# jvasilakes/disentanglement-vae

Hardware: NVIDIA B200
Metric: train_tokens_per_sec (higher is better)
Workload: dtype f32

## Files before the change

disentanglement-vae_b200/_lib.py:

```python
import ctypes as C
import os

_HERE = os.path.dirname(os.path.abspath(__file__))
LIB_PATH = os.path.join(_HERE, "libdvae_b200.so")

MAX_SPACES = 8
HEADS_NSCALARS = 3 + 3 * MAX_SPACES


class DvaeError(RuntimeError):
    pass


_p = C.c_void_p
_i = C.c_int
_l = C.c_int64
_f = C.c_float
_u32 = C.c_uint32
_pp = C.POINTER(C.c_void_p)
_ip = C.POINTER(C.c_int)

SIGNATURES = {
    "dvae_last_error_string": (C.c_char_p, []),
    "dvae_version": (_i, []),
    "dvae_launch_count": (_l, []),
    "dvae_weight_planes_floats": (_l, [_i, _i, _i]),
    "dvae_weight_planes_register": (_i, [_p, _i, _i, _p, _p]),
    "dvae_weight_planes_refresh": (_i, [_p]),
    "dvae_weight_planes_refresh_ex": (_i, [_i, _i, _p]),
    "dvae_weight_planes_enable": (_i, [_i]),
    "dvae_weight_planes_clear": (_i, []),
    "dvae_defer_joins": (_i, [_i]),
    "dvae_join_side_streams": (_i, [_p]),
    "dvae_linear": (_i, [_p, _l, _i, _p, _l, _i, _p, _l, _i, _i, _i, _p, _p, _f, _i, _p]),
    "dvae_tc_linear": (_i, [_p, _l, _i, _p, _l, _i, _p, _l, _i, _i, _i, _p, _p, _f, _i, _i, _p]),
    "dvae_tc16_linear": (_i, [_p, _l, _i, _p, _l, _i, _p, _l, _i, _i, _i, _p, _p, _f, _i, _f, _f, _p, _p, _p]),
    "dvae_colsum": (_i, [_p, _l, _i, _i, _p, _f, _p]),
    "dvae_randn": (_i, [_p, _l, _p, _u32, _p]),
    "dvae_embedding_fwd": (_i, [_p, _i, _p, _l, _l, _i, _i, _f, _p, _u32, _l, _i, _p, _p]),
    "dvae_embedding_bwd": (_i, [_p, _i, _p, _l, _l, _i, _i, _f, _p, _u32, _l, _i, _p, _p]),
    "dvae_bow_encoder_fwd": (_i, [_p, _i, _p, _l, _l, _i, _i, _f, _p, _u32, _p, _l, _p, _p]),
    "dvae_bow_encoder_bwd": (_i, [_p, _l, _p, _i, _p, _l, _l, _i, _i, _f, _p, _u32, _p, _p]),
    "dvae_dropout": (_i, [_p, _l, _l, _i, _f, _p, _u32, _p, _l, _l, _p]),
    "dvae_lstm_step": (_i, [_p, _l, _i, _i, _i, _i, _i, _p, _p, _p, _p, _p, _p, _l, _p, _p, _p, _p, _p]),
    "dvae_vocab_sample_step": (_i, [_p, _l, _i, _i, _i, _p, _p, _p, _u32, _p, _l, _p, _p]),
    "dvae_vocab_sample_step_ex": (_i, [_p, _l, _i, _i, _i, _p, _p, _p, _u32, _p, _l, _p, _p, _p]),
    "dvae_vocab_w_planes_floats": (_l, [_i, _i]),
    "dvae_vocab_w_planes": (_i, [_p, _i, _i, _p, _p]),
    "dvae_vocab_sample_step_planes": (_i, [_p, _l, _i, _i, _i, _p, _p, _p, _p, _u32, _p, _l, _p, _p, _p]),
    "dvae_recount_lengths": (_i, [_p, _l, _l, _i, _i, _l, _l, _l, _p, _p]),
    "dvae_bleu_counts": (_i, [_p, _l, _i, _p, _l, _i, _i, _l, _p, _p]),
    "dvae_bleu_score": (_i, [_p, _p, _p]),
    "dvae_lstm_state_ws_floats": (_l, [_i, _i, _i]),
    "dvae_lstm_seq_fwd": (_i, [_p, _l, _i, _i, _i, _i, _i, _pp, _pp, _pp, _pp, _p, _p, _l, _l, _p, _p, _l, _p, _p,
                               _l, _l, _p, _p, _p, _p]),
    "dvae_lstm_input_proj": (_i, [_p, _l, _i, _i, _i, _i, _i, _pp, _pp, _pp, _p, _p]),
    "dvae_lstm_seq_fwd_ex": (_i, [_p, _l, _i, _i, _i, _i, _i, _pp, _pp, _pp, _pp, _p, _p, _l, _l, _p, _p, _l, _p, _p,
                                  _l, _l, _p, _p, _p, _i, _p]),
    "dvae_lstm_seq_bwd": (_i, [_p, _l, _i, _i, _i, _i, _i, _pp, _pp, _p, _p, _l, _l, _p, _p, _l, _p, _p, _p, _l,
                               _p, _p, _l, _l, _p, _l, _pp, _pp, _pp, _pp, _p, _p, _l, _l, _p, _p]),
    "dvae_lstm_bwd_planes_ws_floats": (_l, [_i, _i, _i, _i, _i]),
    "dvae_lstm_seq_bwd_ex": (_i, [_p, _l, _i, _i, _i, _i, _i, _pp, _pp, _p, _p, _l, _l, _p, _p, _l, _p, _p, _p, _l,
                                  _p, _p, _l, _l, _p, _l, _pp, _pp, _pp, _pp, _p, _p, _l, _l, _p, _p, _p]),
    "dvae_counter_increment": (_i, [_p, _p]),
    "dvae_fork_after": (_i, [_i, _p, _p, C.POINTER(C.c_void_p)]),
    "dvae_nvls_barrier_words": (_l, []),
    "dvae_nvls_all_reduce": (_i, [_p, _l, _pp, _i, _i, _p, C.c_uint32, C.c_uint32, _i, C.c_uint64, _p, _p]),
    "dvae_p2p_all_reduce": (_i, [_pp, _l, _pp, _i, _i, _p, C.c_uint32, C.c_uint32, _i, C.c_uint64, _p, _p]),
    "dvae_heads_ws_floats": (_l, [_i, _i]),
    "dvae_latent_heads_fwd": (_i, [_p, _i, _i, _i, _ip, _ip, _p, _p, _p, _p, _p, _p, _p, _p, _p, _i, _p, _p, _p,
                                   _p, _p, _p, _p, _p]),
    "dvae_heads_bwd_ws_floats": (_l, [_i, _i, _i]),
    "dvae_latent_heads_bwd": (_i, [_p, _i, _i, _i, _ip, _ip, _p, _p, _p, _p, _p, _p, _i, _p, _p, _p, _p, _p, _p,
                                   _p, _p, _p, _p, _p, _p, _p, _p, _p, _p, _p, _p, _p]),
    "dvae_dsc_loss": (_i, [_p, _p, _i, _i, _ip, _ip, _p, _p, _p, _p]),
    "dvae_vocab_ce_ws_floats": (_l, [_i, _i, _i]),
    "dvae_vocab_ce_fwd": (_i, [_p, _l, _i, _i, _i, _i, _p, _p, _p, _l, _p, _i, _p, _p, _p, _p, _p, _p]),
    "dvae_vocab_split_w": (_i, [_p, _i, _i, _i, _p, _p]),
    "dvae_vocab_ce_fwd_ex": (_i, [_p, _l, _i, _i, _i, _i, _p, _p, _p, _l, _p, _i, _p, _p, _p, _p, _p, _i, _p]),
    "dvae_vocab_ce_partials": (_i, [_p, _l, _i, _i, _i, _i, _p, _p, _p, _l, _p, _i, _p, _p]),
    "dvae_vocab_ce_bwd_ws_floats": (_l, [_i, _i, _i]),
    "dvae_vocab_ce_bwd": (_i, [_p, _l, _i, _i, _i, _i, _p, _p, _p, _l, _p, _p, _p, _p, _l, _p, _p, _p, _p, _p]),
    "dvae_entropy_loss": (_i, [_p, _i, _i, _p, _p, _p, _p]),
    "dvae_club_mi": (_i, [_p, _p, _p, _i, _i, _p, _p, _p, _p, _p, _p, _p]),
    "dvae_club_nll": (_i, [_p, _p, _p, _i, _i, _p, _p, _p, _p, _p]),
    "dvae_act_bwd": (_i, [_p, _p, _p, _l, _i, _p]),
    "dvae_relu": (_i, [_p, _l, _p]),
    "dvae_grad_sumsq": (_i, [_p, _l, _p, _p, _p]),
    "dvae_clip_adam": (_i, [_p, _p, _p, _p, _l, _p, _f, _f, _p, _i, _p]),
}

_lib = None
planes_owner = None


def load():
    global _lib
    if _lib is not None:
        return _lib
    if not os.path.exists(LIB_PATH):
        raise DvaeError(
            f"{LIB_PATH} not found: build it with `python -c 'import __graft_entry__ as g; g.build()'` "
            "(nvcc, sm_100a).  There is no CPU or PyTorch fallback for this path.")
    lib = C.CDLL(LIB_PATH)
    for name, (res, args) in SIGNATURES.items():
        try:
            fn = getattr(lib, name)
        except AttributeError as e:
            raise DvaeError(f"{LIB_PATH} does not export {name}") from e
        fn.restype = res
        fn.argtypes = args
    _lib = lib
    return lib


def check(rc, what):
    if rc != 0:
        msg = load().dvae_last_error_string()
        raise DvaeError(f"{what} failed ({rc}): {msg.decode() if msg else ''}")


def ptr(t):
    return None if t is None else t.data_ptr()


def ptr_array(tensors):
    arr = (C.c_void_p * max(len(tensors), 1))()
    for i, t in enumerate(tensors):
        arr[i] = None if t is None else t.data_ptr()
    return arr


def int_array(vals):
    arr = (C.c_int * max(len(vals), 1))()
    for i, v in enumerate(vals):
        arr[i] = int(v)
    return arr


def stream_ptr():
    import torch
    return torch.cuda.current_stream().cuda_stream


def launch_count():
    return int(load().dvae_launch_count())
```

disentanglement-vae_b200/csrc/tc_gemm16.cu:

```cuda
#include <cuda_fp16.h>
#include <stdlib.h>
#include <string.h>

#include "tc_gemm.cuh"
#include "tc_gemm16.cuh"
#include "tc_planes.cuh"

namespace dvae {
namespace tc16 {

using namespace tc;

constexpr int BM = 128, BN = 128, BK = 32;
constexpr int STAGES = 6, MAX_STAGES = 14;
constexpr int RAW_TILE = BM * BK * 4;
constexpr int STAGE_BYTES = 2 * RAW_TILE;
constexpr int PS_PLANE = BM * BK * 2, PS_TILE = 2 * PS_PLANE;
constexpr int PS_LBO = 128, PS_SBO = 512;
static_assert(PS_TILE == RAW_TILE, "in-place conversion: fp16 hi + lo planes occupy exactly the landed fp32 tile");
constexpr int EPI_WARPS = 8, MMA_WARP = 4, TMA_WARP = 5, PROD_WARP0 = 6, PROD_WARPS = 16, EPI2_WARP0 = PROD_WARP0 + PROD_WARPS;
constexpr int NUM_THREADS = (EPI2_WARP0 + 4) * 32;
constexpr int CONV_BARRIER = 1;
constexpr int EPI_SCRATCH_BYTES = 8 * 32 * 32 * 4;
#ifndef DVAE_AS_KB
#define DVAE_AS_KB 2
#endif
constexpr int AS_MAX_KB = 8, AS_KB_PER_STAGE = DVAE_AS_KB, AS_STAGE_BYTES = AS_KB_PER_STAGE * PS_TILE;
constexpr int AS_STAGES = 12 / AS_KB_PER_STAGE, AS_STAGES_NOSCRATCH = 14 / AS_KB_PER_STAGE;
constexpr uint32_t AS_T_AHI = 256, AS_T_ALO = 384;
constexpr float kSingleScale = 256.f;
constexpr int OFF_SCRATCH = STAGES * STAGE_BYTES;
constexpr int OFF_BIAS = OFF_SCRATCH + EPI_SCRATCH_BYTES;
constexpr int OFF_BAR = OFF_BIAS + 8 * 64 * 4;
constexpr int SMEM_BYTES = OFF_BAR + 512;
static_assert(AS_STAGES * AS_STAGE_BYTES <= OFF_SCRATCH, "A-stationary ring must end before the transpose scratch");
static_assert(AS_STAGES_NOSCRATCH * AS_STAGE_BYTES <= OFF_BIAS, "A-stationary mode-1 ring must end before the bias tiles");
static_assert(AS_STAGES_NOSCRATCH <= MAX_STAGES && (3 * MAX_STAGES + 5) * 8 + 4 <= 512, "barrier area");
static_assert(SMEM_BYTES <= 232448, "shared memory per CTA");
constexpr int TMEM_COLS = 512;
constexpr float kLoScale = 2048.f, kLoInv = 1.f / 2048.f;

__device__ __forceinline__ float ex2_ftz(float x) {
  float y;
  asm("ex2.approx.ftz.f32 %0, %1;" : "=f"(y) : "f"(x));
  return y;
}
constexpr float kLog2e = 1.4426950408889634f;

__device__ __forceinline__ unsigned long long gtime16() {
  unsigned long long t;
  asm volatile("mov.u64 %0, %%globaltimer;" : "=l"(t));
  return t;
}
#ifdef DVAE_TC16_PROBES
#define DVAE_TC16_FLAG(bit) (p.dbg_skip_epilogue & (bit))
#define DVAE_TC16_MARK(cond, i) do { if (cond) DBG16(i); } while (0)
#else
#define DVAE_TC16_FLAG(bit) false
#define DVAE_TC16_MARK(cond, i) do { } while (0)
#endif
#define DBG16(i) do { if (p.dbg && blockIdx.x == 0 && blockIdx.y == 0 && blockIdx.z == 0) p.dbg[i] = gtime16(); } while (0)

__device__ __forceinline__ float scale_from_amax(const uint32_t* amax_bits, int n, float static_scale) {
  if (!amax_bits) return static_scale;
  uint32_t mx = 0;
  for (int i = 0; i < n; ++i) mx = max(mx, __ldg(amax_bits + i));
  int se = 267 - (int)(mx >> 23);
  se = se < 1 ? 1 : (se > 253 ? 253 : se);
  return __uint_as_float((unsigned)se << 23);
}

__device__ __forceinline__ void load_tile(uint32_t raw, int mn_major, int ptid, float (&v)[8]) {
  const int row = ptid & 127, kc = ptid >> 7;
  if (!mn_major) {
    const uint32_t ra = raw + (uint32_t)row * 128, sw = row & 7;
#pragma unroll
    for (int i = 0; i < 2; ++i) {
      const uint4 t = lds128(ra + (((uint32_t)(2 * kc + i) ^ sw) << 4));
      v[4 * i] = __uint_as_float(t.x); v[4 * i + 1] = __uint_as_float(t.y);
      v[4 * i + 2] = __uint_as_float(t.z); v[4 * i + 3] = __uint_as_float(t.w);
    }
  } else {
    const uint32_t src = raw + (uint32_t)(8 * kc) * (BM * 4) + (uint32_t)row * 4;
#pragma unroll
    for (int j = 0; j < 8; ++j) v[j] = lds32(src + j * (BM * 4));
  }
}

__device__ __forceinline__ void store_tile(uint32_t tile, int ptid, float s, const float (&v)[8]) {
  const int row = ptid & 127, kc = ptid >> 7;
  const uint32_t base = tile + (uint32_t)(row >> 3) * PS_SBO + (uint32_t)kc * PS_LBO + (row & 7) * 16;
  uint4 hi, lo;
  hi.x = pack_hi_lo(v[0], v[1], s, lo.x);
  hi.y = pack_hi_lo(v[2], v[3], s, lo.y);
  hi.z = pack_hi_lo(v[4], v[5], s, lo.z);
  hi.w = pack_hi_lo(v[6], v[7], s, lo.w);
  sts128(base, hi);
  sts128(base + PS_PLANE, lo);
}

__device__ __forceinline__ uint32_t cluster_size() {
  uint32_t n;
  asm volatile("mov.u32 %0, %%cluster_nctaid.x;" : "=r"(n));
  return n;
}
__device__ __forceinline__ uint32_t cluster_rank() {
  uint32_t r;
  asm volatile("mov.u32 %0, %%cluster_ctarank;" : "=r"(r));
  return r;
}
__device__ __forceinline__ void cluster_sync_all() {
  asm volatile("barrier.cluster.arrive.release.aligned;\n\tbarrier.cluster.wait.acquire.aligned;" ::: "memory");
}
__device__ __forceinline__ void bulk_load_multicast(uint32_t smem_dst, const void* src, uint32_t bytes, uint64_t* bar, uint16_t mask) {
  asm volatile("cp.async.bulk.shared::cluster.global.mbarrier::complete_tx::bytes.multicast::cluster [%0], [%1], %2, [%3], %4;" ::"r"(smem_dst),
               "l"(src), "r"(bytes), "r"(smem_u32(bar)), "h"(mask)
               : "memory");
}
__device__ __forceinline__ void tc_commit_multicast(uint64_t* bar, uint16_t mask) {
  asm volatile("tcgen05.commit.cta_group::1.mbarrier::arrive::one.shared::cluster.multicast::cluster.b64 [%0], %1;" ::"r"(smem_u32(bar)),
               "h"(mask)
               : "memory");
}

__device__ __forceinline__ void bulk_load(uint32_t smem_dst, const void* src, uint32_t bytes, uint64_t* bar) {
  asm volatile("cp.async.bulk.shared::cluster.global.mbarrier::complete_tx::bytes [%0], [%1], %2, [%3];" ::"r"(smem_dst), "l"(src),
               "r"(bytes), "r"(smem_u32(bar))
               : "memory");
}

__global__ void split_planes_kernel(const float* __restrict__ X, int64_t ld, int R, int K, float scale, float lo_scale,
                                    uint8_t* __restrict__ planes) {
  const int KB = (K + BK - 1) / BK, KC = KB * (BK / 8), RP = (R + BM - 1) / BM * BM;
  const int64_t total = (int64_t)RP * KC;
  for (int64_t i = (int64_t)blockIdx.x * blockDim.x + threadIdx.x; i < total; i += (int64_t)gridDim.x * blockDim.x) {
    const int kc = (int)(i % KC), r = (int)(i / KC);
    float v[8];
#pragma unroll
    for (int e = 0; e < 8; ++e) v[e] = (r < R && kc * 8 + e < K) ? __ldg(X + (int64_t)r * ld + kc * 8 + e) : 0.f;
    uint4 h, l;
    h.x = pack_hi_lo(v[0], v[1], scale, l.x, lo_scale); h.y = pack_hi_lo(v[2], v[3], scale, l.y, lo_scale);
    h.z = pack_hi_lo(v[4], v[5], scale, l.z, lo_scale); h.w = pack_hi_lo(v[6], v[7], scale, l.w, lo_scale);
    const int64_t off = ((int64_t)(r >> 7) * KB + (kc >> 2)) * (2 * PS_PLANE) + ((r & 127) >> 3) * PS_SBO + (kc & 3) * PS_LBO + (r & 7) * 16;
    *reinterpret_cast<uint4*>(planes + off) = h;
    *reinterpret_cast<uint4*>(planes + off + PS_PLANE) = l;
  }
}

__global__ void weight_planes_kernel(PlaneTable tab) {
  const PlaneTable::Entry e = tab.e[blockIdx.y >> 1];
  const int tr = blockIdx.y & 1;
  uint8_t* out = reinterpret_cast<uint8_t*>(tr ? e.planes_t : e.planes);
  if (!out) return;
  const int R = tr ? e.C : e.R, K = tr ? e.R : e.C;
  const int64_t ld = e.ld ? e.ld : e.C;
  const float sc = scale_from_amax(e.amax, e.amax_n, 1.f);
  const int KB = (K + BK - 1) / BK, KC = KB * (BK / 8), RP = (R + BM - 1) / BM * BM;
  const int64_t total = (int64_t)RP * KC;
  for (int64_t i = (int64_t)blockIdx.x * blockDim.x + threadIdx.x; i < total; i += (int64_t)gridDim.x * blockDim.x) {
    int kc, r;
    if (!tr) { kc = (int)(i % KC); r = (int)(i / KC); }
    else { r = (int)(i % RP); kc = (int)(i / RP); }
    float v[8];
#pragma unroll
    for (int j = 0; j < 8; ++j) {
      const int k = kc * 8 + j;
      v[j] = (r < R && k < K) ? __ldg(tr ? e.w + (int64_t)k * ld + r : e.w + (int64_t)r * ld + k) : 0.f;
    }
    uint4 h, l;
    h.x = pack_hi_lo(v[0], v[1], sc, l.x); h.y = pack_hi_lo(v[2], v[3], sc, l.y);
    h.z = pack_hi_lo(v[4], v[5], sc, l.z); h.w = pack_hi_lo(v[6], v[7], sc, l.w);
    const int64_t off = ((int64_t)(r >> 7) * KB + (kc >> 2)) * (2 * PS_PLANE) + ((r & 127) >> 3) * PS_SBO + (kc & 3) * PS_LBO + (r & 7) * 16;
    *reinterpret_cast<uint4*>(out + off) = h;
    *reinterpret_cast<uint4*>(out + off + PS_PLANE) = l;
  }
}

int weight_planes_launch(const PlaneTable& tab, cudaStream_t st) {
  if (tab.n <= 0) return DVAE_OK;
  int64_t most = 1;
  for (int i = 0; i < tab.n; ++i) most = max(most, (int64_t)tab.e[i].R * tab.e[i].C / 8);
  int bx = ceil_div(most, 256 * 4);
  bx = bx < 8 ? 8 : (bx > 4 * 148 ? 4 * 148 : bx);
  weight_planes_kernel<<<dim3(bx, 2 * tab.n), 256, 0, st>>>(tab);
  DVAE_LAUNCH_CHECK();
  return DVAE_OK;
}

__global__ void __launch_bounds__(NUM_THREADS, 1)
tc16_gemm_kernel(const __grid_constant__ CUtensorMap tmA, const __grid_constant__ CUtensorMap tmB, Params p) {
  extern __shared__ __align__(1024) uint8_t smem[];
  if (p.skip_flag && *p.skip_flag) return;
  uint64_t* bars = reinterpret_cast<uint64_t*>(smem + OFF_BAR);
  uint64_t* full = bars;
  uint64_t* empty = bars + MAX_STAGES;
  uint64_t* raw_full = bars + 2 * MAX_STAGES;
  uint64_t* tmem_full = raw_full + MAX_STAGES;
  uint64_t* tmem_empty = tmem_full + 2;
  uint64_t* a_full = tmem_empty + 2;
  uint32_t* tmem_slot = reinterpret_cast<uint32_t*>(a_full + 1);

  const int tid = threadIdx.x, warp = tid >> 5, lane = tid & 31;
  const bool wide_epi = p.presplit && p.mode != 0;
  const uint32_t csize = p.mcast ? cluster_size() : 1, crank = p.mcast ? cluster_rank() : 0;
  const uint16_t cmask = (uint16_t)((1u << csize) - 1);
  const bool conv_as_epi = wide_epi && warp >= PROD_WARP0 && warp < PROD_WARP0 + EPI_WARPS;
  asm volatile("griddepcontrol.launch_dependents;" ::: "memory");
  if (tid == 0) DBG16(0);
  if (p.zero_buf) {
    float4* z4 = reinterpret_cast<float4*>(p.zero_buf);
    const int64_t nblk = (int64_t)gridDim.x * gridDim.y * gridDim.z;
    const int64_t blk = ((int64_t)blockIdx.z * gridDim.y + blockIdx.y) * gridDim.x + blockIdx.x;
    for (int64_t i = blk * NUM_THREADS + tid; i < p.zero_n4; i += nblk * NUM_THREADS) z4[i] = make_float4(0.f, 0.f, 0.f, 0.f);
    if (p.zero_buf2) {
      float4* y4 = reinterpret_cast<float4*>(p.zero_buf2);
      for (int64_t i = blk * NUM_THREADS + tid; i < p.zero2_n4; i += nblk * NUM_THREADS) y4[i] = make_float4(0.f, 0.f, 0.f, 0.f);
    }
  }
  const int m0 = blockIdx.x * BM;
  const int nt0 = blockIdx.y * p.tiles_per_cta;
  const int n_tiles = (p.N + BN - 1) / BN;
  const int nt1 = min(n_tiles, nt0 + p.tiles_per_cta);
  const int nkb_total = (p.K + BK - 1) / BK;
  const int kb0 = blockIdx.z * p.kb_per_split;
  const int nkb = max(0, min(nkb_total, kb0 + p.kb_per_split) - kb0);
  const int b_tile0 = p.b_row0 / BN;

  if (tid == 0) {
    if (smem_u32(smem) & 1023) {
      printf("dvae tc16_gemm: dynamic shared memory base is not 1024-byte aligned\n");
      __trap();
    }
    for (int s = 0; s < MAX_STAGES; ++s) {
      mbar_init(&full[s], p.presplit ? 1 : PROD_WARPS / 2 + (p.b_presplit ? 1 : 0));
      mbar_init(&empty[s], p.mcast ? csize : 1);
      mbar_init(&raw_full[s], 1);
    }
    for (int a = 0; a < 2; ++a) {
      mbar_init(&tmem_full[a], 1);
      mbar_init(&tmem_empty[a], wide_epi ? 2 * EPI_WARPS : EPI_WARPS);
    }
    mbar_init(a_full, 2 * EPI_WARPS);
    fence_barrier_init();
  }
  if (warp == TMA_WARP && lane == 0 && !p.presplit) {
    tma_prefetch_desc(&tmA);
    tma_prefetch_desc(&tmB);
  }
  const bool a_stat = p.presplit && !p.no_astat && nkb_total <= AS_MAX_KB && gridDim.z == 1;
  const int nstages = a_stat ? (p.mode == 1 ? AS_STAGES_NOSCRATCH : AS_STAGES) : STAGES;
  const uint32_t stage_bytes = a_stat ? AS_STAGE_BYTES : STAGE_BYTES;
  const int a_blk = min((int)blockIdx.x, (p.M + BM - 1) / BM - 1);
  if (warp == MMA_WARP) tmem_alloc(tmem_slot, TMEM_COLS);
  tc_fence_before();
  __syncthreads();
  if (p.mcast) cluster_sync_all();
  tc_fence_after();
  const uint32_t tmem_base = *tmem_slot;
  const uint32_t smem_u = smem_u32(smem);

  if (warp == TMA_WARP) {
    if (DVAE_TC16_FLAG(16)) {
    } else if (lane == 0 && a_stat) {
      const uint8_t* b_planes = reinterpret_cast<const uint8_t*>(p.b_planes);
      int stage = 0, phase = 0;
      for (int nt = nt0; nt < nt1; ++nt) {
        for (int kb = 0; kb < nkb; kb += AS_KB_PER_STAGE) {
          DVAE_TC16_MARK(nt == nt0 + 1 && kb < 8, 32 + 2 * kb);
          if (!DVAE_TC16_FLAG(8)) mbar_wait(&empty[stage], phase ^ 1);
          else mbar_wait(&full[stage], phase ^ 1);
          DVAE_TC16_MARK(nt == nt0 + 1 && kb < 8, 33 + 2 * kb);
          const uint32_t dst = smem_u + stage * AS_STAGE_BYTES;
          const uint32_t bytes = (uint32_t)min(AS_KB_PER_STAGE, nkb - kb) * PS_TILE;
          mbar_expect_tx(&full[stage], bytes);
          const uint8_t* src = b_planes + ((int64_t)(nt + b_tile0) * nkb_total + kb) * PS_TILE;
          if (csize == 1) {
            bulk_load(dst, src, bytes, &full[stage]);
          } else {
            const uint32_t part = bytes / csize, off = crank * part;
            bulk_load_multicast(dst + off, src + off, part, &full[stage], cmask);
          }
          if (++stage == nstages) { stage = 0; phase ^= 1; }
        }
      }
      if (DVAE_TC16_FLAG(8))
        for (int s2 = 0; s2 < nstages; ++s2) mbar_wait(&full[s2], s2 < stage ? phase : phase ^ 1);
    } else if (lane == 0 && p.presplit) {
      const uint8_t* a_tiles = reinterpret_cast<const uint8_t*>(p.a_planes) +
                               ((int64_t)blockIdx.x * (p.a_kbtot ? p.a_kbtot : nkb_total) + p.a_kb0) * PS_TILE;
      const uint8_t* b_planes = reinterpret_cast<const uint8_t*>(p.b_planes);
      int stage = 0, phase = 0;
      for (int nt = nt0; nt < nt1; ++nt) {
        for (int kb = 0; kb < nkb; ++kb) {
          mbar_wait(&empty[stage], phase ^ 1);
          const uint32_t dst = smem_u + stage * STAGE_BYTES;
          mbar_expect_tx(&full[stage], STAGE_BYTES);
          bulk_load(dst, a_tiles + (int64_t)(kb0 + kb) * PS_TILE, PS_TILE, &full[stage]);
          bulk_load(dst + PS_TILE, b_planes + ((int64_t)(nt + b_tile0) * (p.b_kbtot ? p.b_kbtot : nkb_total) + p.b_kb0 + kb0 + kb) * PS_TILE,
                    PS_TILE, &full[stage]);
          if (++stage == STAGES) { stage = 0; phase ^= 1; }
        }
      }
    } else if (lane == 0) {
      int stage = 0, phase = 0;
      for (int nt = nt0; nt < nt1; ++nt) {
        for (int kb = 0; kb < nkb; ++kb) {
          mbar_wait(&empty[stage], phase ^ 1);
          uint8_t* dst = smem + stage * STAGE_BYTES;
          mbar_expect_tx(&raw_full[stage], p.b_presplit ? RAW_TILE : STAGE_BYTES);
          const int k0 = (kb0 + kb) * BK;
          if (!p.a_mn) tma_load_2d(dst, &tmA, k0, m0, &raw_full[stage]);
          else tma_load_2d(dst, &tmA, m0, k0, &raw_full[stage]);
          if (p.b_presplit) {
            mbar_expect_tx(&full[stage], PS_TILE);
            bulk_load(smem_u + stage * STAGE_BYTES + RAW_TILE,
                      reinterpret_cast<const uint8_t*>(p.b_planes) + ((int64_t)(nt + b_tile0) * p.b_kbtot + p.b_kb0 + kb0 + kb) * PS_TILE,
                      PS_TILE, &full[stage]);
          } else if (!p.b_mn) tma_load_2d(dst + RAW_TILE, &tmB, k0, nt * BN, &raw_full[stage]);
          else tma_load_2d(dst + RAW_TILE, &tmB, nt * BN, k0, &raw_full[stage]);
          if (++stage == STAGES) { stage = 0; phase ^= 1; }
        }
      }
    }
  } else if (warp >= PROD_WARP0 && warp < EPI2_WARP0 && !conv_as_epi) {
    const int ptid = tid - PROD_WARP0 * 32;
    const float sa = scale_from_amax(p.a_amax, p.a_amax_n, p.a_scale), sb = scale_from_amax(p.b_amax, p.b_amax_n, p.b_scale);
    const int n_items = p.presplit ? 0 : (nt1 - nt0) * nkb;
    const int grp = ptid >> 8, gtid = ptid & 255;
    for (int it = grp; it < n_items; it += 2) {
      const int stage = it % STAGES, phase = (it / STAGES) & 1;
      DVAE_TC16_MARK(ptid == 0 && it == 12, 2);
      mbar_wait(&raw_full[stage], phase);
      DVAE_TC16_MARK(ptid == 0 && it == 12, 3);
      float va0[8], va1[8], vb0[8], vb1[8];
      const uint32_t st = smem_u + stage * STAGE_BYTES;
      load_tile(st, p.a_mn, gtid, va0);
      load_tile(st, p.a_mn, gtid + 256, va1);
      if (!p.b_presplit) {
        load_tile(st + RAW_TILE, p.b_mn, gtid, vb0);
        load_tile(st + RAW_TILE, p.b_mn, gtid + 256, vb1);
      }
      asm volatile("bar.sync %0, %1;" ::"r"(CONV_BARRIER + grp), "n"(PROD_WARPS * 16) : "memory");
      store_tile(st, gtid, sa, va0);
      store_tile(st, gtid + 256, sa, va1);
      if (!p.b_presplit) {
        store_tile(st + PS_TILE, gtid, sb, vb0);
        store_tile(st + PS_TILE, gtid + 256, sb, vb1);
      }
      DVAE_TC16_MARK(ptid == 0 && it == 12, 4);
      fence_proxy_async();
      __syncwarp();
      if (lane == 0) mbar_arrive(&full[stage]);
      DVAE_TC16_MARK(ptid == 0 && it == 12, 5);
    }
  } else if (warp == MMA_WARP) {
    constexpr uint32_t idesc = (1u << 4) | ((uint32_t)(BN >> 3) << 17) | ((uint32_t)(BM >> 4) << 24);
    if (elect_one() && nkb > 0) {
      if (a_stat) {
        mbar_wait(a_full, 0);
        tc_fence_after();
      }
      constexpr uint32_t d_hi = ((PS_SBO >> 4) & 0x3FFF) | (1u << 14);
      constexpr uint32_t d_lo = ((PS_LBO >> 4) & 0x3FFF) << 16;
      constexpr uint32_t kstep16 = (2 * PS_LBO) >> 4, plane16 = PS_PLANE >> 4;
      const uint32_t stage16 = stage_bytes >> 4;
      const uint32_t base16 = smem_u >> 4;
      const uint32_t ring16 = base16;
      const uint32_t b_off16 = a_stat ? 0 : 2 * plane16;
      auto desc = [&](uint32_t addr16) { return ((uint64_t)d_hi << 32) | (uint64_t)(d_lo | (addr16 & 0x3FFF)); };
      int stage = 0, phase = 0;
      uint32_t st16 = ring16;
      for (int tile = 0; tile < nt1 - nt0; ++tile) {
        const int acc = tile & 1;
        if (tile >= 2) {
          mbar_wait(&tmem_empty[acc], ((tile >> 1) - 1) & 1);
          tc_fence_after();
        }
        const uint32_t d1 = tmem_base + (a_stat ? acc * 128 : acc * 256), d2 = d1 + 128;
        if (a_stat) {
          for (int kb = 0; kb < nkb; kb += AS_KB_PER_STAGE) {
            if (!DVAE_TC16_FLAG(4)) mbar_wait(&full[stage], phase);
            if (!DVAE_TC16_FLAG(2)) {
#pragma unroll
              for (int kk = 0; kk < AS_KB_PER_STAGE; ++kk) {
                if (kb + kk < nkb) {
                  const uint32_t ta = tmem_base + (uint32_t)(kb + kk) * 16, sb16 = st16 + kk * (PS_TILE >> 4);
#pragma unroll
                  for (int k = 0; k < BK / 16; ++k) {
                    const uint32_t adv = k * kstep16;
                    mma_f16_ts(d1, ta + AS_T_AHI + 8 * k, desc(sb16 + adv), idesc, (kb | kk | k) ? 1u : 0u);
                    mma_f16_ts(d1, ta + AS_T_AHI + 8 * k, desc(sb16 + plane16 + adv), idesc, 1u);
                    mma_f16_ts(d1, ta + AS_T_ALO + 8 * k, desc(sb16 + adv), idesc, 1u);
                  }
                }
              }
            }
            if (!DVAE_TC16_FLAG(8)) {
              if (csize == 1) tc_commit(&empty[stage]);
              else tc_commit_multicast(&empty[stage], cmask);
            }
            st16 += stage16;
            if (++stage == nstages) { stage = 0; phase ^= 1; st16 = ring16; }
          }
          tc_commit(&tmem_full[acc]);
          continue;
        }
        for (int kb = 0; kb < nkb; ++kb) {
          DVAE_TC16_MARK(tile == 1 && kb < 8, 48 + 2 * kb);
          if (!DVAE_TC16_FLAG(4)) mbar_wait(&full[stage], phase);
          DVAE_TC16_MARK(tile == 1 && kb < 8, 49 + 2 * kb);
          const uint32_t sa16 = st16, sb16 = st16 + b_off16;
          if (!DVAE_TC16_FLAG(2)) {
#pragma unroll
            for (int k = 0; k < BK / 16; ++k) {
              const uint32_t adv = k * kstep16;
              const uint32_t accum = (kb | k) ? 1u : 0u;
              mma_f16(d1, desc(sa16 + adv), desc(sb16 + adv), idesc, accum);
              mma_f16(d2, desc(sa16 + adv), desc(sb16 + plane16 + adv), idesc, accum);
              mma_f16(d2, desc(sa16 + plane16 + adv), desc(sb16 + adv), idesc, 1u);
            }
          }
          if (!DVAE_TC16_FLAG(8)) {
            if (csize == 1) tc_commit(&empty[stage]);
            else tc_commit_multicast(&empty[stage], cmask);
          }
          st16 += stage16;
          if (++stage == nstages) { stage = 0; phase ^= 1; st16 = ring16; }
        }
        tc_commit(&tmem_full[acc]);
      }
    }
    __syncwarp();
  } else {
    const int quarter = warp & 3, ehalf = warp >= EPI2_WARP0 ? 1 : 0;
    const int c_lo = !wide_epi ? 2 * ehalf : (conv_as_epi ? 1 + 2 * ((warp - PROD_WARP0) >> 2) : 2 * ehalf);
    const int c_hi = wide_epi ? c_lo + 1 : c_lo + 2;
    const int ew = wide_epi ? c_lo * 4 + quarter : ehalf * 4 + quarter;
    const int row = m0 + quarter * 32 + lane;
    const bool row_ok = row < p.M;
    const float oscale = p.alpha * (p.alpha_dev ? *p.alpha_dev : 1.f) * ((p.c_row_scale && row_ok) ? __ldg(p.c_row_scale + row) : 1.f) /
                         (scale_from_amax(p.a_amax, p.a_amax_n, p.a_scale) * scale_from_amax(p.b_amax, p.b_amax_n, p.b_scale));
    float rm = -INFINITY, rs = 0.f, rt = 0.f, rav = -INFINITY, row_lse = 0.f, row_nlse2 = 0.f, row_scale = 0.f;
    int rai = 0x7fffffff, tgt = -1;
    if (p.mode != 0 && row_ok) {
      const int b = row % p.B, tpos = row / p.B + 1;
      if (p.targets) tgt = (int)p.targets[(int64_t)b * p.tgt_stride_b + tpos];
      if (p.mode == 2) {
        row_lse = p.lse[row];
        row_nlse2 = -row_lse * kLog2e;
        row_scale = (tpos < p.lengths[b]) ? (p.grad_scale ? p.grad_scale[0] : 1.f) / (float)p.B : 0.f;
        tgt -= p.v0;
      }
    }
    if (a_stat) {
      const uint8_t* a_tiles = reinterpret_cast<const uint8_t*>(p.a_planes) + (int64_t)a_blk * nkb_total * PS_TILE;
      const int r = quarter * 32 + lane;
      const uint32_t roff = (uint32_t)(r >> 3) * PS_SBO + (r & 7) * 16;
      const uint32_t tlane = tmem_base + ((uint32_t)(quarter * 32) << 16);
#pragma unroll
      for (int i = 0; i < 2; ++i) {
        const int kb = 2 * c_lo + i;
        if (kb < nkb) {
          const uint8_t* t = a_tiles + (int64_t)kb * PS_TILE + roff;
#pragma unroll
          for (int pl = 0; pl < 2; ++pl) {
            uint32_t v[16];
#pragma unroll
            for (int kc = 0; kc < 4; ++kc) {
              const uint4 q = __ldg(reinterpret_cast<const uint4*>(t + pl * PS_PLANE + kc * PS_LBO));
              v[4 * kc] = q.x; v[4 * kc + 1] = q.y; v[4 * kc + 2] = q.z; v[4 * kc + 3] = q.w;
            }
            tmem_st16(tlane + (pl ? AS_T_ALO : AS_T_AHI) + kb * 16, v);
          }
        }
      }
      tmem_st_wait();
      tc_fence_before();
      __syncwarp();
      if (lane == 0) mbar_arrive(a_full);
    }
    float bias_next[2] = {0.f, 0.f};
    if (p.mode != 0 && nkb > 0) {
#pragma unroll
      for (int h2 = 0; h2 < 2; ++h2) {
        const int col = nt0 * BN + (c_lo + h2) * 32 + lane;
        bias_next[h2] = (nt0 < nt1 && h2 < c_hi - c_lo && col < p.N) ? __ldg(p.bias + col) : 0.f;
      }
    }
    int tile = 0;
    for (int nt = nt0; nt < nt1 && nkb > 0; ++nt, ++tile) {
      const int n0 = nt * BN, acc = tile & 1;
      mbar_wait(&tmem_full[acc], (tile >> 1) & 1);
      tc_fence_after();
      if (tid == 0 && tile < 4) DBG16(14 + 2 * tile);
      DVAE_TC16_MARK(tid == 0 && tile == 2, 96);
      float* sbias = reinterpret_cast<float*>(smem + OFF_BIAS) + (wide_epi ? ew * 32 : ew * 64);
      const uint32_t sbias_u = smem_u + OFF_BIAS + (wide_epi ? ew * 32 : ew * 64) * 4;
      if (p.mode != 0) {
        __syncwarp();
#pragma unroll
        for (int h2 = 0; h2 < 2; ++h2)
          if (h2 < c_hi - c_lo) sbias[h2 * 32 + lane] = bias_next[h2];
        __syncwarp();
#pragma unroll
        for (int h2 = 0; h2 < 2; ++h2) {
          const int col = n0 + BN + (c_lo + h2) * 32 + lane;
          bias_next[h2] = (nt + 1 < nt1 && h2 < c_hi - c_lo && col < p.N) ? __ldg(p.bias + col) : 0.f;
        }
      }
      DVAE_TC16_MARK(tid == 0 && tile == 2, 97);
#pragma unroll 1
      for (int c = c_lo; c < c_hi; ++c) {
        const int col0 = n0 + c * 32;
        if (col0 >= p.N || DVAE_TC16_FLAG(~0)) continue;
        const uint32_t ta = tmem_base + ((uint32_t)(quarter * 32) << 16) + (a_stat ? acc * 128 : acc * 256) + c * 32;
        if (p.mode == 2 && wide_epi) {
          const uint32_t sc = smem_u + OFF_SCRATCH + ew * (32 * 16 * 4);
          const int r0 = m0 + quarter * 32;
          const int nr = min(32, p.M - r0);
          const bool dead = row_scale == 0.f;
          DVAE_TC16_MARK(tid == 0 && tile == 2, 104);
#pragma unroll
          for (int hh = 0; hh < 2; ++hh) {
#pragma unroll
            for (int h8 = 0; h8 < 2; ++h8) {
              float v[8], w[8];
              if (a_stat) {
                tmem_ld8_pair(ta + hh * 16 + h8 * 8, ta + hh * 16 + h8 * 8, v, w);
#pragma unroll
                for (int j = 0; j < 8; ++j) w[j] = 0.f;
              } else {
                tmem_ld8_pair(ta + hh * 16 + h8 * 8, ta + 128 + hh * 16 + h8 * 8, v, w);
              }
#pragma unroll
              for (int q = 0; q < 2; ++q) {
                const uint4 t = lds128(sbias_u + (hh * 16 + h8 * 8 + 4 * q) * 4);
                const float bq[4] = {__uint_as_float(t.x), __uint_as_float(t.y), __uint_as_float(t.z), __uint_as_float(t.w)};
#pragma unroll
                for (int jj = 0; jj < 4; ++jj) {
                  const int j = 4 * q + jj, col = col0 + hh * 16 + h8 * 8 + j;
                  const float e = ex2_ftz(fmaf(fmaf(fmaf(w[j], kLoInv, v[j]), oscale, bq[jj]), kLog2e, row_nlse2));
                  v[j] = (dead || col >= p.N) ? 0.f : (e - (col == tgt ? 1.f : 0.f)) * row_scale;
                }
              }
              if (p.p_planes_a && col0 + hh * 16 + h8 * 8 < p.p_kb_a * BK && m0 < (p.M + BM - 1) / BM * BM)
                store_plane_chunk(p.p_planes_a, row, col0 + hh * 16 + h8 * 8, p.p_kb_a, v, p.p_scale);
#pragma unroll
              for (int j = 0; j < 8; ++j) sts32(sc + (lane * 16 + ((h8 * 8 + j) ^ ((lane >> 1) & 15))) * 4, v[j]);
            }
            __syncwarp();
            if (p.p_planes_t) {
              const int cc = lane & 15, rg = lane >> 4, colw = col0 + hh * 16 + cc;
              float tv[16], ssum = 0.f;
#pragma unroll
              for (int k = 0; k < 16; ++k) {
                const int r = rg * 16 + k;
                tv[k] = lds32(sc + (r * 16 + (cc ^ ((r >> 1) & 15))) * 4);
                ssum += tv[k];
              }
              ssum += __shfl_xor_sync(0xffffffffu, ssum, 16);
              if (colw < p.N) {
                if (rg == 0 && p.p_colsum) atomicAdd(p.p_colsum + colw, ssum);
                const float lo8[8] = {tv[0], tv[1], tv[2], tv[3], tv[4], tv[5], tv[6], tv[7]};
                const float hi8[8] = {tv[8], tv[9], tv[10], tv[11], tv[12], tv[13], tv[14], tv[15]};
                if (r0 + rg * 16 < p.p_kb_t * BK) store_plane_chunk(p.p_planes_t, colw, r0 + rg * 16, p.p_kb_t, lo8, p.p_scale);
                if (r0 + rg * 16 + 8 < p.p_kb_t * BK) store_plane_chunk(p.p_planes_t, colw, r0 + rg * 16 + 8, p.p_kb_t, hi8, p.p_scale);
              }
              __syncwarp();
              continue;
            }
            const int colw = col0 + hh * 16 + (lane & 15);
            float* cp = p.C + (int64_t)(r0 + (lane >> 4)) * p.ldc + colw;
            if (colw < p.N) {
#pragma unroll
              for (int k = 0; k < 16; ++k) {
                const float val = lds32(sc + ((2 * k + (lane >> 4)) * 16 + ((lane & 15) ^ k)) * 4);
                if (2 * k + (lane >> 4) < nr) cp[(int64_t)(2 * k) * p.ldc] = val;
              }
            }
            __syncwarp();
          }
          DVAE_TC16_MARK(tid == 0 && tile == 2, 105);
          continue;
        }
        if (p.mode != 1) {
          const uint32_t sc = smem_u + OFF_SCRATCH + ew * (32 * 32 * 4);
          DVAE_TC16_MARK(tid == 0 && tile == 2, 104 + 3 * (c - c_lo));
#pragma unroll
          for (int hh = 0; hh < 2; ++hh) {
            float v[16], w[16];
            tmem_ld16_pair(ta + hh * 16, ta + 128 + hh * 16, v, w);
            float x[16];
#pragma unroll
            for (int j = 0; j < 16; ++j) x[j] = fmaf(w[j], kLoInv, v[j]) * oscale;
            if (p.mode == 2) {
              float bv[16];
#pragma unroll
              for (int q = 0; q < 4; ++q) {
                const uint4 t = lds128(sbias_u + ((c - c_lo) * 32 + hh * 16 + 4 * q) * 4);
                bv[4 * q] = __uint_as_float(t.x); bv[4 * q + 1] = __uint_as_float(t.y);
                bv[4 * q + 2] = __uint_as_float(t.z); bv[4 * q + 3] = __uint_as_float(t.w);
              }
              const bool dead = row_scale == 0.f;
#pragma unroll
              for (int j = 0; j < 16; ++j) {
                const int col = col0 + hh * 16 + j;
                const float e = ex2_ftz(fmaf(x[j] + bv[j], kLog2e, row_nlse2));
                x[j] = (dead || col >= p.N) ? 0.f : (e - (col == tgt ? 1.f : 0.f)) * row_scale;
              }
            }
#pragma unroll
            for (int j = 0; j < 16; ++j) sts32(sc + (lane * 32 + ((hh * 16 + j) ^ lane)) * 4, x[j]);
          }
          DVAE_TC16_MARK(tid == 0 && tile == 2, 105 + 3 * (c - c_lo));
          __syncwarp();
          const int col = col0 + lane;
          const int r0 = m0 + quarter * 32;
          const int nr = min(32, p.M - r0);
          if (col < p.N && nr > 0) {
            const bool split = gridDim.z > 1 || p.atomic_out;
            float badd = 0.f;
            if (p.mode == 0 && (!split || blockIdx.z == 0)) {
              if (p.bias) badd += __ldg(p.bias + col);
              if (p.bias2) badd += __ldg(p.bias2 + col);
            }
            float* cp = p.C + (int64_t)r0 * p.ldc + col;
            const int64_t ldc = p.ldc;
            auto chunk_at = [&](int rr) { return lds32(sc + (uint32_t)(rr * 32 + (lane ^ rr)) * 4); };
            if (p.mode == 2 || (!split && p.act == 0 && p.beta == 0.f)) {
              if (nr == 32) {
#pragma unroll
                for (int rr = 0; rr < 32; ++rr) cp[rr * ldc] = chunk_at(rr) + badd;
              } else {
                for (int rr = 0; rr < nr; ++rr) cp[rr * ldc] = chunk_at(rr) + badd;
              }
            } else if (split) {
              for (int rr = 0; rr < nr; ++rr) atomicAdd(cp + rr * ldc, chunk_at(rr) + badd);
            } else {
              const float beta = p.beta;
              const bool do_tanh = p.act == 1;
              if (nr == 32 && beta != 0.f) {
#pragma unroll 1
                for (int r8 = 0; r8 < 32; r8 += 8) {
                  float old[8];
#pragma unroll
                  for (int rr = 0; rr < 8; ++rr) old[rr] = cp[(r8 + rr) * ldc];
#pragma unroll
                  for (int rr = 0; rr < 8; ++rr) {
                    float x = chunk_at(r8 + rr) + badd;
                    if (do_tanh) x = tanhf(x);
                    cp[(r8 + rr) * ldc] = fmaf(beta, old[rr], x);
                  }
                }
              } else {
                for (int rr = 0; rr < nr; ++rr) {
                  float x = chunk_at(rr) + badd;
                  if (do_tanh) x = tanhf(x);
                  if (beta != 0.f) x = fmaf(beta, cp[rr * ldc], x);
                  cp[rr * ldc] = x;
                }
              }
            }
          }
          DVAE_TC16_MARK(tid == 0 && tile == 2, 106 + 3 * (c - c_lo));
          __syncwarp();
          continue;
        }
        const bool sample = p.gumbel_seed != nullptr;
        const uint64_t gseed = sample ? *p.gumbel_seed : 0;
#pragma unroll
        for (int hh = 0; hh < 2; ++hh) {
          float v[16], w[16];
          DVAE_TC16_MARK(tid == 0 && tile == 2, 98 + 3 * hh);
          if (a_stat) {
            tmem_ld16(ta + hh * 16, v);
#pragma unroll
            for (int j = 0; j < 16; ++j) w[j] = 0.f;
          } else {
            tmem_ld16_pair(ta + hh * 16, ta + 128 + hh * 16, v, w);
          }
          DVAE_TC16_MARK(tid == 0 && tile == 2, 99 + 3 * hh);
          if (!row_ok) continue;
          const int base = col0 + hh * 16;
          float x[16], xs[16];
          {
            const uint32_t ba = sbias_u + ((c - c_lo) * 32 + hh * 16) * 4;
            float bv[16];
#pragma unroll
            for (int q = 0; q < 4; ++q) {
              const uint4 t = lds128(ba + q * 16);
              bv[4 * q] = __uint_as_float(t.x); bv[4 * q + 1] = __uint_as_float(t.y);
              bv[4 * q + 2] = __uint_as_float(t.z); bv[4 * q + 3] = __uint_as_float(t.w);
            }
#pragma unroll
            for (int j = 0; j < 16; ++j) x[j] = fmaf(fmaf(w[j], kLoInv, v[j]), oscale, bv[j]);
            if (base + 16 > p.N) {
#pragma unroll
              for (int j = 0; j < 16; ++j)
                if (base + j >= p.N) x[j] = -INFINITY;
            }
          }
          if (sample) {
#pragma unroll
            for (int j4 = 0; j4 < 16; j4 += 4) {
              float g[4];
              gumbel4(gseed, p.gumbel_salt, row, base + j4, (p.N + 3) >> 2, g);
#pragma unroll
              for (int jj = 0; jj < 4; ++jj) xs[j4 + jj] = x[j4 + jj] + g[jj];
            }
          } else {
#pragma unroll
            for (int j = 0; j < 16; ++j) xs[j] = x[j];
          }
          float m8[8], m4[4];
#pragma unroll
          for (int j = 0; j < 8; ++j) m8[j] = fmaxf(xs[2 * j], xs[2 * j + 1]);
#pragma unroll
          for (int j = 0; j < 4; ++j) m4[j] = fmaxf(m8[2 * j], m8[2 * j + 1]);
          const float smax = fmaxf(fmaxf(m4[0], m4[1]), fmaxf(m4[2], m4[3]));
          if (smax > rav) {
            unsigned eq = 0;
#pragma unroll
            for (int j = 0; j < 16; ++j) eq |= (xs[j] == smax ? 1u : 0u) << j;
            rav = smax;
            rai = base + __ffs(eq) - 1;
          }
          if (tgt >= base && tgt < base + 16) {
#pragma unroll
            for (int j = 0; j < 16; ++j)
              if (base + j == tgt) rt = x[j];
          }
          float tmax = smax;
          if (sample) {
#pragma unroll
            for (int j = 0; j < 8; ++j) m8[j] = fmaxf(x[2 * j], x[2 * j + 1]);
#pragma unroll
            for (int j = 0; j < 4; ++j) m4[j] = fmaxf(m8[2 * j], m8[2 * j + 1]);
            tmax = fmaxf(fmaxf(m4[0], m4[1]), fmaxf(m4[2], m4[3]));
          }
          if (tmax > rm) { rs *= ex2_ftz((rm - tmax) * kLog2e); rm = tmax; }
          const float nrm2 = -rm * kLog2e;
          float e8[8];
#pragma unroll
          for (int j = 0; j < 8; ++j) e8[j] = ex2_ftz(fmaf(x[2 * j], kLog2e, nrm2)) + ex2_ftz(fmaf(x[2 * j + 1], kLog2e, nrm2));
          rs += ((e8[0] + e8[1]) + (e8[2] + e8[3])) + ((e8[4] + e8[5]) + (e8[6] + e8[7]));
          DVAE_TC16_MARK(tid == 0 && tile == 2, 100 + 3 * hh);
        }
      }
      tc_fence_before();
      __syncwarp();
      if (lane == 0) mbar_arrive(&tmem_empty[acc]);
      if (tid == 0 && tile < 4) DBG16(15 + 2 * tile);
    }
    if (p.mode == 1 && row_ok) {
      const int64_t sp = wide_epi ? (int64_t)blockIdx.y * 4 + c_lo : (int64_t)blockIdx.y * 2 + ehalf;
      *reinterpret_cast<float4*>(p.part + (sp * p.M + row) * 4) = make_float4(rm, rs, rt, rav);
      p.part_idx[sp * p.M + row] = rai;
    }
  }
  tc_fence_before();
  __syncthreads();
  if (p.mcast) cluster_sync_all();
  if (warp == MMA_WARP) tmem_dealloc(tmem_base, TMEM_COLS);
  if (tid == 0) DBG16(1);
}

bool supported(const float* A, int64_t lda, int trans_a, const float* B, int64_t ldb, int trans_b, int M, int N, int K) {
  return enabled() && shape_ok(A, lda, trans_a, B, ldb, trans_b, M, N, K);
}

bool enabled() {
  const char* e = getenv("DVAE_GEMM_IMPL");
  return !(e && (e[0] == 't' || e[0] == 's'));
}

bool shape_ok(const float* A, int64_t lda, int trans_a, const float* B, int64_t ldb, int trans_b, int M, int N, int K) {
  if (((reinterpret_cast<uintptr_t>(A) | reinterpret_cast<uintptr_t>(B)) & 15) || lda % 4 || ldb % 4) return false;
  return M >= 1 && N >= 1 && K >= 1;
}

typedef CUresult (*EncodeTiledFn)(CUtensorMap*, CUtensorMapDataType, cuuint32_t, void*, const cuuint64_t*, const cuuint64_t*,
                                  const cuuint32_t*, const cuuint32_t*, CUtensorMapInterleave, CUtensorMapSwizzle,
                                  CUtensorMapL2promotion, CUtensorMapFloatOOBfill);
static EncodeTiledFn encode_fn() {
  static EncodeTiledFn fn = nullptr;
  if (!fn) {
    void* q = nullptr;
    cudaDriverEntryPointQueryResult r;
    if (cudaGetDriverEntryPoint("cuTensorMapEncodeTiled", &q, cudaEnableDefault, &r) == cudaSuccess && r == cudaDriverEntryPointSuccess)
      fn = reinterpret_cast<EncodeTiledFn>(q);
  }
  return fn;
}
static int make_map(CUtensorMap* m, const float* base, int64_t ld, int mn_major, int rows, int K) {
  EncodeTiledFn fn = encode_fn();
  DVAE_REQUIRE(fn != nullptr, "tc16_gemm: cuTensorMapEncodeTiled is not available from the driver");
  cuuint64_t dims[2] = {(cuuint64_t)(mn_major ? rows : K), (cuuint64_t)(mn_major ? K : rows)};
  cuuint64_t strides[1] = {(cuuint64_t)ld * sizeof(float)};
  cuuint32_t box[2] = {(cuuint32_t)(mn_major ? BM : BK), (cuuint32_t)(mn_major ? BK : BM)};
  cuuint32_t estr[2] = {1, 1};
  CUresult r = fn(m, CU_TENSOR_MAP_DATA_TYPE_FLOAT32, 2, const_cast<float*>(base), dims, strides, box, estr,
                  CU_TENSOR_MAP_INTERLEAVE_NONE, mn_major ? CU_TENSOR_MAP_SWIZZLE_NONE : CU_TENSOR_MAP_SWIZZLE_128B,
                  CU_TENSOR_MAP_L2_PROMOTION_L2_128B, CU_TENSOR_MAP_FLOAT_OOB_FILL_NONE);
  DVAE_REQUIRE(r == CUDA_SUCCESS, "tc16_gemm: cuTensorMapEncodeTiled failed (%d) rows=%d K=%d ld=%lld", (int)r, rows, K, (long long)ld);
  return DVAE_OK;
}

int64_t plane_floats(int R, int K) { return (int64_t)ceil_div(R, BM) * BM * ceil_div(K, BK) * BK; }

bool presplit_enabled() {
  const char* e = getenv("DVAE_VOCAB_PRESPLIT");
  return !(e && e[0] == '0');
}

bool single_acc_planes(int K) { return ceil_div(K, BK) <= AS_MAX_KB; }

int split_planes(const float* X, int64_t ld, int R, int K, float scale, void* planes, cudaStream_t st, bool force_dual) {
  const bool single = !force_dual && single_acc_planes(K);
  const float lo_scale = single ? 1.f : kLoScale;
  if (single) scale *= kSingleScale;
  DVAE_REQUIRE(X && planes && R > 0 && K > 0, "tc16 split_planes: bad argument");
  const int64_t work = (int64_t)ceil_div(R, BM) * BM * ceil_div(K, BK) * (BK / 8);
  int blocks = ceil_div(work, 256);
  if (blocks > 148 * 8) blocks = 148 * 8;
  split_planes_kernel<<<blocks, 256, 0, st>>>(X, ld, R, K, scale, lo_scale, reinterpret_cast<uint8_t*>(planes));
  DVAE_LAUNCH_CHECK();
  return DVAE_OK;
}

static int launch(const Params& p_in, dim3 grid, cudaStream_t st) {
  Params p = p_in;
  if (p.dbg)
    if (const char* e = getenv("DVAE_TC_DBG_MODE"))
      if (atoi(e) != p.mode) p.dbg = nullptr;
  static bool ready = false;
  if (!ready) {
    DVAE_CUDA(cudaFuncSetAttribute(tc16_gemm_kernel, cudaFuncAttributeMaxDynamicSharedMemorySize, SMEM_BYTES));
    ready = true;
  }
  CUtensorMap ma, mb;
  int rc;
  if (p.presplit) {
    memset(&ma, 0, sizeof(ma));
    memset(&mb, 0, sizeof(mb));
  } else {
    if ((rc = make_map(&ma, p.A, p.lda, p.a_mn, p.M, p.K))) return rc;
    if (p.b_presplit) memset(&mb, 0, sizeof(mb));
    else if ((rc = make_map(&mb, p.Bm, p.ldb, p.b_mn, p.N, p.K))) return rc;
  }
  const char* mc_env = getenv("DVAE_TC16_MCAST");
  const bool mcast_on = mc_env && mc_env[0] == '1';
  if (mcast_on && p.presplit && ceil_div(p.K, BK) <= AS_MAX_KB && grid.z == 1 && grid.x >= 2) {
    p.mcast = 1;
    grid.x = (grid.x + 1) / 2 * 2;
    cudaLaunchConfig_t cfg = {};
    cfg.gridDim = grid; cfg.blockDim = dim3(NUM_THREADS); cfg.dynamicSmemBytes = SMEM_BYTES; cfg.stream = st;
    cudaLaunchAttribute attr[1];
    attr[0].id = cudaLaunchAttributeClusterDimension;
    attr[0].val.clusterDim.x = 2; attr[0].val.clusterDim.y = 1; attr[0].val.clusterDim.z = 1;
    cfg.attrs = attr; cfg.numAttrs = 1;
    DVAE_CUDA(cudaLaunchKernelEx(&cfg, tc16_gemm_kernel, ma, mb, p));
    DVAE_LAUNCH_CHECK();
    return DVAE_OK;
  }
  tc16_gemm_kernel<<<grid, NUM_THREADS, SMEM_BYTES, st>>>(ma, mb, p);
  DVAE_LAUNCH_CHECK();
  return DVAE_OK;
}

__global__ void tc16_scale_rows_kernel(float* C, int64_t ldc, int M, int N, float beta) {
  int64_t i = (int64_t)blockIdx.x * blockDim.x + threadIdx.x;
  if (i >= (int64_t)M * N) return;
  float* c = C + (i / N) * ldc + (i % N);
  *c = beta == 0.f ? 0.f : *c * beta;
}

static void apply_hints(Params& p, const GemmHints& h) {
  if (const char* e = getenv("DVAE_TC_DBG")) p.dbg = reinterpret_cast<unsigned long long*>(strtoull(e, nullptr, 0));
  if (const char* e = getenv("DVAE_TC_SKIP_EPILOGUE")) p.dbg_skip_epilogue = atoi(e);
  p.a_amax = h.a_amax_bits; p.b_amax = h.b_amax_bits; p.a_amax_n = h.a_amax_n; p.b_amax_n = h.b_amax_n;
  p.a_scale = h.a_scale; p.b_scale = h.b_scale;
  p.alpha = 1.f; p.alpha_dev = nullptr;
  p.atomic_out = h.atomic_out ? 1 : 0;
}

int linear(const float* A, int64_t lda, int trans_a, const float* B, int64_t ldb, int trans_b, float* C, int64_t ldc, int M,
           int N, int K, const float* bias, const float* bias2, float beta, int act, const GemmHints& hints, cudaStream_t st) {
  Params p = {};
  p.A = A; p.lda = lda; p.Bm = B; p.ldb = ldb;
  p.M = M; p.N = N; p.K = K; p.a_mn = trans_a ? 1 : 0; p.b_mn = trans_b ? 1 : 0; p.tiles_per_cta = 1;
  p.C = C; p.ldc = ldc; p.bias = bias; p.bias2 = bias2; p.beta = beta; p.act = act; p.mode = 0;
  apply_hints(p, hints);
  PlaneHit hit;
  if (hints.b_planes) {
    p.b_presplit = 1; p.b_planes = hints.b_planes; p.b_row0 = hints.b_tile0 * BN; p.b_kb0 = hints.b_kb0; p.b_kbtot = hints.b_kbtot;
  } else if (!hints.b_amax_bits && hints.b_scale == 1.f && find_weight_planes(B, ldb, trans_b, N, K, &hit)) {
    p.b_presplit = 1; p.b_planes = hit.planes; p.b_row0 = hit.tile0 * BN; p.b_kb0 = hit.kb0; p.b_kbtot = hit.kbtot;
  }
  const int tiles = ceil_div(M, BM) * ceil_div(N, BN), nkb = ceil_div(K, BK);
  int splits = 1;
  if (act == 0 && nkb >= 16) {
    const float t_kb = p.b_presplit ? 0.33f + 0.15f * p.a_mn : 0.5f + 0.2f * (p.a_mn + p.b_mn);
    float best = 1e30f;
    for (int s2 = 1; s2 <= 16 && s2 <= nkb / 4; ++s2) {
      const int kbs = ceil_div(nkb, s2), se = ceil_div(nkb, kbs);
      if (se != s2) continue;
      if (hints.max_ctas > 0 && s2 > 1 && tiles * se > hints.max_ctas) break;
      const int waves = ceil_div(tiles * se, 148);
      const float t = waves * (kbs * t_kb + (se > 1 ? 6.f : 4.f)) + (se > 1 ? 2.f : 0.f);
      if (t < best * 0.95f) { best = t; splits = se; }
    }
  }
  if (const char* e = getenv("DVAE_TC16_SPLITS_BIG_MN"))
    if (p.a_mn && p.b_mn && tiles >= 64 && act == 0) splits = atoi(e);
  p.kb_per_split = ceil_div(nkb, splits);
  splits = ceil_div(nkb, p.kb_per_split);
  if (splits > 1 && beta != 1.f && !(beta == 0.f && hints.c_zeroed)) {
    if (beta == 0.f && ldc == N) {
      DVAE_CUDA(cudaMemsetAsync(C, 0, sizeof(float) * (size_t)M * N, st));
    } else {
      tc16_scale_rows_kernel<<<ceil_div((int64_t)M * N, 256), 256, 0, st>>>(C, ldc, M, N, beta);
      DVAE_LAUNCH_CHECK();
    }
  }
  const int conc = hints.concurrency > 1 ? hints.concurrency : 1;
  const int sm_budget = hints.max_ctas > 0 ? hints.max_ctas : 148;
  if (splits == 1 && tiles * conc > sm_budget && ceil_div(N, BN) >= 2) {
    int tpc = ceil_div(tiles * conc, sm_budget);
    if (tpc < 2) tpc = 2;
    if (tpc > ceil_div(N, BN)) tpc = ceil_div(N, BN);
    p.tiles_per_cta = tpc;
  }
  return launch(p, dim3(ceil_div(M, BM), ceil_div(ceil_div(N, BN), p.tiles_per_cta), splits), st);
}

int linear_planes(const void* a_planes, const void* b_planes, float* C, int64_t ldc, int M, int N, int K, const float* bias,
                  float beta, int act, float a_scale, float b_scale, const float* c_row_scale, bool c_zeroed, int max_splits,
                  cudaStream_t st, int b_kb0, int b_kbtot, int max_ctas, int a_kb0, int a_kbtot, const uint32_t* a_amax, int a_amax_n) {
  DVAE_REQUIRE(a_planes && b_planes && C && M > 0 && N > 0 && K > 0, "tc16 linear_planes: bad argument");
  Params p = {};
  p.presplit = 1; p.no_astat = 1; p.a_planes = a_planes; p.b_planes = b_planes; p.a_rows = M; p.b_rows = N;
  p.M = M; p.N = N; p.K = K; p.tiles_per_cta = 1; p.C = C; p.ldc = ldc; p.bias = bias; p.beta = beta; p.act = act; p.mode = 0;
  apply_hints(p, GemmHints());
  p.a_scale = a_scale; p.b_scale = b_scale; p.c_row_scale = c_row_scale;
  p.b_kb0 = b_kb0; p.b_kbtot = b_kbtot;
  p.a_kb0 = a_kb0; p.a_kbtot = a_kbtot;
  if (a_amax) { p.a_amax = a_amax; p.a_amax_n = a_amax_n; }
  const int tiles = ceil_div(M, BM) * ceil_div(N, BN), nkb = ceil_div(K, BK);
  int splits = 1;
  if (act == 0 && nkb >= 8) {
    const float t_kb = 0.27f;
    float best = 1e30f;
    for (int s2 = 1; s2 <= max_splits && s2 <= nkb / 4; ++s2) {
      const int kbs = ceil_div(nkb, s2), se = ceil_div(nkb, kbs);
      if (se != s2) continue;
      if (max_ctas > 0 && s2 > 1 && tiles * se > max_ctas) break;
      const int waves = ceil_div(tiles * se, 148);
      const float t = waves * (kbs * t_kb + (se > 1 ? 5.f : 4.f)) + (se > 1 ? 1.5f : 0.f);
      if (t < best * 0.95f) { best = t; splits = se; }
    }
  }
  p.kb_per_split = ceil_div(nkb, splits);
  splits = ceil_div(nkb, p.kb_per_split);
  if (splits > 1 && beta != 1.f && !(beta == 0.f && c_zeroed)) {
    if (beta == 0.f && ldc == N) {
      DVAE_CUDA(cudaMemsetAsync(C, 0, sizeof(float) * (size_t)M * N, st));
    } else {
      tc16_scale_rows_kernel<<<ceil_div((int64_t)M * N, 256), 256, 0, st>>>(C, ldc, M, N, beta);
      DVAE_LAUNCH_CHECK();
    }
  }
  const int sm_budget = max_ctas > 0 ? max_ctas : 148;
  if (splits == 1 && tiles > sm_budget && ceil_div(N, BN) >= 2) {
    int tpc = ceil_div(tiles, sm_budget);
    if (tpc < 2) tpc = 2;
    if (tpc > ceil_div(N, BN)) tpc = ceil_div(N, BN);
    p.tiles_per_cta = tpc;
  }
  return launch(p, dim3(ceil_div(M, BM), ceil_div(ceil_div(N, BN), p.tiles_per_cta), splits), st);
}

int ce_partials(const float* h, int64_t ldh, int N, int B, int H, int V, const float* w, const float* bias,
                const int64_t* targets, int64_t tgt_stride_b, const int64_t* lengths, int tiles_per_split, int nsplit,
                float* part, int* part_idx, const uint64_t* gumbel_seed, uint32_t gumbel_salt, const void* h_planes,
                const void* w_planes, const int* skip_flag, cudaStream_t st) {
  Params p = {};
  p.skip_flag = skip_flag;
  if (h_planes && w_planes) { p.presplit = 1; p.a_planes = h_planes; p.b_planes = w_planes; p.a_rows = N; p.b_rows = V; }
  p.A = h; p.lda = ldh; p.Bm = w; p.ldb = H;
  p.M = N; p.N = V; p.K = H; p.tiles_per_cta = tiles_per_split; p.bias = bias; p.mode = 1;
  p.kb_per_split = ceil_div(H, BK);
  p.targets = targets; p.tgt_stride_b = tgt_stride_b; p.lengths = lengths; p.B = B; p.part = part; p.part_idx = part_idx;
  p.gumbel_seed = gumbel_seed; p.gumbel_salt = gumbel_salt;
  apply_hints(p, GemmHints());
  if (p.presplit && single_acc_planes(H)) p.a_scale = p.b_scale = kSingleScale;
  return launch(p, dim3(ceil_div(N, BM), nsplit, 1), st);
}

int softmax_grad(const float* h, int64_t ldh, int N, int B, int H, int V, int v0, int vc, const float* w, const float* bias,
                 const int64_t* targets, int64_t tgt_stride_b, const int64_t* lengths, const float* lse,
                 const float* grad_scale, float* P, int64_t ldp, const void* h_planes, const void* w_planes, float* zero_buf,
                 int64_t zero_n4, float* zero_buf2, int64_t zero2_n4, cudaStream_t st, void* p_planes_a, void* p_planes_t,
                 float* p_colsum, float p_scale) {
  Params p = {};
  if (p_planes_a && p_planes_t && h_planes && w_planes) {
    p.p_planes_a = reinterpret_cast<uint8_t*>(p_planes_a); p.p_planes_t = reinterpret_cast<uint8_t*>(p_planes_t);
    p.p_colsum = p_colsum; p.p_scale = p_scale; p.p_kb_a = ceil_div(vc, BK); p.p_kb_t = ceil_div(N, BK);
  }
  p.zero_buf = zero_buf; p.zero_n4 = zero_n4; p.zero_buf2 = zero_buf2; p.zero2_n4 = zero2_n4;
  if (!p.zero_buf) { p.zero_buf = p.zero_buf2; p.zero_n4 = p.zero2_n4; p.zero_buf2 = nullptr; p.zero2_n4 = 0; }
  DVAE_REQUIRE(!(h_planes && w_planes) || v0 % BN == 0, "tc16 softmax_grad: pre-split chunks must start on a %d-row block (v0=%d)", BN, v0);
  if (h_planes && w_planes) { p.presplit = 1; p.a_planes = h_planes; p.b_planes = w_planes; p.a_rows = N; p.b_rows = V; p.b_row0 = v0; }
  p.A = h; p.lda = ldh; p.Bm = w + (int64_t)v0 * H; p.ldb = H;
  const int row_tiles = ceil_div(N, BM), col_tiles = ceil_div(vc, BN);
  int per_cta = ceil_div(col_tiles, max(1, 148 / row_tiles));
  if (per_cta < 1) per_cta = 1;
  p.M = N; p.N = vc; p.K = H; p.tiles_per_cta = per_cta; p.bias = bias + v0; p.mode = 2;
  p.kb_per_split = ceil_div(H, BK);
  p.targets = targets; p.tgt_stride_b = tgt_stride_b; p.lengths = lengths; p.B = B; p.lse = lse; p.grad_scale = grad_scale;
  p.v0 = v0; p.C = P; p.ldc = ldp;
  apply_hints(p, GemmHints());
  if (p.presplit && single_acc_planes(H)) p.a_scale = p.b_scale = kSingleScale;
  return launch(p, dim3(row_tiles, ceil_div(col_tiles, per_cta), 1), st);
}

}
}

extern "C" int dvae_tc16_linear(const float* A, int64_t lda, int trans_a, const float* B, int64_t ldb, int trans_b, float* C,
                                int64_t ldc, int M, int N, int K, const float* bias, const float* bias2, float beta, int act,
                                float a_scale, float b_scale, const uint32_t* a_amax_bits, const uint32_t* b_amax_bits,
                                void* stream) {
  DVAE_REQUIRE(A && B && C && M > 0 && N > 0 && K > 0, "dvae_tc16_linear: bad argument");
  DVAE_REQUIRE(act == 0 || act == 1, "dvae_tc16_linear: unknown activation %d", act);
  DVAE_REQUIRE(dvae::tc16::shape_ok(A, lda, trans_a, B, ldb, trans_b, M, N, K),
               "dvae_tc16_linear: operands must be 16-byte aligned with ld %% 4 == 0 (TMA)");
  dvae::GemmHints h;
  h.a_scale = a_scale; h.b_scale = b_scale; h.a_amax_bits = a_amax_bits; h.b_amax_bits = b_amax_bits;
  return dvae::tc16::linear(A, lda, trans_a, B, ldb, trans_b, C, ldc, M, N, K, bias, bias2, beta, act, h, (cudaStream_t)stream);
}
```

disentanglement-vae_b200/csrc/tc_gemm16.cuh:

```cuda
#pragma once
#include "common.cuh"

namespace dvae {
namespace tc16 {

struct Params {
  const float* A; int64_t lda;
  const float* Bm; int64_t ldb;
  int M, N, K;
  int a_mn, b_mn;
  int tiles_per_cta;
  float* C; int64_t ldc;
  const float* bias; const float* bias2;
  float beta; int act;
  int mode;
  int kb_per_split;
  const uint32_t* a_amax; const uint32_t* b_amax; float a_scale, b_scale; int a_amax_n, b_amax_n;
  float alpha; const float* alpha_dev;
  const int64_t* targets; int64_t tgt_stride_b; const int64_t* lengths; int B;
  float* part; int* part_idx;
  const float* lse; const float* grad_scale; int v0;
  const uint64_t* gumbel_seed; uint32_t gumbel_salt;
  float* zero_buf; int64_t zero_n4;
  float* zero_buf2; int64_t zero2_n4;
  int mcast;
  int a_kbtot; int a_kb0;
  int b_presplit; int b_kbtot; int b_kb0;
  int atomic_out;
  int no_astat;
  const float* c_row_scale;
  int presplit; int b_row0;
  const void* a_planes; const void* b_planes; int a_rows, b_rows;
  uint8_t* p_planes_a; uint8_t* p_planes_t; float* p_colsum; float p_scale; int p_kb_a, p_kb_t;
  const int* skip_flag;
  int dbg_skip_epilogue;
  unsigned long long* dbg;
};

bool enabled();
bool shape_ok(const float* A, int64_t lda, int trans_a, const float* B, int64_t ldb, int trans_b, int M, int N, int K);
bool supported(const float* A, int64_t lda, int trans_a, const float* B, int64_t ldb, int trans_b, int M, int N, int K);
int linear(const float* A, int64_t lda, int trans_a, const float* B, int64_t ldb, int trans_b, float* C, int64_t ldc, int M,
           int N, int K, const float* bias, const float* bias2, float beta, int act, const GemmHints& hints, cudaStream_t st);
int64_t plane_floats(int R, int K);
int split_planes(const float* X, int64_t ld, int R, int K, float scale, void* planes, cudaStream_t st, bool force_dual = false);
int linear_planes(const void* a_planes, const void* b_planes, float* C, int64_t ldc, int M, int N, int K, const float* bias,
                  float beta, int act, float a_scale, float b_scale, const float* c_row_scale, bool c_zeroed, int max_splits,
                  cudaStream_t st, int b_kb0 = 0, int b_kbtot = 0, int max_ctas = 0, int a_kb0 = 0, int a_kbtot = 0,
                  const uint32_t* a_amax = nullptr, int a_amax_n = 1);
constexpr int kMaxPlaneEntries = 24;
struct PlaneTable {
  struct Entry { const float* w; int R, C; void* planes; void* planes_t; int64_t ld; const uint32_t* amax; int amax_n; };
  Entry e[kMaxPlaneEntries];
  int n;
};
int weight_planes_launch(const PlaneTable& tab, cudaStream_t st);
struct PlaneHit { const void* planes; int tile0, kb0, kbtot; };
bool find_weight_planes(const float* B, int64_t ldb, int trans_b, int N, int K, PlaneHit* hit);
bool presplit_enabled();
int ce_partials(const float* h, int64_t ldh, int N, int B, int H, int V, const float* w, const float* bias,
                const int64_t* targets, int64_t tgt_stride_b, const int64_t* lengths, int tiles_per_split, int nsplit,
                float* part, int* part_idx, const uint64_t* gumbel_seed, uint32_t gumbel_salt, const void* h_planes,
                const void* w_planes, const int* skip_flag, cudaStream_t st);
int softmax_grad(const float* h, int64_t ldh, int N, int B, int H, int V, int v0, int vc, const float* w, const float* bias,
                 const int64_t* targets, int64_t tgt_stride_b, const int64_t* lengths, const float* lse,
                 const float* grad_scale, float* P, int64_t ldp, const void* h_planes, const void* w_planes, float* zero_buf,
                 int64_t zero_n4, float* zero_buf2, int64_t zero2_n4, cudaStream_t st, void* p_planes_a = nullptr,
                 void* p_planes_t = nullptr, float* p_colsum = nullptr, float p_scale = 1.f);

}
}
```

disentanglement-vae_b200/csrc/tc_planes.cuh:

```cuda
#pragma once
#include <cuda_fp16.h>

#include "common.cuh"

namespace dvae {
namespace tc16 {

constexpr int kPlaneRows = 128, kPlaneK = 32;
constexpr int kPlaneBytes = kPlaneRows * kPlaneK * 2, kPlaneTileBytes = 2 * kPlaneBytes;
constexpr float kPlaneLoScale = 2048.f;

__device__ __forceinline__ uint32_t pack_hi_lo(float x0, float x1, float s, uint32_t& lo, float ls = kPlaneLoScale) {
  const float2 x = __fmul2_rn(make_float2(x0, x1), make_float2(s, s));
  const __half2 h = __float22half2_rn(x);
  const float2 hf = __half22float2(h);
  const float2 r = __ffma2_rn(x, make_float2(ls, ls), __fmul2_rn(hf, make_float2(-ls, -ls)));
  const __half2 l = __float22half2_rn(r);
  lo = *reinterpret_cast<const uint32_t*>(&l);
  return *reinterpret_cast<const uint32_t*>(&h);
}

__host__ __device__ __forceinline__ int64_t plane_chunk_offset(int r, int k, int KB) {
  return ((int64_t)(r >> 7) * KB + (k >> 5)) * kPlaneTileBytes + ((r & 127) >> 3) * 512 + ((k & 31) >> 3) * 128 + (r & 7) * 16;
}

__device__ __forceinline__ void store_plane_chunk(uint8_t* planes, int r, int k, int KB, const float (&v)[8], float s) {
  uint4 h, l;
  h.x = pack_hi_lo(v[0], v[1], s, l.x); h.y = pack_hi_lo(v[2], v[3], s, l.y);
  h.z = pack_hi_lo(v[4], v[5], s, l.z); h.w = pack_hi_lo(v[6], v[7], s, l.w);
  const int64_t off = plane_chunk_offset(r, k, KB);
  *reinterpret_cast<uint4*>(planes + off) = h;
  *reinterpret_cast<uint4*>(planes + off + kPlaneBytes) = l;
}

}
}
```

disentanglement-vae_b200/csrc/vocab_ce.cu:

```cuda
#include <math.h>

#include "gemm_simt.cuh"
#include "tc_gemm16.cuh"

namespace dvae {

int linear_impl(const float* A, int64_t lda, int trans_a, const float* B, int64_t ldb, int trans_b, float* C,
                int64_t ldc, int M, int N, int K, const float* bias, const float* bias2, float beta, int act,
                cudaStream_t st);
int colsum_impl(const float* X, int64_t ldx, int M, int N, float* out, float beta, cudaStream_t st);

using GCE = GemmTile<128, 128, 16, 8, 8, true, true>;

struct CeArgs;
static bool use_tc16(int N, int V, int H, const float* h, int64_t ldh, const float* w) {
  return !force_simt_gemm() && N >= 64 && V >= 128 && H >= 32 && tc16::supported(h, ldh, 0, w, H, 0, N, V, H);
}
static bool use_presplit(int N, int V, int H) { return tc16::presplit_enabled() && H % 32 == 0 && N >= 256 && V >= 1024; }

struct CeArgs {
  const float* h; int64_t ldh;
  const float* w; const float* bias;
  const int64_t* targets; int64_t tgt_stride_b;
  const int64_t* lengths;
  int N, B, H, V, sos;
  int tiles_per_split, nsplit;
  float* part;
  int* part_idx;
  const uint64_t* gumbel_seed; uint32_t gumbel_salt;
  const void* h_planes; const void* w_planes;
  const int* skip_flag;
};

__device__ __forceinline__ void merge_ms(float& m, float& s, float m2, float s2) {
  float M = fmaxf(m, m2);
  if (M == -INFINITY) { s = 0.f; m = M; return; }
  s = s * expf(m - M) + s2 * expf(m2 - M);
  m = M;
}

__global__ void __launch_bounds__(GCE::NT) vocab_ce_fwd_kernel(CeArgs p) {
  __shared__ __align__(16) float smem[GCE::SMEM_FLOATS];
  if (p.skip_flag && *p.skip_flag) return;
  const int m0 = blockIdx.x * GCE::BM, split = blockIdx.y;
  const int ty = threadIdx.x / GCE::TX, tx = threadIdx.x % GCE::TX;
  const int vtiles = (p.V + GCE::BN - 1) / GCE::BN;
  const int vt0 = split * p.tiles_per_split, vt1 = min(vtiles, vt0 + p.tiles_per_split);
  float rm[GCE::TM], rs[GCE::TM], rt[GCE::TM], rav[GCE::TM];
  int rai[GCE::TM], tgt[GCE::TM];
#pragma unroll
  for (int i = 0; i < GCE::TM; ++i) {
    rm[i] = -INFINITY; rs[i] = 0.f; rt[i] = 0.f; rav[i] = -INFINITY; rai[i] = 0x7fffffff;
    int n = m0 + GCE::row_of(ty, i);
    tgt[i] = -1;
    if (n < p.N && p.targets) tgt[i] = (int)p.targets[(int64_t)(n % p.B) * p.tgt_stride_b + (n / p.B) + 1];
  }
  for (int vt = vt0; vt < vt1; ++vt) {
    const int n0 = vt * GCE::BN;
    float acc[GCE::TM][GCE::TN];
#pragma unroll
    for (int i = 0; i < GCE::TM; ++i)
#pragma unroll
      for (int j = 0; j < GCE::TN; ++j) acc[i][j] = 0.f;
    GCE::run(p.h, p.ldh, m0, p.N, p.w, p.H, n0, p.V, 0, p.H, p.H, smem, acc);
    float bj[GCE::TN];
    int cj[GCE::TN];
#pragma unroll
    for (int j = 0; j < GCE::TN; ++j) {
      cj[j] = n0 + GCE::col_of(tx, j);
      bj[j] = cj[j] < p.V ? p.bias[cj[j]] : 0.f;
    }
#pragma unroll
    for (int i = 0; i < GCE::TM; ++i) {
      float tmax = -INFINITY;
      float gn[GCE::TN];
#pragma unroll
      for (int j = 0; j < GCE::TN; ++j) gn[j] = 0.f;
      if (p.gumbel_seed) {
        const uint64_t gseed = *p.gumbel_seed;
        const int n = m0 + GCE::row_of(ty, i);
#pragma unroll
        for (int j4 = 0; j4 < GCE::TN; j4 += 4) {
          float g[4];
          gumbel4(gseed, p.gumbel_salt, n, cj[j4], (p.V + 3) >> 2, g);
          gn[j4] = g[0]; gn[j4 + 1] = g[1]; gn[j4 + 2] = g[2]; gn[j4 + 3] = g[3];
        }
      }
#pragma unroll
      for (int j = 0; j < GCE::TN; ++j) {
        float v = cj[j] < p.V ? acc[i][j] + bj[j] : -INFINITY;
        acc[i][j] = v;
        tmax = fmaxf(tmax, v);
        const float vs = v + gn[j];
        if (vs > rav[i] || (vs == rav[i] && cj[j] < rai[i])) { rav[i] = vs; rai[i] = cj[j]; }
        if (cj[j] == tgt[i]) rt[i] = v;
      }
      if (tmax > rm[i]) { rs[i] *= expf(rm[i] - tmax); rm[i] = tmax; }
      if (rm[i] != -INFINITY) {
#pragma unroll
        for (int j = 0; j < GCE::TN; ++j) rs[i] += expf(acc[i][j] - rm[i]);
      }
    }
  }
#pragma unroll
  for (int i = 0; i < GCE::TM; ++i) {
#pragma unroll
    for (int o = 8; o > 0; o >>= 1) {
      float m2 = __shfl_xor_sync(0xffffffffu, rm[i], o), s2 = __shfl_xor_sync(0xffffffffu, rs[i], o);
      float t2 = __shfl_xor_sync(0xffffffffu, rt[i], o), av2 = __shfl_xor_sync(0xffffffffu, rav[i], o);
      int ai2 = __shfl_xor_sync(0xffffffffu, rai[i], o);
      merge_ms(rm[i], rs[i], m2, s2);
      rt[i] += t2;
      if (av2 > rav[i] || (av2 == rav[i] && ai2 < rai[i])) { rav[i] = av2; rai[i] = ai2; }
    }
    int n = m0 + GCE::row_of(ty, i);
    if (tx == 0 && n < p.N) {
      float4 o4 = make_float4(rm[i], rs[i], rt[i], rav[i]);
      *reinterpret_cast<float4*>(p.part + ((int64_t)split * p.N + n) * 4) = o4;
      p.part_idx[(int64_t)split * p.N + n] = rai[i];
    }
  }
}

constexpr int kFinThreads = 128, kFinMaxBlocks = 96, kFinLanes = 8;
__global__ void __launch_bounds__(kFinThreads) vocab_ce_finalize_kernel(CeArgs p, float* lse, float* nll, int32_t* argmax,
                                                                       float* block_sums) {
  __shared__ float red[kFinThreads / 32];
  const int sub = threadIdx.x % kFinLanes, slot = threadIdx.x / kFinLanes;
  constexpr int kRows = kFinThreads / kFinLanes;
  float local = 0.f;
  for (int n0 = blockIdx.x * kRows; n0 < p.N; n0 += gridDim.x * kRows) {
    const int n = n0 + slot;
    float m = -INFINITY, s = 0.f, t = 0.f, av = -INFINITY;
    int ai = 0x7fffffff;
    if (n < p.N) {
      for (int sp = sub; sp < p.nsplit; sp += kFinLanes) {
        float4 q = *reinterpret_cast<const float4*>(p.part + ((int64_t)sp * p.N + n) * 4);
        int qi = p.part_idx[(int64_t)sp * p.N + n];
        merge_ms(m, s, q.x, q.y);
        t += q.z;
        if (q.w > av || (q.w == av && qi < ai)) { av = q.w; ai = qi; }
      }
    }
#pragma unroll
    for (int o = 1; o < kFinLanes; o <<= 1) {
      const float m2 = __shfl_xor_sync(0xffffffffu, m, o), s2 = __shfl_xor_sync(0xffffffffu, s, o);
      const float t2 = __shfl_xor_sync(0xffffffffu, t, o), av2 = __shfl_xor_sync(0xffffffffu, av, o);
      const int ai2 = __shfl_xor_sync(0xffffffffu, ai, o);
      merge_ms(m, s, m2, s2);
      t += t2;
      if (av2 > av || (av2 == av && ai2 < ai)) { av = av2; ai = ai2; }
    }
    if (sub == 0 && n < p.N) {
      float l = m + logf(s), e = l - t;
      if (lse) lse[n] = l;
      if (nll) nll[n] = e;
      if (argmax) argmax[n] = ai;
      int b = n % p.B, tpos = n / p.B + 1;
      if (tpos < p.lengths[b]) local += e;
    }
  }
  local = warp_sum(local);
  if ((threadIdx.x & 31) == 0) red[threadIdx.x >> 5] = local;
  __syncthreads();
  if (threadIdx.x == 0) {
    float tot = 0.f;
    for (int i = 0; i < kFinThreads / 32; ++i) tot += red[i];
    block_sums[blockIdx.x] = tot;
  }
}

__global__ void __launch_bounds__(128) vocab_ce_loss_kernel(CeArgs p, const float* block_sums, int nblocks, float* loss) {
  __shared__ float red[4];
  float local = 0.f;
  for (int b = threadIdx.x; b < p.B; b += blockDim.x) {
    if (p.lengths[b] > 0) {
      float l0 = (float)(1.0 + log(1.0 + (double)(p.V - 1) * exp(-1.0)));
      local += l0 - (p.targets[(int64_t)b * p.tgt_stride_b] == p.sos ? 1.f : 0.f);
    }
  }
  local = warp_sum(local);
  if ((threadIdx.x & 31) == 0) red[threadIdx.x >> 5] = local;
  __syncthreads();
  if (threadIdx.x == 0) {
    float tot = red[0] + red[1] + red[2] + red[3];
    for (int i = 0; i < nblocks; ++i) tot += block_sums[i];
    loss[0] = tot / (float)p.B;
  }
}

__global__ void vocab_sample_finalize_kernel(CeArgs p, int64_t* tokens, int64_t tok_stride) {
  const int n = blockIdx.x * blockDim.x + threadIdx.x;
  if (n >= p.N || (p.skip_flag && *p.skip_flag)) return;
  float av = -INFINITY;
  int ai = 0x7fffffff;
  for (int sp = 0; sp < p.nsplit; ++sp) {
    const float q = p.part[((int64_t)sp * p.N + n) * 4 + 3];
    const int qi = p.part_idx[(int64_t)sp * p.N + n];
    if (q > av || (q == av && qi < ai)) { av = q; ai = qi; }
  }
  tokens[(int64_t)n * tok_stride] = ai;
}

struct PArgs {
  const float* h; int64_t ldh;
  const float* w; const float* bias;
  const int64_t* targets; int64_t tgt_stride_b;
  const int64_t* lengths;
  const float* lse;
  const float* grad_scale;
  int N, B, H, V, v0, vc;
  float* P; int64_t ldp;
};

__global__ void __launch_bounds__(GCE::NT) vocab_p_kernel(PArgs p) {
  __shared__ __align__(16) float smem[GCE::SMEM_FLOATS];
  const int m0 = blockIdx.y * GCE::BM, n0 = p.v0 + blockIdx.x * GCE::BN;
  const int ty = threadIdx.x / GCE::TX, tx = threadIdx.x % GCE::TX;
  float acc[GCE::TM][GCE::TN];
#pragma unroll
  for (int i = 0; i < GCE::TM; ++i)
#pragma unroll
    for (int j = 0; j < GCE::TN; ++j) acc[i][j] = 0.f;
  GCE::run(p.h, p.ldh, m0, p.N, p.w, p.H, n0, min(p.V, p.v0 + p.vc), 0, p.H, p.H, smem, acc);
  const float gs = (p.grad_scale ? p.grad_scale[0] : 1.f) / (float)p.B;
#pragma unroll
  for (int i = 0; i < GCE::TM; ++i) {
    int n = m0 + GCE::row_of(ty, i);
    if (n >= p.N) continue;
    int b = n % p.B, tpos = n / p.B + 1;
    float scale = (tpos < p.lengths[b]) ? gs : 0.f;
    int tgt = (int)p.targets[(int64_t)b * p.tgt_stride_b + tpos];
    float l = p.lse[n];
#pragma unroll
    for (int j = 0; j < GCE::TN; ++j) {
      int v = n0 + GCE::col_of(tx, j);
      if (v >= p.V || v >= p.v0 + p.vc) continue;
      float pr = scale == 0.f ? 0.f : (expf(acc[i][j] + p.bias[v] - l) - (v == tgt ? 1.f : 0.f)) * scale;
      p.P[(int64_t)n * p.ldp + (v - p.v0)] = pr;
    }
  }
}

static int ce_partials(CeArgs& p, cudaStream_t st) {
  if (!force_simt_gemm() && p.N >= 64 && p.V >= 128 && p.H >= 32 && tc16::supported(p.h, p.ldh, 0, p.w, p.H, 0, p.N, p.V, p.H)) {
    const int launched = p.nsplit;
    p.nsplit = (p.h_planes && p.w_planes ? 4 : 2) * launched;
    p.part_idx = reinterpret_cast<int*>(p.part + (int64_t)p.nsplit * p.N * 4);
    return tc16::ce_partials(p.h, p.ldh, p.N, p.B, p.H, p.V, p.w, p.bias, p.targets, p.tgt_stride_b, p.lengths,
                             p.tiles_per_split, launched, p.part, p.part_idx, p.gumbel_seed, p.gumbel_salt, p.h_planes,
                             p.w_planes, p.skip_flag, st);
  }
  if (!force_simt_gemm() && p.N >= 64 && p.V >= 128 && p.H >= 32 && tc::tc_linear_supported(p.h, p.ldh, p.w, p.H, p.N, p.V, p.H))
    return tc::tc_ce_partials(p.h, p.ldh, p.N, p.B, p.H, p.V, p.w, p.bias, p.targets, p.tgt_stride_b, p.lengths,
                              p.tiles_per_split, p.nsplit, p.part, p.part_idx, p.gumbel_seed, p.gumbel_salt, st);
  dim3 grid(ceil_div(p.N, GCE::BM), p.nsplit);
  vocab_ce_fwd_kernel<<<grid, GCE::NT, 0, st>>>(p);
  DVAE_LAUNCH_CHECK();
  return DVAE_OK;
}

static int ce_nsplit(int N, int V, int* tiles_per_split) {
  int row_tiles = ceil_div(N, GCE::BM), vtiles = ceil_div(V, GCE::BN);
  int want = 148 / row_tiles;
  if (want < 1) want = 1;
  if (want > vtiles) want = vtiles;
  int tps = ceil_div(vtiles, want);
  *tiles_per_split = tps;
  return ceil_div(vtiles, tps);
}

static int p_chunk(int N, int V) {
  int64_t vmax = (14LL << 20) / (N > 0 ? N : 1);
  vmax = vmax / 128 * 128;
  if (vmax < 128) vmax = 128;
  const int64_t vr = (int64_t)ceil_div(V, 128) * 128;
  if (vmax >= vr) return (int)vr;
  const int64_t nc = (vr + vmax - 1) / vmax;
  const int64_t vc = ((V + nc - 1) / nc + 127) / 128 * 128;
  return (int)vc;
}

static int p_chunk_planes(int N, int V) {
  static const int64_t budget = [] {
    const char* e = getenv("DVAE_VOCAB_PCHUNK_M");
    return (int64_t)(e ? atoi(e) : 512) << 20;
  }();
  int64_t vmax = budget / (N > 0 ? N : 1);
  vmax = vmax / 128 * 128;
  if (vmax < 128) vmax = 128;
  const int64_t vr = (int64_t)ceil_div(V, 128) * 128;
  if (vmax >= vr) return (int)vr;
  const int64_t nc = (vr + vmax - 1) / vmax;
  return (int)(((V + nc - 1) / nc + 127) / 128 * 128);
}
static bool p_planes_enabled() {
  const char* e = getenv("DVAE_VOCAB_PPLANES");
  return !(e && e[0] == '0');
}

}

using namespace dvae;

static int64_t ce_part_floats(int N, int V) {
  int tps;
  int ns = ce_nsplit(N, V, &tps);
  return (4LL * ns * N * 5 + 8 + kFinMaxBlocks + 3) / 4 * 4;
}
extern "C" int64_t dvae_vocab_ce_ws_floats(int N, int V, int H) {
  return ce_part_floats(N, V) + tc16::plane_floats(N, H) + tc16::plane_floats(V, H);
}

static thread_local const void* g_wsplit_ws = nullptr;
static thread_local const void* g_wsplit_w = nullptr;

extern "C" int dvae_vocab_split_w(const float* w, int N, int V, int H, float* ws, void* stream) {
  DVAE_REQUIRE(w && ws && N > 0 && V > 0 && H > 0, "dvae_vocab_split_w: bad argument");
  g_wsplit_ws = g_wsplit_w = nullptr;
  if (force_simt_gemm() || !tc16::enabled() || !use_presplit(N, V, H) || (reinterpret_cast<uintptr_t>(w) & 15)) return DVAE_OK;
  float* wp = ws + ce_part_floats(N, V) + tc16::plane_floats(N, H);
  int rc = tc16::split_planes(w, H, V, H, 1.f, wp, (cudaStream_t)stream);
  if (rc) return rc;
  g_wsplit_ws = ws; g_wsplit_w = w;
  return DVAE_OK;
}

static int vocab_ce_fwd_impl(const float* h, int64_t ldh, int T1, int B, int H, int V, const float* w,
                             const float* bias, const int64_t* targets, int64_t tgt_stride_b,
                             const int64_t* lengths, int sos, float* lse, float* nll, int32_t* argmax,
                             float* loss, float* ws, bool w_planes_ready, void* stream) {
  cudaStream_t st = (cudaStream_t)stream;
  DVAE_REQUIRE(h && w && bias && targets && lengths && loss && ws, "dvae_vocab_ce_fwd: null pointer");
  DVAE_REQUIRE(T1 > 0 && B > 0 && H > 0 && V > 0, "dvae_vocab_ce_fwd: bad shape T1=%d B=%d H=%d V=%d", T1, B, H, V);
  CeArgs p;
  p.h = h; p.ldh = ldh; p.w = w; p.bias = bias; p.targets = targets; p.tgt_stride_b = tgt_stride_b;
  p.lengths = lengths; p.N = T1 * B; p.B = B; p.H = H; p.V = V; p.sos = sos;
  p.nsplit = ce_nsplit(p.N, V, &p.tiles_per_split);
  p.part = ws;
  p.part_idx = reinterpret_cast<int*>(ws + (int64_t)p.nsplit * p.N * 4);
  p.gumbel_seed = nullptr; p.gumbel_salt = 0;
  p.h_planes = p.w_planes = nullptr; p.skip_flag = nullptr;
  if (use_tc16(p.N, V, H, h, ldh, w) && use_presplit(p.N, V, H)) {
    float* hp = ws + ce_part_floats(p.N, V);
    float* wp = hp + tc16::plane_floats(p.N, H);
    int rc;
    if ((rc = tc16::split_planes(h, ldh, p.N, H, 1.f, hp, st))) return rc;
    if (!(w_planes_ready && g_wsplit_ws == ws && g_wsplit_w == w) && (rc = tc16::split_planes(w, H, V, H, 1.f, wp, st))) return rc;
    p.h_planes = hp; p.w_planes = wp;
  }
  g_wsplit_ws = g_wsplit_w = nullptr;
  { int rc = ce_partials(p, st); if (rc) return rc; }
  float* block_sums = ws + (int64_t)p.nsplit * p.N * 5 + 8;
  const int nblk = min(kFinMaxBlocks, ceil_div(p.N, kFinThreads / kFinLanes));
  vocab_ce_finalize_kernel<<<nblk, kFinThreads, 0, st>>>(p, lse, nll, argmax, block_sums);
  DVAE_LAUNCH_CHECK();
  vocab_ce_loss_kernel<<<1, 128, 0, st>>>(p, block_sums, nblk, loss);
  DVAE_LAUNCH_CHECK();
  return DVAE_OK;
}

extern "C" int dvae_vocab_ce_fwd(const float* h, int64_t ldh, int T1, int B, int H, int V, const float* w,
                                 const float* bias, const int64_t* targets, int64_t tgt_stride_b,
                                 const int64_t* lengths, int sos, float* lse, float* nll, int32_t* argmax,
                                 float* loss, float* ws, void* stream) {
  return vocab_ce_fwd_impl(h, ldh, T1, B, H, V, w, bias, targets, tgt_stride_b, lengths, sos, lse, nll, argmax, loss, ws,
                           false, stream);
}

extern "C" int dvae_vocab_ce_fwd_ex(const float* h, int64_t ldh, int T1, int B, int H, int V, const float* w,
                                    const float* bias, const int64_t* targets, int64_t tgt_stride_b,
                                    const int64_t* lengths, int sos, float* lse, float* nll, int32_t* argmax,
                                    float* loss, float* ws, int flags, void* stream) {
  return vocab_ce_fwd_impl(h, ldh, T1, B, H, V, w, bias, targets, tgt_stride_b, lengths, sos, lse, nll, argmax, loss, ws,
                           (flags & 1) != 0, stream);
}

static int p_buffers(int N, int V) { return p_chunk(N, V) < V ? 2 : 1; }

static int p_buffers_planes(int N, int V) { return p_chunk_planes(N, V) < V ? 2 : 1; }
static int64_t p_region_floats(int N, int V) {
  const int64_t a = (int64_t)p_buffers(N, V) * N * p_chunk(N, V);
  const int vcp = p_chunk_planes(N, V);
  const int64_t b = (int64_t)p_buffers_planes(N, V) * (tc16::plane_floats(N, vcp) + tc16::plane_floats(vcp, N));
  return (a > b ? a : b) + 4;
}
extern "C" int64_t dvae_vocab_ce_bwd_ws_floats(int N, int V, int H) {
  return p_region_floats(N, V) / 4 * 4 + tc16::plane_floats(N, H) + tc16::plane_floats(V, H) + tc16::plane_floats(H, V) +
         tc16::plane_floats(H, N);
}

extern "C" int dvae_vocab_ce_bwd(const float* h, int64_t ldh, int T1, int B, int H, int V, const float* w,
                                 const float* bias, const int64_t* targets, int64_t tgt_stride_b,
                                 const int64_t* lengths, const float* lse, const float* grad_scale_dev,
                                 float* d_h, int64_t lddh, float* d_w, float* d_bias, const float* fwd_ws, float* ws,
                                 void* stream) {
  cudaStream_t st = (cudaStream_t)stream;
  DVAE_REQUIRE(h && w && bias && targets && lengths && lse && d_h && d_w && d_bias && ws, "dvae_vocab_ce_bwd: null pointer");
  DVAE_REQUIRE(T1 > 0 && B > 0 && H > 0 && V > 0, "dvae_vocab_ce_bwd: bad shape");
  const int N = T1 * B;
  int vc_max = p_chunk(N, V), nbuf = p_buffers(N, V);
  const int64_t front = p_region_floats(N, V) / 4 * 4;
  PArgs p;
  p.h = h; p.ldh = ldh; p.w = w; p.bias = bias; p.targets = targets; p.tgt_stride_b = tgt_stride_b;
  p.lengths = lengths; p.lse = lse; p.grad_scale = grad_scale_dev; p.N = N; p.B = B; p.H = H; p.V = V;
  p.P = ws; p.ldp = vc_max;
  GemmHints ph;
  ph.a_scale = 1.f;
  while (ph.a_scale * 2.f <= (float)B) ph.a_scale *= 2.f;
  const void *h_planes = nullptr, *w_planes = nullptr;
  if (use_tc16(N, min(vc_max, V), H, h, ldh, w) && use_presplit(N, V, H)) {
    if (fwd_ws) {
      const float* hp = fwd_ws + ce_part_floats(N, V);
      h_planes = hp; w_planes = hp + tc16::plane_floats(N, H);
    } else {
      float* hp = ws + front;
      float* wp = hp + tc16::plane_floats(N, H);
      int rc;
      if ((rc = tc16::split_planes(h, ldh, N, H, 1.f, hp, st))) return rc;
      if ((rc = tc16::split_planes(w, H, V, H, 1.f, wp, st))) return rc;
      h_planes = hp; w_planes = wp;
    }
  }
  const void *wT_planes = nullptr, *hT_planes = nullptr;
  int wT_kbtot = 0;
  if (h_planes && H % 32 == 0 && N >= 128 && (reinterpret_cast<uintptr_t>(w) & 15) == 0 && ldh == H &&
      !(getenv("DVAE_VOCAB_TPLANES") && getenv("DVAE_VOCAB_TPLANES")[0] == '0')) {
    float* tp = ws + front + tc16::plane_floats(N, H) + tc16::plane_floats(V, H);
    tc16::PlaneHit hit;
    tc16::PlaneTable tab;
    tab.n = 0;
    if (tc16::find_weight_planes(w, H, 1, H, V, &hit) && hit.tile0 == 0 && hit.kb0 == 0) {
      wT_planes = hit.planes; wT_kbtot = hit.kbtot;
    } else {
      tab.e[tab.n++] = tc16::PlaneTable::Entry{w, V, H, nullptr, tp};
      wT_planes = tp; wT_kbtot = ceil_div(V, 32);
    }
    float* hp_t = tp + tc16::plane_floats(H, V);
    tab.e[tab.n++] = tc16::PlaneTable::Entry{h, N, H, nullptr, hp_t};
    hT_planes = hp_t;
    int rc = tc16::weight_planes_launch(tab, st);
    if (rc) return rc;
  }
  const bool pp = wT_planes && hT_planes && h_planes && w_planes && p_planes_enabled() && lddh % 4 == 0 &&
                  tc16::supported(h, ldh, 0, w, H, 0, N, min(vc_max, V), H);
  int64_t pa_fl = 0, pt_fl = 0;
  if (pp) {
    vc_max = p_chunk_planes(N, V); nbuf = p_buffers_planes(N, V);
    pa_fl = tc16::plane_floats(N, vc_max); pt_fl = tc16::plane_floats(vc_max, N);
    DVAE_CUDA(cudaMemsetAsync(d_bias, 0, sizeof(float) * V, st));
  }
  int chunk = 0;
  const int nchunks = ceil_div(V, vc_max);
  for (int v0 = 0; v0 < V; v0 += vc_max, ++chunk) {
    const int vc = min(vc_max, V - v0);
    float* Pc = ws + (int64_t)(chunk % nbuf) * N * vc_max;
    p.v0 = v0; p.vc = vc; p.P = Pc;
    int rc;
    bool dh_zeroed = false, dw_zeroed = false;
    if (pp) {
      float* pa = ws + (int64_t)(chunk % nbuf) * (pa_fl + pt_fl);
      float* pt = pa + pa_fl;
      const bool zh = chunk == 0 && lddh == H && (((uintptr_t)d_h) & 15) == 0 && ((int64_t)N * H) % 4 == 0;
      const bool zw = (((uintptr_t)(d_w + (int64_t)v0 * H)) & 15) == 0 && ((int64_t)vc * H) % 4 == 0;
      if ((rc = tc16::softmax_grad(h, ldh, N, B, H, V, v0, vc, w, bias, targets, tgt_stride_b, lengths, lse, grad_scale_dev, nullptr,
                                   vc_max, h_planes, w_planes, zh ? d_h : nullptr, (int64_t)N * H / 4,
                                   zw ? d_w + (int64_t)v0 * H : nullptr, (int64_t)vc * H / 4, st, pa, pt, d_bias + v0, ph.a_scale))) return rc;
      Fork fork(st);
      if ((rc = tc16::linear_planes(pa, wT_planes, d_h, lddh, N, H, vc, nullptr, chunk ? 1.f : 0.f, 0, ph.a_scale, 1.f, nullptr, zh, 16, st,
                                    v0 / 32, wT_kbtot))) return rc;
      static const int dw_cap = [] { const char* e = getenv("DVAE_VOCAB_DW_MAX_CTAS"); return e ? atoi(e) : 0; }();
      if ((rc = tc16::linear_planes(pt, hT_planes, d_w + (int64_t)v0 * H, H, vc, H, N, nullptr, 0.f, 0, ph.a_scale, 1.f, nullptr, zw, 16,
                                    fork.side(0), 0, 0, dw_cap))) return rc;
      if (chunk + 1 == nchunks || chunk + 1 >= nbuf)
        if ((rc = fork.join())) return rc;
      continue;
    }
    if (!force_simt_gemm() && N >= 64 && vc >= 128 && H >= 32 && tc16::supported(h, ldh, 0, w, H, 0, N, vc, H)) {
      const bool zh = chunk == 0 && lddh == H && (((uintptr_t)d_h) & 15) == 0 && ((int64_t)N * H) % 4 == 0;
      const bool zw = (((uintptr_t)(d_w + (int64_t)v0 * H)) & 15) == 0 && ((int64_t)vc * H) % 4 == 0;
      if ((rc = tc16::softmax_grad(h, ldh, N, B, H, V, v0, vc, w, bias, targets, tgt_stride_b, lengths, lse, grad_scale_dev, Pc,
                                   vc_max, h_planes, w_planes, zh ? d_h : nullptr, (int64_t)N * H / 4,
                                   zw ? d_w + (int64_t)v0 * H : nullptr, (int64_t)vc * H / 4, st))) return rc;
      dh_zeroed = zh; dw_zeroed = zw;
    } else if (!force_simt_gemm() && N >= 64 && vc >= 128 && H >= 32 && tc::tc_linear_supported(h, ldh, w, H, N, vc, H)) {
      if ((rc = tc::tc_softmax_grad(h, ldh, N, B, H, v0, vc, w, bias, targets, tgt_stride_b, lengths, lse, grad_scale_dev, Pc,
                                    vc_max, st))) return rc;
    } else {
      dim3 grid(ceil_div(vc, GCE::BN), ceil_div(N, GCE::BM));
      vocab_p_kernel<<<grid, GCE::NT, 0, st>>>(p);
      DVAE_LAUNCH_CHECK();
    }
    Fork fork(st);
    GemmHints ph_h = ph, ph_w = ph;
    ph_h.c_zeroed = dh_zeroed; ph_w.c_zeroed = dw_zeroed;
    if (wT_planes) { ph_h.b_planes = wT_planes; ph_h.b_tile0 = 0; ph_h.b_kb0 = v0 / 32; ph_h.b_kbtot = wT_kbtot; }
    if (hT_planes) { ph_w.b_planes = hT_planes; ph_w.b_tile0 = 0; ph_w.b_kb0 = 0; ph_w.b_kbtot = ceil_div(N, 32); }
    if ((rc = linear_impl_ex(Pc, vc_max, 0, w + (int64_t)v0 * H, H, 1, d_h, lddh, N, H, vc, nullptr, nullptr, chunk ? 1.f : 0.f, 0, ph_h, st))) return rc;
    if ((rc = linear_impl_ex(Pc, vc_max, 1, h, ldh, 1, d_w + (int64_t)v0 * H, H, vc, H, N, nullptr, nullptr, 0.f, 0, ph_w, fork.side(0)))) return rc;
    if ((rc = colsum_impl(Pc, vc_max, N, vc, d_bias + v0, 0.f, fork.side(1)))) return rc;
    if (chunk + 1 == nchunks || chunk + 1 >= nbuf)
      if ((rc = fork.join())) return rc;
  }
  return DVAE_OK;
}

extern "C" int dvae_vocab_ce_partials(const float* h, int64_t ldh, int T1, int B, int H, int V, const float* w,
                                      const float* bias, const int64_t* targets, int64_t tgt_stride_b,
                                      const int64_t* lengths, int sos, float* ws, void* stream) {
  DVAE_REQUIRE(h && w && bias && targets && lengths && ws, "dvae_vocab_ce_partials: null pointer");
  DVAE_REQUIRE(T1 > 0 && B > 0 && H > 0 && V > 0, "dvae_vocab_ce_partials: bad shape");
  CeArgs p;
  p.h = h; p.ldh = ldh; p.w = w; p.bias = bias; p.targets = targets; p.tgt_stride_b = tgt_stride_b;
  p.lengths = lengths; p.N = T1 * B; p.B = B; p.H = H; p.V = V; p.sos = sos;
  p.nsplit = ce_nsplit(p.N, V, &p.tiles_per_split);
  p.part = ws;
  p.part_idx = reinterpret_cast<int*>(ws + (int64_t)p.nsplit * p.N * 4);
  p.gumbel_seed = nullptr; p.gumbel_salt = 0;
  p.h_planes = p.w_planes = nullptr; p.skip_flag = nullptr;
  if (use_tc16(p.N, V, H, h, ldh, w) && use_presplit(p.N, V, H)) {
    float* hp = ws + ce_part_floats(p.N, V);
    p.h_planes = hp; p.w_planes = hp + tc16::plane_floats(p.N, H);
  }
  return ce_partials(p, (cudaStream_t)stream);
}

static int vocab_sample_step_impl(const float* h, int64_t ldh, int B, int H, int V, const float* w, const float* bias,
                                  const uint64_t* seed_dev, uint32_t salt, int64_t* tokens_out, int64_t tok_stride,
                                  const int32_t* forced_flag_dev, const float* w_planes, float* ws, void* stream) {
  cudaStream_t st = (cudaStream_t)stream;
  DVAE_REQUIRE(h && w && bias && seed_dev && tokens_out && ws, "dvae_vocab_sample_step: null pointer");
  DVAE_REQUIRE(B > 0 && H > 0 && V > 0, "dvae_vocab_sample_step: bad shape");
  CeArgs p;
  p.h = h; p.ldh = ldh; p.w = w; p.bias = bias; p.targets = nullptr; p.tgt_stride_b = 0; p.lengths = nullptr;
  p.N = B; p.B = B; p.H = H; p.V = V; p.sos = 0;
  p.nsplit = ce_nsplit(p.N, V, &p.tiles_per_split);
  p.part = ws;
  p.part_idx = reinterpret_cast<int*>(ws + (int64_t)p.nsplit * p.N * 4);
  p.gumbel_seed = seed_dev; p.gumbel_salt = salt;
  p.h_planes = p.w_planes = nullptr;
  p.skip_flag = forced_flag_dev;
  if (w_planes && use_tc16(B, V, H, h, ldh, w) && use_presplit(B, V, H)) {
    float* hp = ws + ce_part_floats(B, V);
    int rc2 = tc16::split_planes(h, ldh, B, H, 1.f, hp, st);
    if (rc2) return rc2;
    p.h_planes = hp; p.w_planes = w_planes;
  }
  int rc = ce_partials(p, st);
  if (rc) return rc;
  vocab_sample_finalize_kernel<<<ceil_div(B, 128), 128, 0, st>>>(p, tokens_out, tok_stride);
  DVAE_LAUNCH_CHECK();
  return DVAE_OK;
}

extern "C" int dvae_vocab_sample_step(const float* h, int64_t ldh, int B, int H, int V, const float* w, const float* bias,
                                      const uint64_t* seed_dev, uint32_t salt, int64_t* tokens_out, int64_t tok_stride,
                                      float* ws, void* stream) {
  return vocab_sample_step_impl(h, ldh, B, H, V, w, bias, seed_dev, salt, tokens_out, tok_stride, nullptr, nullptr, ws, stream);
}

extern "C" int dvae_vocab_sample_step_ex(const float* h, int64_t ldh, int B, int H, int V, const float* w, const float* bias,
                                         const uint64_t* seed_dev, uint32_t salt, int64_t* tokens_out, int64_t tok_stride,
                                         const int32_t* forced_flag_dev, float* ws, void* stream) {
  return vocab_sample_step_impl(h, ldh, B, H, V, w, bias, seed_dev, salt, tokens_out, tok_stride, forced_flag_dev, nullptr, ws, stream);
}

extern "C" int64_t dvae_vocab_w_planes_floats(int V, int H) { return tc16::plane_floats(V, H); }

extern "C" int dvae_vocab_w_planes(const float* w, int V, int H, float* planes, void* stream) {
  DVAE_REQUIRE(w && planes && V > 0 && H > 0, "dvae_vocab_w_planes: bad argument");
  return tc16::split_planes(w, H, V, H, 1.f, planes, (cudaStream_t)stream);
}

extern "C" int dvae_vocab_sample_step_planes(const float* h, int64_t ldh, int B, int H, int V, const float* w, const float* bias,
                                             const float* w_planes, const uint64_t* seed_dev, uint32_t salt, int64_t* tokens_out,
                                             int64_t tok_stride, const int32_t* forced_flag_dev, float* ws, void* stream) {
  return vocab_sample_step_impl(h, ldh, B, H, V, w, bias, seed_dev, salt, tokens_out, tok_stride, forced_flag_dev, w_planes, ws, stream);
}
```

disentanglement-vae_b200/engine.py:

```python
import os
import random

import torch
import torch.distributed as dist

from . import _lib
from ._lib import ptr, check
from .plan import StepPlan
from .losses import get_cyclic_kl_weight


def d_bow(plan):
    return bool(plan.d.bow)


class TrainEngine:
    NSLOT = max(3, int(os.environ.get("DVAE_ENGINE_SLOTS", "4")))

    def __init__(self, model, params, B, T, lr=None, total_steps=None, use_graph=True, max_norm=5.0,
                 process_group=None, seed=None, teacher_forcing_prob=None):
        model._require_cuda()
        self.model, self.params, self.B, self.T = model, params, B, T
        self.lib = _lib.load()
        self.device = model._flat.device
        self.plan = StepPlan(model, B, T, self.device)
        self.d = d = self.plan.d
        self.world = dist.get_world_size(process_group) if (dist.is_available() and dist.is_initialized()) else 1
        self.rank = dist.get_rank(process_group) if self.world > 1 else 0
        self.pg = process_group
        self.max_norm = max_norm
        self.lr = float(params["learn_rate"] if lr is None else lr)
        self.total_steps = total_steps
        self.lambdas = params["lambdas"]
        if total_steps is None and any(v == "cyclic" for v in self.lambdas.values()):
            raise ValueError("a \"cyclic\" lambda needs total_steps (= epochs * len(dataloader), run.py:215-216)")
        self.tf_prob = float(params.get("teacher_forcing_prob", 1.0) if teacher_forcing_prob is None else teacher_forcing_prob)
        self.sampled = self.tf_prob < 1.0
        self.aux = bool(len(model.adversaries) or len(model.mi_estimators))
        if self.aux and self.world > 1:
            raise NotImplementedError("adversarial_loss / mi_loss models train on one GPU through the engine (their private "
                                      "optimizers are not all-reduced)")
        self.n = model._flat_numel
        f32 = dict(device=self.device, dtype=torch.float32)
        self.flat = model._flat[:self.n]
        self.use_graph = use_graph
        self._nvls = None
        if self.world > 1 and use_graph and not self.aux and os.environ.get("DVAE_DP_NVLS", "1") != "0":
            self._setup_nvls()
        if self._nvls is None:
            self.grad = torch.zeros(self.n, **f32)
        self.m = torch.zeros(self.n, **f32)
        self.v = torch.zeros(self.n, **f32)
        self.G = model.grad_views(self.grad)
        named = dict(model.named_parameters())
        for n in model._layout:
            named[n].grad = self.G[n]
        self.n_dsc = max(sum(1 for o in d.dsc_out if o > 0), 1)
        self.hyper = torch.zeros(8, **f32)
        self.kl_w = torch.zeros(max(d.S, 1), **f32)
        self.sumsq = torch.zeros(1, **f32)
        self.red_ws = torch.zeros(1032, **f32)
        T1 = max(T - 1, 1)
        lay, off = {}, 0
        for name, nbytes in (("inputs", B * T * 8), ("lengths", B * 8), ("seed", 8), ("labels", self.n_dsc * B * 4),
                             ("scal", (8 + max(d.S, 1)) * 4), ("coins", T1 * 4)):
            lay[name] = (off, nbytes)
            off = (off + nbytes + 15) // 16 * 16
        self._stage_bytes, self._stage_lay = off, lay
        self.d_stage = torch.zeros(off, device=self.device, dtype=torch.uint8)

        def view(buf, name, dtype, *shape):
            o, n = lay[name]
            return buf[o:o + n].view(dtype).view(*shape)
        self.inputs = view(self.d_stage, "inputs", torch.int64, B, T)
        self.lengths = view(self.d_stage, "lengths", torch.int64, B)
        self.labels = view(self.d_stage, "labels", torch.float32, self.n_dsc, B)
        self.d_scal = view(self.d_stage, "scal", torch.float32, 8 + max(d.S, 1))
        self.coins = view(self.d_stage, "coins", torch.int32, T1)
        self.coins.fill_(1)
        self.plan.seed_dev = view(self.d_stage, "seed", torch.int64, 1)
        self.preds = torch.zeros(B, T, device=self.device, dtype=torch.int64) if self.sampled else None
        ns = self.NSLOT
        self.h_stage = torch.zeros(ns, off, dtype=torch.uint8).pin_memory()
        self.h_outs = torch.zeros(ns, self.plan.out.numel(), dtype=torch.float32).pin_memory()
        self._hv = [{k: view(self.h_stage[i], k, dt, *shp).numpy() for k, dt, shp in
                     (("inputs", torch.int64, (B, T)), ("lengths", torch.int64, (B,)), ("seed", torch.int64, (1,)),
                      ("labels", torch.float32, (self.n_dsc, B)), ("scal", torch.float32, (8 + max(d.S, 1),)),
                      ("coins", torch.int32, (T1,)))} for i in range(ns)]
        for hv in self._hv:
            hv["coins"][:] = 1
            hv["lengths"][:] = 1
        self.h_out = self.h_outs[0]
        self._slot_ev = [None] * ns
        self._slot = -1
        self.step_idx = 0
        self.adam_step = 0
        base = int(params.get("random_seed", 10)) if seed is None else int(seed)
        if seed is None:
            base += 7919 * self.rank
        self._gen = torch.Generator().manual_seed(base)
        self._pyrand = random.Random(base)
        self._eval_gen = torch.Generator().manual_seed(base + 0x5EED)
        self._eval_pyrand = random.Random(base + 0x5EED)
        self._eval = None
        self.use_graph = use_graph and not self.aux
        self._graphs = None
        self._buckets = None
        self._comm = None
        self._xchg_in_capture = False
        self._dp_ctr = torch.zeros(1, dtype=torch.int32, device=self.device)
        self._side = None
        self.label_names = [n for n, o in zip(d.space_names, d.dsc_out) if o > 0]
        self.last_aux = {}
        self.fixed_eps = None
        self._wplanes, self._plane_token = [], object()
        if os.environ.get("DVAE_WEIGHT_PLANES", "1") != "0" and not d.bow:
            self._alloc_weight_planes()

    def _alloc_weight_planes(self):
        lib, P = self.lib, self.model._P
        names = [n for n in P if (".recurrent.weight_ih_" in n)]
        todo = [(n, True, True) for n in names] + [("decoder.linear.weight", False, True)]
        for n, normal, transposed in todo:
            w = P[n]
            R, C = w.shape
            if R * C < (1 << 14) or (w.data_ptr() & 15):
                continue
            mk = lambda tr: torch.empty(lib.dvae_weight_planes_floats(R, C, tr), device=self.device, dtype=torch.float32)
            self._wplanes.append((w, mk(0) if normal else None, mk(1) if transposed else None))

    def _register_weight_planes(self):
        if not self._wplanes or _lib.planes_owner is self._plane_token:
            return
        check(self.lib.dvae_weight_planes_clear(), "dvae_weight_planes_clear")
        for w, pl, plt in self._wplanes:
            check(self.lib.dvae_weight_planes_register(ptr(w), w.size(0), w.size(1), ptr(pl), ptr(plt)), "dvae_weight_planes_register")
        _lib.planes_owner = self._plane_token

    def _forward(self, fork_ok=True, train=True, sampled=None, preds=None):
        pl, P, m = self.plan, self.model._P, self.model
        sampled = self.sampled if sampled is None else sampled
        preds = self.preds if preds is None else preds
        n_pl = len(self._wplanes)
        n_ih = sum(1 for w, a, b in self._wplanes if a is not None)
        if n_pl:
            check(self.lib.dvae_weight_planes_refresh_ex(0, n_ih, _lib.stream_ptr()), "dvae_weight_planes_refresh")
        self.hyper[:5].copy_(self.d_scal[:5])
        self.kl_w.copy_(self.d_scal[8:8 + self.kl_w.numel()])
        if self.fixed_eps is not None:
            pl.eps.copy_(self.fixed_eps)
        else:
            pl.randn_eps()
        cur = torch.cuda.current_stream()
        hoist = fork_ok and os.environ.get("DVAE_HOIST", "1") != "0" and not d_bow(pl) and not sampled
        refresh_wt = n_pl > n_ih and train
        fork_prep = None
        if hoist:
            if self._side is None:
                self._side = torch.cuda.Stream(device=self.device)

            def fork_prep():
                self._side.wait_stream(cur)
                with torch.cuda.stream(self._side):
                    pl.decode_prepare(P, self.inputs, m.sos_token_idx, train)
                    if refresh_wt:
                        check(self.lib.dvae_weight_planes_refresh_ex(n_ih, n_pl - n_ih, _lib.stream_ptr()), "dvae_weight_planes_refresh")
        if refresh_wt and not hoist:
            check(self.lib.dvae_weight_planes_refresh_ex(n_ih, n_pl - n_ih, _lib.stream_ptr()), "dvae_weight_planes_refresh")
        pl.encode(P, self.inputs, self.lengths, train, after_l0_proj=fork_prep)
        pl.heads(P, pl.ctx, pl.eps, self.labels, self.kl_w)
        if hoist:
            cur.wait_stream(self._side)
        if sampled:
            preds.copy_(self.inputs)
            preds[:, 0].fill_(m.sos_token_idx)
            h_top = pl.decode_sampled(P, preds, self.coins, train)
        else:
            h_top = pl.decode_forced(P, self.inputs, m.sos_token_idx, train)
        pl.vocab_ce(P, h_top, self.inputs, self.lengths)
        return h_top, hoist

    def _fwd_bwd(self, part=None, g_z=None):
        pl, P, G, m = self.plan, self.model._P, self.G, self.model
        st = _lib.stream_ptr()
        cur = torch.cuda.current_stream()
        xchg = self._xchg_in_capture and part is None
        if xchg:
            check(self.lib.dvae_counter_increment(ptr(self._dp_ctr), st), "dvae_counter_increment")
        if part == 0 or part is None or (part == 1 and not self._three_buckets()):
            h_top, hoist = self._forward()
            if callable(g_z):
                g_z = g_z()
            self._g_z = g_z
            self._g_top = pl.vocab_ce_bwd(P, G, h_top, self.inputs, self.lengths, None)
            self._hoist = hoist
            if part == 0:
                check(self.lib.dvae_join_side_streams(st), "dvae_join_side_streams")
                return
            if xchg:
                self._signal(0, True)
        if part in (None, 1):
            g_top, hoist = self._g_top, self._hoist
            check(self.lib.dvae_defer_joins(1), "dvae_defer_joins")
            try:
                pl.decode_bwd(P, G, g_top, emb_grad="decoder.embedding.weight" in m._layout,
                              aux_stream=self._side if hoist else None)
            finally:
                if part == 1:
                    check(self.lib.dvae_join_side_streams(st), "dvae_join_side_streams")
                    if hoist:
                        cur.wait_stream(self._side)
            self._aux_pending = hoist and part is None
            if xchg:
                self._signal(1, True, self._side if hoist else None)
        emb_enc = "encoder.embedding.weight" in m._layout
        if part in (None, 2):
            check(self.lib.dvae_defer_joins(1), "dvae_defer_joins")
            try:
                g_ctx = pl.heads_bwd(P, G, pl.ctx, pl.eps, self.labels, self.kl_w, pl.g_hid, g_z=getattr(self, "_g_z", None))
                if getattr(self, "_aux_pending", False):
                    torch.cuda.current_stream().wait_stream(self._side)
                    self._aux_pending = False
                self._g_ctx = g_ctx
                split = part == 2 and self._three_buckets()
                if xchg:
                    pl.encode_bwd(P, G, self.inputs, self.lengths, g_ctx, emb_grad=emb_enc, layers=(pl.d.Le - 1, 1))
                    self._signal(2, True)
                    pl.encode_bwd(P, G, self.inputs, self.lengths, g_ctx, emb_grad=emb_enc, layers=(0, 0))
                    self._signal(3, True)
                else:
                    pl.encode_bwd(P, G, self.inputs, self.lengths, g_ctx, emb_grad=emb_enc, layers=(pl.d.Le - 1, 1) if split else None)
            finally:
                check(self.lib.dvae_join_side_streams(st), "dvae_join_side_streams")
        if part == 3:
            check(self.lib.dvae_defer_joins(1), "dvae_defer_joins")
            try:
                pl.encode_bwd(P, G, self.inputs, self.lengths, self._g_ctx, emb_grad=emb_enc, layers=(0, 0))
            finally:
                check(self.lib.dvae_join_side_streams(st), "dvae_join_side_streams")

    def _setup_nvls(self):
        import sys
        import ctypes as C

        def agreed(ok, why, phase):
            flag = torch.tensor([1 if ok else 0], dtype=torch.int32, device=self.device)
            torch.cuda.synchronize()
            dist.all_reduce(flag, op=dist.ReduceOp.MIN, group=self.pg)
            if int(flag.item()) == 1:
                return True
            print(f"[dvae_b200] rank {self.rank}: in-graph gradient exchange unavailable ({phase}: {why or 'another rank failed'}); "
                  "using NCCL all-reduce between stage graphs", file=sys.stderr, flush=True)
            return False

        mode = "p2p" if self.world == 2 else "nvls"
        n_pad = (self.n + 3) // 4 * 4
        ok, why, st = True, "", {}
        try:
            import torch.distributed._symmetric_memory as symm
            grp = self.pg if self.pg is not None else dist.group.WORLD
            buf = symm.empty(n_pad, dtype=torch.float32, device=self.device)
            hb = symm.rendezvous(buf, group=grp)
            bar = symm.empty(int(self.lib.dvae_nvls_barrier_words()), dtype=torch.int32, device=self.device)
            bar.zero_()
            hbar = symm.rendezvous(bar, group=grp)
            if mode != "p2p" and not hb.multicast_ptr:
                raise RuntimeError("no multicast address (NVSwitch multicast unavailable)")
            buf.fill_(float(self.rank + 1))
            st = dict(buf=buf, bar=bar, hb=hb, hbar=hbar, mc=int(hb.multicast_ptr), mode=mode,
                      bar_ptrs=(C.c_void_p * self.world)(*[int(p) for p in hbar.buffer_ptrs]),
                      buf_ptrs=[int(p) for p in hb.buffer_ptrs])
        except Exception as e:
            ok, why = False, repr(e)[:200]
        if not agreed(ok, why, "symmetric memory"):
            return
        try:
            one = torch.ones(1, dtype=torch.int32, device=self.device)
            err = torch.zeros(1, dtype=torch.int32, device=self.device)
            if mode == "p2p":
                peers = (C.c_void_p * self.world)(*st["buf_ptrs"])
                check(self.lib.dvae_p2p_all_reduce(peers, n_pad, st["bar_ptrs"], self.rank, self.world, ptr(one), 1, 0, 0,
                                                   5_000_000_000, ptr(err), _lib.stream_ptr()), "dvae_p2p_all_reduce")
            else:
                check(self.lib.dvae_nvls_all_reduce(st["mc"], n_pad, st["bar_ptrs"], self.rank, self.world, ptr(one), 1, 0, 0,
                                                    5_000_000_000, ptr(err), _lib.stream_ptr()), "dvae_nvls_all_reduce")
            torch.cuda.synchronize()
            want = float(self.world * (self.world + 1) // 2)
            if int(err.item()) != 0 or not bool((st["buf"] == want).all()):
                raise RuntimeError("timeout or wrong sums")
        except Exception as e:
            ok, why = False, repr(e)[:200]
        if not agreed(ok, why, "self-test"):
            return
        st["buf"].zero_()
        if not agreed(True, "", "zero"):
            return
        self.grad = st["buf"][:self.n]
        self._nvls = st

    XCHG_CTAS = (16, 16, 32, 64)

    def _signal(self, k, include_sides, extra=None):
        import ctypes as C
        out = C.c_void_p()
        check(self.lib.dvae_fork_after(1 if include_sides else 0, extra.cuda_stream if extra is not None else None,
                                       _lib.stream_ptr(), C.byref(out)), "dvae_fork_after")
        nv = self._nvls
        ctas = self.XCHG_CTAS[k]
        for j, v in enumerate(self._buckets[k]):
            off = v.data_ptr() - nv["buf"].data_ptr()
            n = (v.numel() + 3) // 4 * 4
            if nv["mode"] == "p2p":
                peers = (C.c_void_p * self.world)(*[bp + off for bp in nv["buf_ptrs"]])
                check(self.lib.dvae_p2p_all_reduce(peers, n, nv["bar_ptrs"], self.rank, self.world, ptr(self._dp_ctr),
                                                   16, 2 * k + j + 1, ctas, 0, None, out.value), "dvae_p2p_all_reduce")
            else:
                check(self.lib.dvae_nvls_all_reduce(nv["mc"] + off, n, nv["bar_ptrs"], self.rank, self.world, ptr(self._dp_ctr),
                                                    16, 2 * k + j + 1, ctas, 0, None, out.value), "dvae_nvls_all_reduce")

    def _one_graph_dp(self):
        return self._nvls is not None and self.use_graph and self._three_buckets()

    @property
    def exchange_mode(self):
        if self.world == 1:
            return "none"
        return self._nvls["mode"] if self._one_graph_dp() else "nccl+stages"

# ... 446 lines not shown
```

disentanglement-vae_b200/plan.py:

```python
import torch

from . import _lib
from ._lib import ptr, ptr_array, int_array, check

SALT_ENC_EMB, SALT_DEC_EMB, SALT_ENC_LAYER, SALT_DEC_LAYER, SALT_EPS, SALT_SAMPLE = 1, 3, 16, 32, 64, 4096


class Dims:

    def __init__(self, model):
        enc, dec = model.encoder, model.decoder
        self.V, self.E = enc.embedding.weight.shape
        self.H = enc.hidden_size
        self.Hd = dec.hidden_size
        self.bow = not hasattr(enc, "recurrent")
        self.D = enc.num_directions
        self.Le = 0 if not hasattr(enc, "recurrent") else enc.num_layers
        self.Ld = dec.num_layers
        self.C = self.H * enc.num_layers * self.D
        self.space_names = list(model.context2params.keys())
        self.space_dims = [model.context2params[n].out_features // 2 for n in self.space_names]
        self.S = len(self.space_names)
        self.Z = sum(self.space_dims)
        self.dsc_out = [model.discriminators[n].output_dim if n in model.discriminators else 0
                        for n in self.space_names]
        self.OD = sum(self.dsc_out)
        self.H2L = 2 * self.Hd * self.Ld
        self.sos, self.eos = model.sos_token_idx, model.eos_token_idx
        self.p_enc, self.p_dec = float(enc.dropout_rate), float(dec.dropout_rate)
        assert self.S <= _lib.MAX_SPACES, f"at most {_lib.MAX_SPACES} latent spaces"


class StepPlan:
    def __init__(self, model, B, T, device):
        self.lib = _lib.load()
        self.d = d = Dims(model)
        self.B, self.T, self.T1 = B, T, T - 1
        self.N = self.T1 * B
        self.device = device
        self.busy = False
        f32 = dict(device=device, dtype=torch.float32)
        H, D, E = d.H, d.D, d.E

        def buf(*shape):
            return torch.empty(*shape, **f32)

        self.x_enc = buf(T, B, E)
        self.e_gates = [buf(D, T, B, 4 * H) for _ in range(d.Le)]
        self.e_cs = [buf(D, T, B, H) for _ in range(d.Le)]
        self.e_hs = [buf(T, B, D * H) for _ in range(d.Le)]
        self.e_xin = [None] + [buf(T, B, D * H) for _ in range(1, d.Le)]
        self.ctx = buf(B, d.C)
        self.ctx_c = buf(B, d.C)
        self.eps = buf(B, d.Z)
        self.z, self.mu, self.logvar = buf(B, d.Z), buf(B, d.Z), buf(B, d.Z)
        self.hid = buf(B, d.H2L)
        self.dsc_logits = buf(B, max(d.OD, 1))
        self.out = torch.zeros(_lib.HEADS_NSCALARS + 5, **f32)
        self.scalars = self.out[:_lib.HEADS_NSCALARS]
        self.heads_ws = torch.zeros(self.lib.dvae_heads_ws_floats(B, d.S), **f32)
        T1 = max(self.T1, 1)
        self.x_dec = buf(T1, B, E)
        Hd = d.Hd
        self.d_gates = [buf(1, T1, B, 4 * Hd) for _ in range(d.Ld)]
        self.d_cs = [buf(1, T1, B, Hd) for _ in range(d.Ld)]
        self.d_hs = [buf(T1, B, Hd) for _ in range(d.Ld)]
        self.d_xin = [None] + [buf(T1, B, Hd) for _ in range(1, d.Ld)]
        self.state_ws = buf(self.lib.dvae_lstm_state_ws_floats(B, max(H, Hd), D))
        self.bow_argmax = torch.zeros(B, E, device=device, dtype=torch.int32) if d.bow else None
        self.lse, self.nll = buf(max(self.N, 1)), buf(max(self.N, 1))
        self.argmax = torch.zeros(max(self.N, 1), device=device, dtype=torch.int32)
        self.recon = self.out[_lib.HEADS_NSCALARS:_lib.HEADS_NSCALARS + 1]
        self.ce_ws = buf(self.lib.dvae_vocab_ce_ws_floats(max(self.N, 1), d.V, d.Hd))
        self.sample_ws = None
        self._bwd_ready = False
        self.seed_dev = torch.zeros(1, device=device, dtype=torch.int64)
        self.labels = buf(max(sum(1 for o in d.dsc_out if o > 0), 1), B)
        self._space_dims = int_array(d.space_dims)
        self._dsc_out = int_array(d.dsc_out)
        self.train_mode = False

    def _alloc_bwd(self):
        if self._bwd_ready:
            return
        d, B, T, T1 = self.d, self.B, self.T, max(self.T1, 1)
        f32 = dict(device=self.device, dtype=torch.float32)
        w = max(d.E, d.H * d.D, d.Hd)
        self.g_top = torch.empty(T1, B, d.Hd, **f32)
        self.g_dx = [torch.empty(max(T, T1), B, w, **f32) for _ in range(2)]
        self.g_hid = torch.empty(B, d.H2L, **f32)
        self.g_ctx = torch.empty(B, d.C, **f32)
        self.heads_bwd_ws = torch.empty(self.lib.dvae_heads_bwd_ws_floats(B, d.Z, d.H2L), **f32)
        self.ce_bwd_ws = torch.empty(self.lib.dvae_vocab_ce_bwd_ws_floats(max(self.N, 1), d.V, d.Hd), **f32)
        need = [self.lib.dvae_lstm_bwd_planes_ws_floats(T1, B, d.E if l == 0 else d.Hd, d.Hd, 1) for l in range(d.Ld)]
        need += [self.lib.dvae_lstm_bwd_planes_ws_floats(T, B, d.E if l == 0 else d.D * d.H, d.H, d.D) for l in range(d.Le)]
        self.lstm_bwd_planes = torch.empty(max(need), **f32)
        self._bwd_ready = True

    @staticmethod
    def _enc_w(P, l, dirs):
        sfx = [f"_l{l}" + ("_reverse" if k else "") for k in range(dirs)]
        return tuple([P[f"encoder.recurrent.{n}{s}"] for s in sfx] for n in ("weight_ih", "weight_hh", "bias_ih", "bias_hh"))

    @staticmethod
    def _dec_w(P, l):
        return tuple([P[f"decoder.recurrent.{n}_l{l}"]] for n in ("weight_ih", "weight_hh", "bias_ih", "bias_hh"))

    def encode(self, P, inputs, lengths, train, after_l0_proj=None):
        lib, d, st = self.lib, self.d, _lib.stream_ptr()
        B, T = self.B, self.T
        p = d.p_enc if train else 0.0
        if d.bow:
            check(lib.dvae_bow_encoder_fwd(ptr(P["encoder.embedding.weight"]), d.E, ptr(inputs), inputs.stride(0),
                                           inputs.stride(1), T, B, p, ptr(self.seed_dev), SALT_ENC_EMB, ptr(self.ctx), d.C,
                                           ptr(self.bow_argmax), st), "dvae_bow_encoder_fwd")
            self._enc_p = p
            return self.ctx
        check(lib.dvae_embedding_fwd(ptr(P["encoder.embedding.weight"]), d.E, ptr(inputs), inputs.stride(0),
                                     inputs.stride(1), T, B, p, ptr(self.seed_dev), SALT_ENC_EMB, -1, 0,
                                     ptr(self.x_enc), st), "dvae_embedding_fwd")
        x, I = self.x_enc, d.E
        for l in range(d.Le):
            if l > 0:
                I = d.D * d.H
                if p > 0.0:
                    check(lib.dvae_dropout(ptr(self.e_hs[l - 1]), I, T * B, I, p, ptr(self.seed_dev),
                                           SALT_ENC_LAYER + l, ptr(self.e_xin[l]), I, 0, st), "dvae_dropout")
                    x = self.e_xin[l]
                else:
                    x = self.e_hs[l - 1]
            w_ih, w_hh, b_ih, b_hh = self._enc_w(P, l, d.D)
            off = l * d.D * d.H
            split = l == 0 and after_l0_proj is not None
            if split:
                check(lib.dvae_lstm_input_proj(ptr(x), I, T, B, I, d.H, d.D, ptr_array(w_ih), ptr_array(b_ih),
                                               ptr_array(b_hh), ptr(self.e_gates[l]), st), "dvae_lstm_input_proj(enc)")
                after_l0_proj()
            check(lib.dvae_lstm_seq_fwd_ex(ptr(x), I, T, B, I, d.H, d.D, ptr_array(w_ih), ptr_array(w_hh),
                                           ptr_array(b_ih), ptr_array(b_hh), None, None, 0, 0, ptr(lengths),
                                           ptr(self.e_hs[l]), d.D * d.H, self.ctx.data_ptr() + 4 * off,
                                           self.ctx_c.data_ptr() + 4 * off, d.C, d.H, ptr(self.e_gates[l]),
                                           ptr(self.e_cs[l]), ptr(self.state_ws), 1 if split else 0, st),
                  "dvae_lstm_seq_fwd(enc)")
        self._enc_p = p
        return self.ctx

    def heads(self, P, ctx, eps, labels, kl_w):
        lib, d, st = self.lib, self.d, _lib.stream_ptr()
        check(lib.dvae_latent_heads_fwd(ptr(ctx), self.B, d.C, d.S, self._space_dims, self._dsc_out,
                                        ptr(P["_c2p.weight"]), ptr(P["_c2p.bias"]), ptr(eps),
                                        ptr(P.get("_dsc.weight")), ptr(P.get("_dsc.bias")), ptr(labels), ptr(kl_w),
                                        ptr(P["z2hidden.weight"]), ptr(P["z2hidden.bias"]), d.H2L, ptr(self.z),
                                        ptr(self.mu), ptr(self.logvar), ptr(self.hid), ptr(self.dsc_logits),
                                        ptr(self.scalars), ptr(self.heads_ws), st), "dvae_latent_heads_fwd")

    def decode_forced(self, P, tokens, first_token, train, hid=None):
        lib, d, st = self.lib, self.d, _lib.stream_ptr()
        B, T1 = self.B, self.T1
        hid = self.hid if hid is None else hid
        p = d.p_dec if train else 0.0
        prepared = getattr(self, "_dec_prepared", None) == (tokens.data_ptr(), first_token, p)
        self._dec_prepared = None
        if not prepared:
            check(lib.dvae_embedding_fwd(ptr(P["decoder.embedding.weight"]), d.E, ptr(tokens), tokens.stride(0),
                                         tokens.stride(1), T1, B, p, ptr(self.seed_dev), SALT_DEC_EMB, first_token, 0,
                                         ptr(self.x_dec), st), "dvae_embedding_fwd")
        x, I = self.x_dec, d.E
        for l in range(d.Ld):
            if l > 0:
                I = d.Hd
                if p > 0.0:
                    check(lib.dvae_dropout(ptr(self.d_hs[l - 1]), I, T1 * B, I, p, ptr(self.seed_dev),
                                           SALT_DEC_LAYER + l, ptr(self.d_xin[l]), I, 0, st), "dvae_dropout")
                    x = self.d_xin[l]
                else:
                    x = self.d_hs[l - 1]
            w_ih, w_hh, b_ih, b_hh = self._dec_w(P, l)
            check(lib.dvae_lstm_seq_fwd_ex(ptr(x), I, T1, B, I, d.Hd, 1, ptr_array(w_ih), ptr_array(w_hh),
                                           ptr_array(b_ih), ptr_array(b_hh), hid.data_ptr() + 4 * l * d.Hd,
                                           hid.data_ptr() + 4 * (d.Ld + l) * d.Hd, d.H2L, 0, None, ptr(self.d_hs[l]),
                                           d.Hd, None, None, 0, 0, ptr(self.d_gates[l]), ptr(self.d_cs[l]),
                                           ptr(self.state_ws), 1 if (prepared and l == 0) else 0, st),
                  "dvae_lstm_seq_fwd(dec)")
        self._dec_p = p
        self._dec_tokens, self._dec_first = tokens, first_token
        self._dec_hid = hid
        return self.d_hs[-1]

    def decode_prepare(self, P, tokens, first_token, train):
        lib, d, st = self.lib, self.d, _lib.stream_ptr()
        B, T1 = self.B, self.T1
        p = d.p_dec if train else 0.0
        check(lib.dvae_embedding_fwd(ptr(P["decoder.embedding.weight"]), d.E, ptr(tokens), tokens.stride(0),
                                     tokens.stride(1), T1, B, p, ptr(self.seed_dev), SALT_DEC_EMB, first_token, 0,
                                     ptr(self.x_dec), st), "dvae_embedding_fwd")
        w_ih, _, b_ih, b_hh = self._dec_w(P, 0)
        check(lib.dvae_lstm_input_proj(ptr(self.x_dec), d.E, T1, B, d.E, d.Hd, 1, ptr_array(w_ih), ptr_array(b_ih),
                                       ptr_array(b_hh), ptr(self.d_gates[0]), st), "dvae_lstm_input_proj(dec)")
        self._dec_prepared = (tokens.data_ptr(), first_token, p)
        check(lib.dvae_vocab_split_w(ptr(P["decoder.linear.weight"]), max(self.N, 1), d.V, d.Hd, ptr(self.ce_ws), st),
              "dvae_vocab_split_w")
        self._w_planes_ready = P["decoder.linear.weight"].data_ptr()

    def decode_sampled(self, P, preds, coins, train, hid=None):
        lib, d, st = self.lib, self.d, _lib.stream_ptr()
        B, T1 = self.B, self.T1
        hid = self.hid if hid is None else hid
        p = d.p_dec if train else 0.0
        if self.sample_ws is None:
            self.sample_ws = torch.empty(lib.dvae_vocab_ce_ws_floats(B, d.V, d.Hd), device=self.device, dtype=torch.float32)
        emb = P["decoder.embedding.weight"]
        W = [self._dec_w(P, l) for l in range(d.Ld)]
        dev_coins = torch.is_tensor(coins)
        if dev_coins:
            assert coins.dtype == torch.int32 and coins.is_cuda and coins.numel() >= T1
        w_planes = None
        if B >= 256 and d.V >= 1024 and d.Hd % 32 == 0:
            if getattr(self, "w_out_planes", None) is None:
                self.w_out_planes = torch.empty(lib.dvae_vocab_w_planes_floats(d.V, d.Hd), device=self.device, dtype=torch.float32)
            w_planes = self.w_out_planes
            check(lib.dvae_vocab_w_planes(ptr(P["decoder.linear.weight"]), d.V, d.Hd, ptr(w_planes), st), "dvae_vocab_w_planes")
        for s in range(T1):
            check(lib.dvae_embedding_fwd(ptr(emb), d.E, ptr(preds), preds.stride(0), preds.stride(1), 1, B, p,
                                         ptr(self.seed_dev), SALT_DEC_EMB, d.sos, s, ptr(self.x_dec), st),
                  "dvae_embedding_fwd(step)")
            x, I = self.x_dec, d.E
            for l in range(d.Ld):
                if l > 0:
                    I = d.Hd
                    if p > 0.0:
                        check(lib.dvae_dropout(ptr(self.d_hs[l - 1]), I, B, I, p, ptr(self.seed_dev),
                                               SALT_DEC_LAYER + l, ptr(self.d_xin[l]), I, s * B, st), "dvae_dropout(step)")
                        x = self.d_xin[l]
                    else:
                        x = self.d_hs[l - 1]
                w_ih, w_hh, b_ih, b_hh = W[l]
                check(lib.dvae_lstm_step(ptr(x), I, s, T1, B, I, d.Hd, ptr(w_ih[0]), ptr(w_hh[0]), ptr(b_ih[0]),
                                         ptr(b_hh[0]), hid.data_ptr() + 4 * l * d.Hd,
                                         hid.data_ptr() + 4 * (d.Ld + l) * d.Hd, d.H2L, ptr(self.d_hs[l]),
                                         ptr(self.d_gates[l]), ptr(self.d_cs[l]), ptr(self.state_ws), st),
                      "dvae_lstm_step")
            if dev_coins or not coins[s]:
                h_s = self.d_hs[-1].data_ptr() + 4 * s * B * d.Hd
                flag = coins.data_ptr() + 4 * s if dev_coins else None
                check(lib.dvae_vocab_sample_step_planes(h_s, d.Hd, B, d.Hd, d.V, ptr(P["decoder.linear.weight"]),
                                                        ptr(P["decoder.linear.bias"]), ptr(w_planes), ptr(self.seed_dev),
                                                        SALT_SAMPLE + s, preds.data_ptr() + 8 * (s + 1) * preds.stride(1),
                                                        preds.stride(0), flag, ptr(self.sample_ws), st), "dvae_vocab_sample_step")
        self._dec_p = p
        self._dec_tokens, self._dec_first = preds, d.sos
        self._dec_hid = hid
        return self.d_hs[-1]

    def vocab_ce(self, P, h_top, targets, lengths):
        lib, d, st = self.lib, self.d, _lib.stream_ptr()
        w_ready = getattr(self, "_w_planes_ready", None) == P["decoder.linear.weight"].data_ptr()
        self._w_planes_ready = None
        check(lib.dvae_vocab_ce_fwd_ex(ptr(h_top), d.Hd, self.T1, self.B, d.Hd, d.V, ptr(P["decoder.linear.weight"]),
                                       ptr(P["decoder.linear.bias"]), ptr(targets), targets.stride(0), ptr(lengths),
                                       d.sos, ptr(self.lse), ptr(self.nll), ptr(self.argmax), ptr(self.recon),
                                       ptr(self.ce_ws), 1 if w_ready else 0, st), "dvae_vocab_ce_fwd")
        self._ce_planes_valid = (h_top.data_ptr(), P["decoder.linear.weight"].data_ptr())
        return self.recon

    def vocab_ce_bwd(self, P, G, h_top, targets, lengths, grad_scale_dev):
        self._alloc_bwd()
        lib, d, st = self.lib, self.d, _lib.stream_ptr()
        reuse = getattr(self, "_ce_planes_valid", None) == (h_top.data_ptr(), P["decoder.linear.weight"].data_ptr())
        self._ce_planes_valid = None
        check(lib.dvae_vocab_ce_bwd(ptr(h_top), d.Hd, self.T1, self.B, d.Hd, d.V, ptr(P["decoder.linear.weight"]),
                                    ptr(P["decoder.linear.bias"]), ptr(targets), targets.stride(0), ptr(lengths),
                                    ptr(self.lse), ptr(grad_scale_dev), ptr(self.g_top), d.Hd,
                                    ptr(G["decoder.linear.weight"]), ptr(G["decoder.linear.bias"]),
                                    ptr(self.ce_ws) if reuse else None, ptr(self.ce_bwd_ws), st),
              "dvae_vocab_ce_bwd")
        return self.g_top

    def decode_bwd(self, P, G, g_top, emb_grad=True, aux_stream=None):
        self._alloc_bwd()
        lib, d, st = self.lib, self.d, _lib.stream_ptr()
        B, T1 = self.B, self.T1
        hid = self._dec_hid
        g_in, p = g_top, self._dec_p
        for l in range(d.Ld - 1, -1, -1):
            I = d.E if l == 0 else d.Hd
            x = self.x_dec if l == 0 else (self.d_xin[l] if p > 0.0 else self.d_hs[l - 1])
            g_out = self.g_dx[l % 2]
            w_ih, w_hh, _, _ = self._dec_w(P, l)
            gw_ih, gw_hh, gb_ih, gb_hh = self._dec_w(G, l)
            need_dx = l > 0 or emb_grad
            check(lib.dvae_lstm_seq_bwd_ex(ptr(x), I, T1, B, I, d.Hd, 1, ptr_array(w_ih), ptr_array(w_hh),
                                        hid.data_ptr() + 4 * l * d.Hd, hid.data_ptr() + 4 * (d.Ld + l) * d.Hd,
                                        d.H2L, 0, None, ptr(self.d_hs[l]), d.Hd, ptr(self.d_gates[l]),
                                        ptr(self.d_cs[l]), ptr(g_in), d.Hd, None, None, 0, 0,
                                        ptr(g_out) if need_dx else None, I, ptr_array(gw_ih), ptr_array(gw_hh),
                                        ptr_array(gb_ih), ptr_array(gb_hh), self.g_hid.data_ptr() + 4 * l * d.Hd,
                                        self.g_hid.data_ptr() + 4 * (d.Ld + l) * d.Hd, d.H2L, 0,
                                        ptr(self.state_ws), ptr(self.lstm_bwd_planes), st), "dvae_lstm_seq_bwd(dec)")
            if l > 0 and p > 0.0:
                check(lib.dvae_dropout(ptr(g_out), I, T1 * B, I, p, ptr(self.seed_dev), SALT_DEC_LAYER + l,
                                       ptr(g_out), I, 0, st), "dvae_dropout(bwd)")
            g_in = g_out
        if emb_grad:
            tok = self._dec_tokens
            if aux_stream is not None:
                aux_stream.wait_stream(torch.cuda.current_stream())
                st = aux_stream.cuda_stream
            check(lib.dvae_embedding_bwd(ptr(g_in), d.E, ptr(tok), tok.stride(0), tok.stride(1), T1, B, p,
                                         ptr(self.seed_dev), SALT_DEC_EMB, self._dec_first, 0,
                                         ptr(G["decoder.embedding.weight"]), st), "dvae_embedding_bwd")
        return self.g_hid

    def heads_bwd(self, P, G, ctx, eps, labels, kl_w, g_hid, g_z=None, g_mu=None, g_logvar=None, g_logits=None):
        self._alloc_bwd()
        lib, d, st = self.lib, self.d, _lib.stream_ptr()
        check(lib.dvae_latent_heads_bwd(ptr(ctx), self.B, d.C, d.S, self._space_dims, self._dsc_out,
                                        ptr(P["_c2p.weight"]), ptr(eps), ptr(P.get("_dsc.weight")), ptr(labels),
                                        ptr(kl_w), ptr(P["z2hidden.weight"]), d.H2L, ptr(self.z), ptr(self.mu),
                                        ptr(self.logvar), ptr(self.hid), ptr(self.dsc_logits), ptr(g_hid),
                                        ptr(g_z), ptr(g_mu), ptr(g_logvar), ptr(g_logits), ptr(G["_c2p.weight"]),
                                        ptr(G["_c2p.bias"]), ptr(G.get("_dsc.weight")), ptr(G.get("_dsc.bias")),
                                        ptr(G["z2hidden.weight"]), ptr(G["z2hidden.bias"]), ptr(self.g_ctx),
                                        ptr(self.heads_bwd_ws), st), "dvae_latent_heads_bwd")
        return self.g_ctx

    def encode_bwd(self, P, G, inputs, lengths, g_ctx, emb_grad=True, layers=None):
        self._alloc_bwd()
        lib, d, st = self.lib, self.d, _lib.stream_ptr()
        B, T = self.B, self.T
        p = self._enc_p
        if d.bow:
            if emb_grad:
                check(lib.dvae_bow_encoder_bwd(ptr(g_ctx), d.C, ptr(self.bow_argmax), d.E, ptr(inputs), inputs.stride(0),
                                               inputs.stride(1), T, B, p, ptr(self.seed_dev), SALT_ENC_EMB,
                                               ptr(G["encoder.embedding.weight"]), st), "dvae_bow_encoder_bwd")
            return
        first, last = (d.Le - 1, 0) if layers is None else layers
        g_in = None if first == d.Le - 1 else self._enc_g_in
        for l in range(first, last - 1, -1):
            I = d.E if l == 0 else d.D * d.H
            x = self.x_enc if l == 0 else (self.e_xin[l] if p > 0.0 else self.e_hs[l - 1])
            g_out = self.g_dx[l % 2]
            w_ih, w_hh, _, _ = self._enc_w(P, l, d.D)
            gw_ih, gw_hh, gb_ih, gb_hh = self._enc_w(G, l, d.D)
            need_dx = l > 0 or emb_grad
            off = l * d.D * d.H
            check(lib.dvae_lstm_seq_bwd_ex(ptr(x), I, T, B, I, d.H, d.D, ptr_array(w_ih), ptr_array(w_hh), None, None,
                                        0, 0, ptr(lengths), ptr(self.e_hs[l]), d.D * d.H, ptr(self.e_gates[l]),
                                        ptr(self.e_cs[l]), ptr(g_in), d.D * d.H, g_ctx.data_ptr() + 4 * off, None,
                                        d.C, d.H, ptr(g_out) if need_dx else None, I, ptr_array(gw_ih),
                                        ptr_array(gw_hh), ptr_array(gb_ih), ptr_array(gb_hh), None, None, 0, 0,
                                        ptr(self.state_ws), ptr(self.lstm_bwd_planes), st), "dvae_lstm_seq_bwd(enc)")
            if l > 0 and p > 0.0:
                check(lib.dvae_dropout(ptr(g_out), I, T * B, I, p, ptr(self.seed_dev), SALT_ENC_LAYER + l,
                                       ptr(g_out), I, 0, st), "dvae_dropout(bwd)")
            g_in = g_out
        self._enc_g_in = g_in
        if emb_grad and last == 0:
            check(lib.dvae_embedding_bwd(ptr(g_in), d.E, ptr(inputs), inputs.stride(0), inputs.stride(1), T, B, p,
                                         ptr(self.seed_dev), SALT_ENC_EMB, -1, 0, ptr(G["encoder.embedding.weight"]),
                                         st), "dvae_embedding_bwd")

    def randn_eps(self, salt_offset=0):
        check(self.lib.dvae_randn(ptr(self.eps), self.eps.numel(), ptr(self.seed_dev), SALT_EPS + salt_offset,
                                  _lib.stream_ptr()), "dvae_randn")
        return self.eps

    def recount_lengths(self, tokens, lengths_out, eos, pad=0, min_len=1):
        check(self.lib.dvae_recount_lengths(ptr(tokens), tokens.stride(0), tokens.stride(1), tokens.size(0), tokens.size(1),
                                            eos, pad, min_len, ptr(lengths_out), _lib.stream_ptr()), "dvae_recount_lengths")
        return lengths_out
```

include/dvae_b200.h:

```cpp
#ifndef DVAE_B200_H_
#define DVAE_B200_H_

#include <stdint.h>

#ifdef __cplusplus
extern "C" {
#endif

#define DVAE_OK 0
#define DVAE_EINVAL (-1)
#define DVAE_ECUDA (-2)
#define DVAE_EWORKSPACE (-3)

#define DVAE_MAX_SPACES 8

const char* dvae_last_error_string(void);
int dvae_version(void);
int64_t dvae_launch_count(void);

int dvae_linear(const float* A, int64_t lda, int trans_a, const float* B, int64_t ldb, int trans_b,
                float* C, int64_t ldc, int M, int N, int K, const float* bias, const float* bias2,
                float beta, int act, void* stream);

int dvae_tc_linear(const float* A, int64_t lda, int trans_a, const float* B, int64_t ldb, int trans_b,
                   float* C, int64_t ldc, int M, int N, int K, const float* bias, const float* bias2,
                   float beta, int act, int passes, void* stream);

int dvae_tc16_linear(const float* A, int64_t lda, int trans_a, const float* B, int64_t ldb, int trans_b,
                     float* C, int64_t ldc, int M, int N, int K, const float* bias, const float* bias2,
                     float beta, int act, float a_scale, float b_scale, const uint32_t* a_amax_bits,
                     const uint32_t* b_amax_bits, void* stream);

int dvae_entropy_loss(const float* logits, int B, int O, float* loss, const float* g_loss, float* d_logits,
                      void* stream);
int dvae_club_mi(const float* mu, const float* logvar, const float* y, int B, int D, float* mi,
                 const float* g_mi, float* d_mu, float* d_logvar, float* d_y, float* ws, void* stream);
int dvae_club_nll(const float* mu, const float* logvar, const float* y, int B, int D, float* loss,
                  const float* g_loss, float* d_mu, float* d_logvar, void* stream);
int dvae_act_bwd(const float* y, const float* g, float* d, int64_t n, int act, void* stream);
int dvae_relu(float* x, int64_t n, void* stream);

int64_t dvae_weight_planes_floats(int R, int C, int transposed);
int dvae_weight_planes_register(const float* w, int R, int C, void* planes, void* planes_t);
int dvae_weight_planes_refresh(void* stream);
int dvae_weight_planes_refresh_ex(int first, int count, void* stream);
int dvae_weight_planes_enable(int on);
int dvae_weight_planes_clear(void);

int dvae_defer_joins(int on);
int dvae_join_side_streams(void* stream);

int dvae_counter_increment(uint32_t* counter, void* stream);
int dvae_fork_after(int include_sides, void* extra_stream, void* stream, void** forked_stream_out);

int64_t dvae_nvls_barrier_words(void);
int dvae_p2p_all_reduce(float* const* peer_ptrs_host, int64_t n, uint32_t* const* barrier_ptrs_host, int rank, int world,
                        const uint32_t* counter_dev, uint32_t epoch_mul, uint32_t epoch_add, int ctas,
                        uint64_t soft_timeout_ns, uint32_t* err_dev, void* stream);
int dvae_nvls_all_reduce(float* mc_ptr, int64_t n, uint32_t* const* barrier_ptrs_host, int rank, int world,
                         const uint32_t* counter_dev, uint32_t epoch_mul, uint32_t epoch_add, int ctas,
                         uint64_t soft_timeout_ns, uint32_t* err_dev, void* stream);

int dvae_colsum(const float* X, int64_t ldx, int M, int N, float* out, float beta, void* stream);

int dvae_randn(float* out, int64_t n, const uint64_t* seed_dev, uint32_t salt, void* stream);
int dvae_embedding_fwd(const float* emb, int E, const int64_t* tokens, int64_t tok_stride_b,
                       int64_t tok_stride_t, int T, int B, float p, const uint64_t* seed_dev,
                       uint32_t salt, int64_t first_token, int t0, float* x, void* stream);
int dvae_embedding_bwd(const float* d_x, int E, const int64_t* tokens, int64_t tok_stride_b,
                       int64_t tok_stride_t, int T, int B, float p, const uint64_t* seed_dev,
                       uint32_t salt, int64_t first_token, int t0, float* d_emb, void* stream);
int dvae_bow_encoder_fwd(const float* emb, int E, const int64_t* tokens, int64_t tok_stride_b, int64_t tok_stride_t,
                         int T, int B, float p, const uint64_t* seed_dev, uint32_t salt, float* ctx, int64_t ldctx,
                         int32_t* argmax, void* stream);
int dvae_bow_encoder_bwd(const float* d_ctx, int64_t ldd, const int32_t* argmax, int E, const int64_t* tokens,
                         int64_t tok_stride_b, int64_t tok_stride_t, int T, int B, float p, const uint64_t* seed_dev,
                         uint32_t salt, float* d_emb, void* stream);
int dvae_dropout(const float* x, int64_t ldx, int64_t rows, int width, float p,
                 const uint64_t* seed_dev, uint32_t salt, float* y, int64_t ldy, int64_t row0,
                 void* stream);

int64_t dvae_lstm_state_ws_floats(int B, int H, int D);
int dvae_lstm_seq_fwd(const float* x, int64_t ldx, int T, int B, int I, int H, int D,
                      const float* const* w_ih_host, const float* const* w_hh_host,
                      const float* const* b_ih_host, const float* const* b_hh_host,
                      const float* h0, const float* c0, int64_t ld0, int64_t dir0,
                      const int64_t* lengths, float* hs, int64_t ldhs, float* hn, float* cn,
                      int64_t ldn, int64_t dirn, float* gates, float* cs, float* state_ws,
                      void* stream);

int dvae_lstm_step(const float* x, int64_t ldx, int t, int T, int B, int I, int H, const float* w_ih,
                   const float* w_hh, const float* b_ih, const float* b_hh, const float* h0,
                   const float* c0, int64_t ld0, float* hs, float* gates, float* cs, float* state_ws,
                   void* stream);

int dvae_lstm_input_proj(const float* x, int64_t ldx, int T, int B, int I, int H, int D,
                         const float* const* w_ih, const float* const* b_ih, const float* const* b_hh,
                         float* gates, void* stream);
int dvae_lstm_seq_fwd_ex(const float* x, int64_t ldx, int T, int B, int I, int H, int D,
                         const float* const* w_ih, const float* const* w_hh, const float* const* b_ih,
                         const float* const* b_hh, const float* h0, const float* c0, int64_t ld0,
                         int64_t dir0, const int64_t* lengths, float* hs, int64_t ldhs, float* hn,
                         float* cn, int64_t ldn, int64_t dirn, float* gates, float* cs, float* state_ws,
                         int flags, void* stream);

int dvae_lstm_seq_bwd(const float* x, int64_t ldx, int T, int B, int I, int H, int D,
                      const float* const* w_ih_host, const float* const* w_hh_host,
                      const float* h0, const float* c0, int64_t ld0, int64_t dir0,
                      const int64_t* lengths, const float* hs, int64_t ldhs, float* gates,
                      const float* cs, const float* d_hs, int64_t lddhs, const float* d_hn,
                      const float* d_cn, int64_t ldn, int64_t dirn, float* d_x, int64_t lddx,
                      float* const* d_w_ih_host, float* const* d_w_hh_host,
                      float* const* d_b_ih_host, float* const* d_b_hh_host, float* d_h0,
                      float* d_c0, int64_t ldd0, int64_t dird0, float* state_ws, void* stream);

int64_t dvae_lstm_bwd_planes_ws_floats(int T, int B, int I, int H, int D);
int dvae_lstm_seq_bwd_ex(const float* x, int64_t ldx, int T, int B, int I, int H, int D,
                         const float* const* w_ih_host, const float* const* w_hh_host,
                         const float* h0, const float* c0, int64_t ld0, int64_t dir0,
                         const int64_t* lengths, const float* hs, int64_t ldhs, float* gates,
                         const float* cs, const float* d_hs, int64_t lddhs, const float* d_hn,
                         const float* d_cn, int64_t ldn, int64_t dirn, float* d_x, int64_t lddx,
                         float* const* d_w_ih_host, float* const* d_w_hh_host,
                         float* const* d_b_ih_host, float* const* d_b_hh_host, float* d_h0,
                         float* d_c0, int64_t ldd0, int64_t dird0, float* state_ws, float* planes_ws,
                         void* stream);

#define DVAE_HEADS_NSCALARS (3 + 3 * DVAE_MAX_SPACES)
int64_t dvae_heads_ws_floats(int B, int S);
int dvae_latent_heads_fwd(const float* ctx, int B, int C, int S, const int* space_dims_host,
                          const int* dsc_out_host, const float* w_c2p, const float* b_c2p,
                          const float* eps, const float* w_dsc, const float* b_dsc,
                          const float* labels, const float* kl_w_dev, const float* w_z2h,
                          const float* b_z2h, int H2L, float* z, float* mu, float* logvar,
                          float* hid, float* dsc_logits, float* scalars, float* ws, void* stream);

int64_t dvae_heads_bwd_ws_floats(int B, int Z, int H2L);
int dvae_latent_heads_bwd(const float* ctx, int B, int C, int S, const int* space_dims_host,
                          const int* dsc_out_host, const float* w_c2p, const float* eps,
                          const float* w_dsc, const float* labels, const float* kl_w_dev,
                          const float* w_z2h, int H2L, const float* z, const float* mu,
                          const float* logvar, const float* hid, const float* dsc_logits,
                          const float* d_hid, const float* d_z_extra, const float* d_mu_extra,
                          const float* d_logvar_extra, const float* d_logits_extra, float* d_w_c2p,
                          float* d_b_c2p, float* d_w_dsc, float* d_b_dsc, float* d_w_z2h,
                          float* d_b_z2h, float* d_ctx, float* ws, void* stream);

int dvae_dsc_loss(const float* dsc_logits, const float* labels, int B, int S,
                  const int* space_dims_host, const int* dsc_out_host, float* out,
                  const float* d_out, float* d_logits, void* stream);

int64_t dvae_vocab_ce_ws_floats(int N, int V, int H);
int dvae_vocab_ce_fwd(const float* h, int64_t ldh, int T1, int B, int H, int V, const float* w,
                      const float* bias, const int64_t* targets, int64_t tgt_stride_b,
                      const int64_t* lengths, int sos, float* lse, float* nll, int32_t* argmax,
                      float* loss, float* ws, void* stream);

int dvae_vocab_split_w(const float* w, int N, int V, int H, float* ws, void* stream);
int dvae_vocab_ce_fwd_ex(const float* h, int64_t ldh, int T1, int B, int H, int V, const float* w,
                         const float* bias, const int64_t* targets, int64_t tgt_stride_b,
                         const int64_t* lengths, int sos, float* lse, float* nll, int32_t* argmax,
                         float* loss, float* ws, int flags, void* stream);

int dvae_vocab_ce_partials(const float* h, int64_t ldh, int T1, int B, int H, int V, const float* w,
                           const float* bias, const int64_t* targets, int64_t tgt_stride_b,
                           const int64_t* lengths, int sos, float* ws, void* stream);

int dvae_vocab_sample_step(const float* h, int64_t ldh, int B, int H, int V, const float* w,
                           const float* bias, const uint64_t* seed_dev, uint32_t salt, int64_t* tokens_out,
                           int64_t tok_stride, float* ws, void* stream);

int dvae_vocab_sample_step_ex(const float* h, int64_t ldh, int B, int H, int V, const float* w,
                              const float* bias, const uint64_t* seed_dev, uint32_t salt, int64_t* tokens_out,
                              int64_t tok_stride, const int32_t* forced_flag_dev, float* ws, void* stream);

int64_t dvae_vocab_w_planes_floats(int V, int H);
int dvae_vocab_w_planes(const float* w, int V, int H, float* planes, void* stream);
int dvae_vocab_sample_step_planes(const float* h, int64_t ldh, int B, int H, int V, const float* w,
                                  const float* bias, const float* w_planes, const uint64_t* seed_dev, uint32_t salt,
                                  int64_t* tokens_out, int64_t tok_stride, const int32_t* forced_flag_dev, float* ws,
                                  void* stream);

int dvae_recount_lengths(const int64_t* tokens, int64_t tok_stride_b, int64_t tok_stride_t, int B, int T,
                         int64_t eos, int64_t pad, int64_t min_len, int64_t* lengths_out, void* stream);

#define DVAE_BLEU_MAX_T 256
int dvae_bleu_counts(const int64_t* ref, int64_t ref_stride, int T_ref, const int64_t* cand, int64_t cand_stride,
                     int T_cand, int B, int64_t eos, int64_t* counts, void* stream);
int dvae_bleu_score(const int64_t* counts, float* score_out, void* stream);

int64_t dvae_vocab_ce_bwd_ws_floats(int N, int V, int H);
int dvae_vocab_ce_bwd(const float* h, int64_t ldh, int T1, int B, int H, int V, const float* w,
                      const float* bias, const int64_t* targets, int64_t tgt_stride_b,
                      const int64_t* lengths, const float* lse, const float* grad_scale_dev,
                      float* d_h, int64_t lddh, float* d_w, float* d_bias, const float* fwd_ws, float* ws,
                      void* stream);

int dvae_grad_sumsq(const float* g, int64_t n, float* sumsq, float* ws, void* stream);
int dvae_clip_adam(float* p, float* g, float* m, float* v, int64_t n, const float* sumsq,
                   float max_norm, float grad_scale, const float* hyper_dev, int zero_grad,
                   void* stream);

#ifdef __cplusplus
}
#endif
#endif
```

Before: 1.151 million.

## Compute vocab cross-entropy only on live (non-padded) rows via device row map

Adds live-row variants of the vocabulary cross-entropy forward and backward that compact the sequence positions still within their lengths into a row map and a device-side live count. The tensor-core GEMM kernels read the live count and reshape their grid split (row tiles, column groups, K splits), writing scattered results through the row map with atomics. Padded positions past each sequence's length then skip the large vocab projection and softmax-gradient work. The trade-off is extra compaction work, atomic scatter outputs, and early-exiting CTAs when few rows are padded. The engine enables this path by default.

```diff
diff --git a/disentanglement-vae_b200/_lib.py b/disentanglement-vae_b200/_lib.py
--- a/disentanglement-vae_b200/_lib.py
+++ b/disentanglement-vae_b200/_lib.py
@@ -79,8 +79,11 @@
     "dvae_vocab_split_w": (_i, [_p, _i, _i, _i, _p, _p]),
     "dvae_vocab_ce_fwd_ex": (_i, [_p, _l, _i, _i, _i, _i, _p, _p, _p, _l, _p, _i, _p, _p, _p, _p, _p, _i, _p]),
     "dvae_vocab_ce_partials": (_i, [_p, _l, _i, _i, _i, _i, _p, _p, _p, _l, _p, _i, _p, _p]),
+    "dvae_vocab_ce_fwd_live": (_i, [_p, _l, _i, _i, _i, _i, _p, _p, _p, _l, _p, _i, _p, _p, _p, _p, _p, _i, _p]),
+    "dvae_vocab_live_rows_at": (_l, [_i, _i, _i]),
     "dvae_vocab_ce_bwd_ws_floats": (_l, [_i, _i, _i]),
     "dvae_vocab_ce_bwd": (_i, [_p, _l, _i, _i, _i, _i, _p, _p, _p, _l, _p, _p, _p, _p, _l, _p, _p, _p, _p, _p]),
+    "dvae_vocab_ce_bwd_live": (_i, [_p, _l, _i, _i, _i, _i, _p, _p, _p, _l, _p, _p, _p, _p, _l, _p, _p, _p, _p, _p]),
     "dvae_entropy_loss": (_i, [_p, _i, _i, _p, _p, _p, _p]),
     "dvae_club_mi": (_i, [_p, _p, _p, _i, _i, _p, _p, _p, _p, _p, _p, _p]),
     "dvae_club_nll": (_i, [_p, _p, _p, _i, _i, _p, _p, _p, _p, _p]),
diff --git a/disentanglement-vae_b200/csrc/tc_gemm16.cu b/disentanglement-vae_b200/csrc/tc_gemm16.cu
--- a/disentanglement-vae_b200/csrc/tc_gemm16.cu
+++ b/disentanglement-vae_b200/csrc/tc_gemm16.cu
@@ -28,7 +28,6 @@
 constexpr int AS_MAX_KB = 8, AS_KB_PER_STAGE = DVAE_AS_KB, AS_STAGE_BYTES = AS_KB_PER_STAGE * PS_TILE;
 constexpr int AS_STAGES = 12 / AS_KB_PER_STAGE, AS_STAGES_NOSCRATCH = 14 / AS_KB_PER_STAGE;
 constexpr uint32_t AS_T_AHI = 256, AS_T_ALO = 384;
-constexpr float kSingleScale = 256.f;
 constexpr int OFF_SCRATCH = STAGES * STAGE_BYTES;
 constexpr int OFF_BIAS = OFF_SCRATCH + EPI_SCRATCH_BYTES;
 constexpr int OFF_BAR = OFF_BIAS + 8 * 64 * 4;
@@ -217,13 +216,43 @@
       for (int64_t i = blk * NUM_THREADS + tid; i < p.zero2_n4; i += nblk * NUM_THREADS) y4[i] = make_float4(0.f, 0.f, 0.f, 0.f);
     }
   }
-  const int m0 = blockIdx.x * BM;
-  const int nt0 = blockIdx.y * p.tiles_per_cta;
   const int n_tiles = (p.N + BN - 1) / BN;
-  const int nt1 = min(n_tiles, nt0 + p.tiles_per_cta);
   const int nkb_total = (p.K + BK - 1) / BK;
-  const int kb0 = blockIdx.z * p.kb_per_split;
-  const int nkb = max(0, min(nkb_total, kb0 + p.kb_per_split) - kb0);
+  int bx = blockIdx.x, by = blockIdx.y, bz = blockIdx.z, M = p.M, tpc = p.tiles_per_cta, kbps = p.kb_per_split;
+  int kb_end = nkb_total;
+  int64_t mstride = p.M;
+  if (p.m_live) {
+    const int live = *p.m_live;
+    if (p.live_k) {
+      kb_end = (live + BK - 1) / BK;
+      kbps = (kb_end + (int)gridDim.z - 1) / (int)gridDim.z;
+      if (bz * kbps >= kb_end) return;
+    } else {
+      M = live;
+      const int rt = (M + BM - 1) / BM;
+      const int ctas = gridDim.x * gridDim.y * gridDim.z, c = (blockIdx.z * gridDim.y + blockIdx.y) * gridDim.x + blockIdx.x;
+      if (rt == 0) return;
+      if (p.mode != 0) {
+        int groups;
+        live_split(rt, ctas, n_tiles, &tpc, &groups);
+        if (c >= rt * groups) return;
+        bx = c % rt; by = c / rt; bz = 0;
+        mstride = (int64_t)rt * BM;
+      } else {
+        const int tiles = rt * gridDim.y;
+        int splits = max(1, min(nkb_total, ctas / tiles));
+        kbps = (nkb_total + splits - 1) / splits;
+        splits = (nkb_total + kbps - 1) / kbps;
+        if (c >= tiles * splits) return;
+        bx = c % rt; by = (c / rt) % gridDim.y; bz = c / tiles;
+      }
+    }
+  }
+  const int m0 = bx * BM;
+  const int nt0 = by * tpc;
+  const int nt1 = min(n_tiles, nt0 + tpc);
+  const int kb0 = bz * kbps;
+  const int nkb = max(0, min(kb_end, kb0 + kbps) - kb0);
   const int b_tile0 = p.b_row0 / BN;
 
   if (tid == 0) {
@@ -250,7 +279,7 @@
   const bool a_stat = p.presplit && !p.no_astat && nkb_total <= AS_MAX_KB && gridDim.z == 1;
   const int nstages = a_stat ? (p.mode == 1 ? AS_STAGES_NOSCRATCH : AS_STAGES) : STAGES;
   const uint32_t stage_bytes = a_stat ? AS_STAGE_BYTES : STAGE_BYTES;
-  const int a_blk = min((int)blockIdx.x, (p.M + BM - 1) / BM - 1);
+  const int a_blk = min(bx, (M + BM - 1) / BM - 1);
   if (warp == MMA_WARP) tmem_alloc(tmem_slot, TMEM_COLS);
   tc_fence_before();
   __syncthreads();
@@ -287,7 +316,7 @@
         for (int s2 = 0; s2 < nstages; ++s2) mbar_wait(&full[s2], s2 < stage ? phase : phase ^ 1);
     } else if (lane == 0 && p.presplit) {
       const uint8_t* a_tiles = reinterpret_cast<const uint8_t*>(p.a_planes) +
-                               ((int64_t)blockIdx.x * (p.a_kbtot ? p.a_kbtot : nkb_total) + p.a_kb0) * PS_TILE;
+                               ((int64_t)bx * (p.a_kbtot ? p.a_kbtot : nkb_total) + p.a_kb0) * PS_TILE;
       const uint8_t* b_planes = reinterpret_cast<const uint8_t*>(p.b_planes);
       int stage = 0, phase = 0;
       for (int nt = nt0; nt < nt1; ++nt) {
@@ -437,16 +466,17 @@
     const int c_hi = wide_epi ? c_lo + 1 : c_lo + 2;
     const int ew = wide_epi ? c_lo * 4 + quarter : ehalf * 4 + quarter;
     const int row = m0 + quarter * 32 + lane;
-    const bool row_ok = row < p.M;
+    const bool row_ok = row < M;
     const float oscale = p.alpha * (p.alpha_dev ? *p.alpha_dev : 1.f) * ((p.c_row_scale && row_ok) ? __ldg(p.c_row_scale + row) : 1.f) /
                          (scale_from_amax(p.a_amax, p.a_amax_n, p.a_scale) * scale_from_amax(p.b_amax, p.b_amax_n, p.b_scale));
     float rm = -INFINITY, rs = 0.f, rt = 0.f, rav = -INFINITY, row_lse = 0.f, row_nlse2 = 0.f, row_scale = 0.f;
     int rai = 0x7fffffff, tgt = -1;
     if (p.mode != 0 && row_ok) {
-      const int b = row % p.B, tpos = row / p.B + 1;
+      const int n = p.row_map ? __ldg(p.row_map + row) : row;
+      const int b = n % p.B, tpos = n / p.B + 1;
       if (p.targets) tgt = (int)p.targets[(int64_t)b * p.tgt_stride_b + tpos];
       if (p.mode == 2) {
-        row_lse = p.lse[row];
+        row_lse = p.lse[n];
         row_nlse2 = -row_lse * kLog2e;
         row_scale = (tpos < p.lengths[b]) ? (p.grad_scale ? p.grad_scale[0] : 1.f) / (float)p.B : 0.f;
         tgt -= p.v0;
@@ -517,7 +547,7 @@
         if (p.mode == 2 && wide_epi) {
           const uint32_t sc = smem_u + OFF_SCRATCH + ew * (32 * 16 * 4);
           const int r0 = m0 + quarter * 32;
-          const int nr = min(32, p.M - r0);
+          const int nr = min(32, M - r0);
           const bool dead = row_scale == 0.f;
           DVAE_TC16_MARK(tid == 0 && tile == 2, 104);
 #pragma unroll
@@ -543,7 +573,7 @@
                   v[j] = (dead || col >= p.N) ? 0.f : (e - (col == tgt ? 1.f : 0.f)) * row_scale;
                 }
               }
-              if (p.p_planes_a && col0 + hh * 16 + h8 * 8 < p.p_kb_a * BK && m0 < (p.M + BM - 1) / BM * BM)
+              if (p.p_planes_a && col0 + hh * 16 + h8 * 8 < p.p_kb_a * BK && m0 < (M + BM - 1) / BM * BM)
                 store_plane_chunk(p.p_planes_a, row, col0 + hh * 16 + h8 * 8, p.p_kb_a, v, p.p_scale);
 #pragma unroll
               for (int j = 0; j < 8; ++j) sts32(sc + (lane * 16 + ((h8 * 8 + j) ^ ((lane >> 1) & 15))) * 4, v[j]);
@@ -616,11 +646,11 @@
           __syncwarp();
           const int col = col0 + lane;
           const int r0 = m0 + quarter * 32;
-          const int nr = min(32, p.M - r0);
+          const int nr = min(32, M - r0);
           if (col < p.N && nr > 0) {
             const bool split = gridDim.z > 1 || p.atomic_out;
             float badd = 0.f;
-            if (p.mode == 0 && (!split || blockIdx.z == 0)) {
+            if (p.mode == 0 && (!split || bz == 0)) {
               if (p.bias) badd += __ldg(p.bias + col);
               if (p.bias2) badd += __ldg(p.bias2 + col);
             }
@@ -634,6 +664,8 @@
               } else {
                 for (int rr = 0; rr < nr; ++rr) cp[rr * ldc] = chunk_at(rr) + badd;
               }
+            } else if (split && p.row_map) {
+              for (int rr = 0; rr < nr; ++rr) atomicAdd(p.C + (int64_t)__ldg(p.row_map + r0 + rr) * ldc + col, chunk_at(rr) + badd);
             } else if (split) {
               for (int rr = 0; rr < nr; ++rr) atomicAdd(cp + rr * ldc, chunk_at(rr) + badd);
             } else {
@@ -753,9 +785,9 @@
       if (tid == 0 && tile < 4) DBG16(15 + 2 * tile);
     }
     if (p.mode == 1 && row_ok) {
-      const int64_t sp = wide_epi ? (int64_t)blockIdx.y * 4 + c_lo : (int64_t)blockIdx.y * 2 + ehalf;
-      *reinterpret_cast<float4*>(p.part + (sp * p.M + row) * 4) = make_float4(rm, rs, rt, rav);
-      p.part_idx[sp * p.M + row] = rai;
+      const int64_t sp = wide_epi ? (int64_t)by * 4 + c_lo : (int64_t)by * 2 + ehalf;
+      *reinterpret_cast<float4*>(p.part + (sp * mstride + row) * 4) = make_float4(rm, rs, rt, rav);
+      p.part_idx[sp * mstride + row] = rai;
     }
   }
   tc_fence_before();
@@ -850,7 +882,7 @@
   }
   const char* mc_env = getenv("DVAE_TC16_MCAST");
   const bool mcast_on = mc_env && mc_env[0] == '1';
-  if (mcast_on && p.presplit && ceil_div(p.K, BK) <= AS_MAX_KB && grid.z == 1 && grid.x >= 2) {
+  if (mcast_on && p.presplit && ceil_div(p.K, BK) <= AS_MAX_KB && grid.z == 1 && grid.x >= 2 && !p.m_live) {
     p.mcast = 1;
     grid.x = (grid.x + 1) / 2 * 2;
     cudaLaunchConfig_t cfg = {};
@@ -936,8 +968,11 @@
 
 int linear_planes(const void* a_planes, const void* b_planes, float* C, int64_t ldc, int M, int N, int K, const float* bias,
                   float beta, int act, float a_scale, float b_scale, const float* c_row_scale, bool c_zeroed, int max_splits,
-                  cudaStream_t st, int b_kb0, int b_kbtot, int max_ctas, int a_kb0, int a_kbtot, const uint32_t* a_amax, int a_amax_n) {
+                  cudaStream_t st, int b_kb0, int b_kbtot, int max_ctas, int a_kb0, int a_kbtot, const uint32_t* a_amax, int a_amax_n,
+                  const int* m_live, const int* row_map, int live_k) {
   DVAE_REQUIRE(a_planes && b_planes && C && M > 0 && N > 0 && K > 0, "tc16 linear_planes: bad argument");
+  DVAE_REQUIRE(!m_live || ((beta == 1.f || (beta == 0.f && c_zeroed)) && act == 0 && !bias && !c_row_scale && (live_k || row_map)),
+               "tc16 linear_planes: live rows need a cleared (or accumulated) C, no bias / activation, and a row map for live M");
   Params p = {};
   p.presplit = 1; p.no_astat = 1; p.a_planes = a_planes; p.b_planes = b_planes; p.a_rows = M; p.b_rows = N;
   p.M = M; p.N = N; p.K = K; p.tiles_per_cta = 1; p.C = C; p.ldc = ldc; p.bias = bias; p.beta = beta; p.act = act; p.mode = 0;
@@ -946,6 +981,7 @@
   p.b_kb0 = b_kb0; p.b_kbtot = b_kbtot;
   p.a_kb0 = a_kb0; p.a_kbtot = a_kbtot;
   if (a_amax) { p.a_amax = a_amax; p.a_amax_n = a_amax_n; }
+  if (m_live) { p.m_live = m_live; p.row_map = row_map; p.live_k = live_k; p.atomic_out = 1; }
   const int tiles = ceil_div(M, BM) * ceil_div(N, BN), nkb = ceil_div(K, BK);
   int splits = 1;
   if (act == 0 && nkb >= 8) {
@@ -983,9 +1019,11 @@
 int ce_partials(const float* h, int64_t ldh, int N, int B, int H, int V, const float* w, const float* bias,
                 const int64_t* targets, int64_t tgt_stride_b, const int64_t* lengths, int tiles_per_split, int nsplit,
                 float* part, int* part_idx, const uint64_t* gumbel_seed, uint32_t gumbel_salt, const void* h_planes,
-                const void* w_planes, const int* skip_flag, cudaStream_t st) {
+                const void* w_planes, const int* skip_flag, cudaStream_t st, const int* m_live, const int* row_map) {
   Params p = {};
   p.skip_flag = skip_flag;
+  DVAE_REQUIRE(!m_live || (h_planes && w_planes && !gumbel_seed), "tc16 ce_partials: live rows need pre-split operands");
+  p.m_live = m_live; p.row_map = row_map;
   if (h_planes && w_planes) { p.presplit = 1; p.a_planes = h_planes; p.b_planes = w_planes; p.a_rows = N; p.b_rows = V; }
   p.A = h; p.lda = ldh; p.Bm = w; p.ldb = H;
   p.M = N; p.N = V; p.K = H; p.tiles_per_cta = tiles_per_split; p.bias = bias; p.mode = 1;
@@ -1001,8 +1039,10 @@
                  const int64_t* targets, int64_t tgt_stride_b, const int64_t* lengths, const float* lse,
                  const float* grad_scale, float* P, int64_t ldp, const void* h_planes, const void* w_planes, float* zero_buf,
                  int64_t zero_n4, float* zero_buf2, int64_t zero2_n4, cudaStream_t st, void* p_planes_a, void* p_planes_t,
-                 float* p_colsum, float p_scale) {
+                 float* p_colsum, float p_scale, const int* m_live, const int* row_map) {
   Params p = {};
+  DVAE_REQUIRE(!m_live || (p_planes_a && p_planes_t && h_planes && w_planes), "tc16 softmax_grad: live rows need the planes output");
+  p.m_live = m_live; p.row_map = row_map;
   if (p_planes_a && p_planes_t && h_planes && w_planes) {
     p.p_planes_a = reinterpret_cast<uint8_t*>(p_planes_a); p.p_planes_t = reinterpret_cast<uint8_t*>(p_planes_t);
     p.p_colsum = p_colsum; p.p_scale = p_scale; p.p_kb_a = ceil_div(vc, BK); p.p_kb_t = ceil_div(N, BK);
diff --git a/disentanglement-vae_b200/csrc/tc_gemm16.cuh b/disentanglement-vae_b200/csrc/tc_gemm16.cuh
--- a/disentanglement-vae_b200/csrc/tc_gemm16.cuh
+++ b/disentanglement-vae_b200/csrc/tc_gemm16.cuh
@@ -33,9 +33,18 @@
   const void* a_planes; const void* b_planes; int a_rows, b_rows;
   uint8_t* p_planes_a; uint8_t* p_planes_t; float* p_colsum; float p_scale; int p_kb_a, p_kb_t;
   const int* skip_flag;
+  const int* m_live; const int* row_map; int live_k;
   int dbg_skip_epilogue;
   unsigned long long* dbg;
 };
+
+__host__ __device__ inline void live_split(int row_tiles, int ctas, int col_tiles, int* tiles_per_cta, int* groups) {
+  int g = row_tiles > 0 ? ctas / row_tiles : 1;
+  g = g < 1 ? 1 : (g > col_tiles ? col_tiles : g);
+  const int tpc = (col_tiles + g - 1) / g;
+  *tiles_per_cta = tpc;
+  *groups = (col_tiles + tpc - 1) / tpc;
+}
 
 bool enabled();
 bool shape_ok(const float* A, int64_t lda, int trans_a, const float* B, int64_t ldb, int trans_b, int M, int N, int K);
@@ -43,11 +52,13 @@
 int linear(const float* A, int64_t lda, int trans_a, const float* B, int64_t ldb, int trans_b, float* C, int64_t ldc, int M,
            int N, int K, const float* bias, const float* bias2, float beta, int act, const GemmHints& hints, cudaStream_t st);
 int64_t plane_floats(int R, int K);
+bool single_acc_planes(int K);
 int split_planes(const float* X, int64_t ld, int R, int K, float scale, void* planes, cudaStream_t st, bool force_dual = false);
 int linear_planes(const void* a_planes, const void* b_planes, float* C, int64_t ldc, int M, int N, int K, const float* bias,
                   float beta, int act, float a_scale, float b_scale, const float* c_row_scale, bool c_zeroed, int max_splits,
                   cudaStream_t st, int b_kb0 = 0, int b_kbtot = 0, int max_ctas = 0, int a_kb0 = 0, int a_kbtot = 0,
-                  const uint32_t* a_amax = nullptr, int a_amax_n = 1);
+                  const uint32_t* a_amax = nullptr, int a_amax_n = 1, const int* m_live = nullptr, const int* row_map = nullptr,
+                  int live_k = 0);
 constexpr int kMaxPlaneEntries = 24;
 struct PlaneTable {
   struct Entry { const float* w; int R, C; void* planes; void* planes_t; int64_t ld; const uint32_t* amax; int amax_n; };
@@ -61,12 +72,14 @@
 int ce_partials(const float* h, int64_t ldh, int N, int B, int H, int V, const float* w, const float* bias,
                 const int64_t* targets, int64_t tgt_stride_b, const int64_t* lengths, int tiles_per_split, int nsplit,
                 float* part, int* part_idx, const uint64_t* gumbel_seed, uint32_t gumbel_salt, const void* h_planes,
-                const void* w_planes, const int* skip_flag, cudaStream_t st);
+                const void* w_planes, const int* skip_flag, cudaStream_t st, const int* m_live = nullptr,
+                const int* row_map = nullptr);
 int softmax_grad(const float* h, int64_t ldh, int N, int B, int H, int V, int v0, int vc, const float* w, const float* bias,
                  const int64_t* targets, int64_t tgt_stride_b, const int64_t* lengths, const float* lse,
                  const float* grad_scale, float* P, int64_t ldp, const void* h_planes, const void* w_planes, float* zero_buf,
                  int64_t zero_n4, float* zero_buf2, int64_t zero2_n4, cudaStream_t st, void* p_planes_a = nullptr,
-                 void* p_planes_t = nullptr, float* p_colsum = nullptr, float p_scale = 1.f);
+                 void* p_planes_t = nullptr, float* p_colsum = nullptr, float p_scale = 1.f, const int* m_live = nullptr,
+                 const int* row_map = nullptr);
 
 }
 }
diff --git a/disentanglement-vae_b200/csrc/tc_planes.cuh b/disentanglement-vae_b200/csrc/tc_planes.cuh
--- a/disentanglement-vae_b200/csrc/tc_planes.cuh
+++ b/disentanglement-vae_b200/csrc/tc_planes.cuh
@@ -9,6 +9,7 @@
 constexpr int kPlaneRows = 128, kPlaneK = 32;
 constexpr int kPlaneBytes = kPlaneRows * kPlaneK * 2, kPlaneTileBytes = 2 * kPlaneBytes;
 constexpr float kPlaneLoScale = 2048.f;
+constexpr float kSingleScale = 256.f;
 
 __device__ __forceinline__ uint32_t pack_hi_lo(float x0, float x1, float s, uint32_t& lo, float ls = kPlaneLoScale) {
   const float2 x = __fmul2_rn(make_float2(x0, x1), make_float2(s, s));
diff --git a/disentanglement-vae_b200/csrc/vocab_ce.cu b/disentanglement-vae_b200/csrc/vocab_ce.cu
--- a/disentanglement-vae_b200/csrc/vocab_ce.cu
+++ b/disentanglement-vae_b200/csrc/vocab_ce.cu
@@ -2,6 +2,7 @@
 
 #include "gemm_simt.cuh"
 #include "tc_gemm16.cuh"
+#include "tc_planes.cuh"
 
 namespace dvae {
 
@@ -30,6 +31,7 @@
   const uint64_t* gumbel_seed; uint32_t gumbel_salt;
   const void* h_planes; const void* w_planes;
   const int* skip_flag;
+  const int* m_live; const int* rows; int live_ctas;
 };
 
 __device__ __forceinline__ void merge_ms(float& m, float& s, float m2, float s2) {
@@ -128,15 +130,25 @@
   __shared__ float red[kFinThreads / 32];
   const int sub = threadIdx.x % kFinLanes, slot = threadIdx.x / kFinLanes;
   constexpr int kRows = kFinThreads / kFinLanes;
+  int rows = p.N, nsplit = p.nsplit;
+  int64_t stride = p.N;
+  if (p.m_live) {
+    rows = *p.m_live;
+    const int rt = (rows + GCE::BM - 1) / GCE::BM;
+    int tpc, groups;
+    tc16::live_split(rt, p.live_ctas, (p.V + GCE::BN - 1) / GCE::BN, &tpc, &groups);
+    nsplit = 4 * groups;
+    stride = (int64_t)rt * GCE::BM;
+  }
   float local = 0.f;
-  for (int n0 = blockIdx.x * kRows; n0 < p.N; n0 += gridDim.x * kRows) {
-    const int n = n0 + slot;
+  for (int k0 = blockIdx.x * kRows; k0 < rows; k0 += gridDim.x * kRows) {
+    const int k = k0 + slot;
     float m = -INFINITY, s = 0.f, t = 0.f, av = -INFINITY;
     int ai = 0x7fffffff;
-    if (n < p.N) {
-      for (int sp = sub; sp < p.nsplit; sp += kFinLanes) {
-        float4 q = *reinterpret_cast<const float4*>(p.part + ((int64_t)sp * p.N + n) * 4);
-        int qi = p.part_idx[(int64_t)sp * p.N + n];
+    if (k < rows) {
+      for (int sp = sub; sp < nsplit; sp += kFinLanes) {
+        float4 q = *reinterpret_cast<const float4*>(p.part + ((int64_t)sp * stride + k) * 4);
+        int qi = p.part_idx[(int64_t)sp * stride + k];
         merge_ms(m, s, q.x, q.y);
         t += q.z;
         if (q.w > av || (q.w == av && qi < ai)) { av = q.w; ai = qi; }
@@ -151,7 +163,8 @@
       t += t2;
       if (av2 > av || (av2 == av && ai2 < ai)) { av = av2; ai = ai2; }
     }
-    if (sub == 0 && n < p.N) {
+    if (sub == 0 && k < rows) {
+      const int n = p.rows ? p.rows[k] : k;
       float l = m + logf(s), e = l - t;
       if (lse) lse[n] = l;
       if (nll) nll[n] = e;
@@ -242,14 +255,17 @@
   }
 }
 
+static int64_t part_rows(const CeArgs& p) { return p.m_live ? (int64_t)ceil_div(p.N, GCE::BM) * GCE::BM : p.N; }
+
 static int ce_partials(CeArgs& p, cudaStream_t st) {
   if (!force_simt_gemm() && p.N >= 64 && p.V >= 128 && p.H >= 32 && tc16::supported(p.h, p.ldh, 0, p.w, p.H, 0, p.N, p.V, p.H)) {
     const int launched = p.nsplit;
     p.nsplit = (p.h_planes && p.w_planes ? 4 : 2) * launched;
-    p.part_idx = reinterpret_cast<int*>(p.part + (int64_t)p.nsplit * p.N * 4);
+    p.part_idx = reinterpret_cast<int*>(p.part + (int64_t)p.nsplit * part_rows(p) * 4);
+    if (p.m_live) p.live_ctas = ceil_div(p.N, GCE::BM) * launched;
     return tc16::ce_partials(p.h, p.ldh, p.N, p.B, p.H, p.V, p.w, p.bias, p.targets, p.tgt_stride_b, p.lengths,
                              p.tiles_per_split, launched, p.part, p.part_idx, p.gumbel_seed, p.gumbel_salt, p.h_planes,
-                             p.w_planes, p.skip_flag, st);
+                             p.w_planes, p.skip_flag, st, p.m_live, p.rows);
   }
   if (!force_simt_gemm() && p.N >= 64 && p.V >= 128 && p.H >= 32 && tc::tc_linear_supported(p.h, p.ldh, p.w, p.H, p.N, p.V, p.H))
     return tc::tc_ce_partials(p.h, p.ldh, p.N, p.B, p.H, p.V, p.w, p.bias, p.targets, p.tgt_stride_b, p.lengths,
@@ -294,11 +310,79 @@
   const int64_t nc = (vr + vmax - 1) / vmax;
   return (int)(((V + nc - 1) / nc + 127) / 128 * 128);
 }
+static bool tplanes_enabled() {
+  const char* e = getenv("DVAE_VOCAB_TPLANES");
+  return !(e && e[0] == '0');
+}
 static bool p_planes_enabled() {
   const char* e = getenv("DVAE_VOCAB_PPLANES");
   return !(e && e[0] == '0');
 }
 
+
+
+__global__ void __launch_bounds__(1024) vocab_live_rows_kernel(const int64_t* __restrict__ lengths, int T1, int B, int* __restrict__ rows,
+                                                               int* __restrict__ m_live) {
+  __shared__ int wcnt[32];
+  const int lane = threadIdx.x & 31, w = threadIdx.x >> 5, nw = blockDim.x >> 5;
+  int base = 0;
+  for (int t = 0; t < T1; ++t) {
+    for (int b0 = 0; b0 < B; b0 += blockDim.x) {
+      const int b = b0 + threadIdx.x;
+      const bool live = b < B && t + 1 < lengths[b];
+      const unsigned bal = __ballot_sync(0xffffffffu, live);
+      if (lane == 0) wcnt[w] = __popc(bal);
+      __syncthreads();
+      int before = 0, total = 0;
+      for (int i = 0; i < nw; ++i) {
+        const int c = wcnt[i];
+        before += i < w ? c : 0;
+        total += c;
+      }
+      __syncthreads();
+      if (live) rows[base + before + __popc(bal & ((1u << lane) - 1))] = t * B + b;
+      base += total;
+    }
+  }
+  if (threadIdx.x == 0) *m_live = base;
+}
+
+__global__ void __launch_bounds__(256) vocab_live_gather_kernel(const float* __restrict__ h, int N, int H, const int* __restrict__ rows,
+                                                                const int* __restrict__ m_live, float a_scale, float a_lo_scale,
+                                                                uint8_t* __restrict__ a_planes, uint8_t* __restrict__ t_planes) {
+  const int M = *m_live;
+  const int KB = (H + 31) / 32, KC = KB * 4;
+  const int64_t na = (int64_t)((M + 127) / 128) * 128 * KC;
+  const int HP = (H + 127) / 128 * 128, KBt = (N + 31) / 32;
+  const int64_t nt = (int64_t)HP * ((M + 31) / 32 * 4);
+  for (int64_t i = (int64_t)blockIdx.x * blockDim.x + threadIdx.x; i < na + nt; i += (int64_t)gridDim.x * blockDim.x) {
+    float v[8];
+    if (i < na) {
+      const int kc = (int)(i % KC), r = (int)(i / KC);
+      if (r < M && kc * 8 + 8 <= H) {
+        const float4* src = reinterpret_cast<const float4*>(h + (int64_t)__ldg(rows + r) * H + kc * 8);
+        const float4 x0 = __ldg(src), x1 = __ldg(src + 1);
+        v[0] = x0.x; v[1] = x0.y; v[2] = x0.z; v[3] = x0.w; v[4] = x1.x; v[5] = x1.y; v[6] = x1.z; v[7] = x1.w;
+      } else {
+#pragma unroll
+        for (int e = 0; e < 8; ++e) v[e] = 0.f;
+      }
+      uint4 hi, lo;
+      hi.x = tc16::pack_hi_lo(v[0], v[1], a_scale, lo.x, a_lo_scale); hi.y = tc16::pack_hi_lo(v[2], v[3], a_scale, lo.y, a_lo_scale);
+      hi.z = tc16::pack_hi_lo(v[4], v[5], a_scale, lo.z, a_lo_scale); hi.w = tc16::pack_hi_lo(v[6], v[7], a_scale, lo.w, a_lo_scale);
+      const int64_t off = tc16::plane_chunk_offset(r, kc * 8, KB);
+      *reinterpret_cast<uint4*>(a_planes + off) = hi;
+      *reinterpret_cast<uint4*>(a_planes + off + tc16::kPlaneBytes) = lo;
+    } else {
+      const int64_t j = i - na;
+      const int r = (int)(j % HP), k0 = (int)(j / HP) * 8;
+#pragma unroll
+      for (int e = 0; e < 8; ++e) v[e] = (r < H && k0 + e < M) ? __ldg(h + (int64_t)__ldg(rows + k0 + e) * H + r) : 0.f;
+      tc16::store_plane_chunk(t_planes, r, k0, KBt, v, 1.f);
+    }
+  }
+}
+
 }
 
 using namespace dvae;
@@ -306,11 +390,14 @@
 static int64_t ce_part_floats(int N, int V) {
   int tps;
   int ns = ce_nsplit(N, V, &tps);
-  return (4LL * ns * N * 5 + 8 + kFinMaxBlocks + 3) / 4 * 4;
-}
+  const int64_t rows = (int64_t)ceil_div(N, GCE::BM) * GCE::BM;
+  return (4LL * ns * rows * 5 + 8 + kFinMaxBlocks + 3) / 4 * 4;
+}
+static int64_t live_off(int N, int V, int H) { return ce_part_floats(N, V) + tc16::plane_floats(N, H) + tc16::plane_floats(V, H); }
 extern "C" int64_t dvae_vocab_ce_ws_floats(int N, int V, int H) {
-  return ce_part_floats(N, V) + tc16::plane_floats(N, H) + tc16::plane_floats(V, H);
-}
+  return live_off(N, V, H) + tc16::plane_floats(H, N) + (N + 8 + 3) / 4 * 4;
+}
+extern "C" int64_t dvae_vocab_live_rows_at(int N, int V, int H) { return live_off(N, V, H) + tc16::plane_floats(H, N); }
 
 static thread_local const void* g_wsplit_ws = nullptr;
 static thread_local const void* g_wsplit_w = nullptr;
@@ -326,14 +413,19 @@
   return DVAE_OK;
 }
 
+static bool live_ok(int N, int V, int H, const float* h, int64_t ldh, const float* w) {
+  return use_tc16(N, V, H, h, ldh, w) && use_presplit(N, V, H) && ldh == H && (reinterpret_cast<uintptr_t>(h) & 15) == 0 &&
+         (reinterpret_cast<uintptr_t>(w) & 15) == 0 && p_planes_enabled() && tplanes_enabled();
+}
+
 static int vocab_ce_fwd_impl(const float* h, int64_t ldh, int T1, int B, int H, int V, const float* w,
                              const float* bias, const int64_t* targets, int64_t tgt_stride_b,
                              const int64_t* lengths, int sos, float* lse, float* nll, int32_t* argmax,
-                             float* loss, float* ws, bool w_planes_ready, void* stream) {
+                             float* loss, float* ws, bool w_planes_ready, bool live, void* stream) {
   cudaStream_t st = (cudaStream_t)stream;
   DVAE_REQUIRE(h && w && bias && targets && lengths && loss && ws, "dvae_vocab_ce_fwd: null pointer");
   DVAE_REQUIRE(T1 > 0 && B > 0 && H > 0 && V > 0, "dvae_vocab_ce_fwd: bad shape T1=%d B=%d H=%d V=%d", T1, B, H, V);
-  CeArgs p;
+  CeArgs p = {};
   p.h = h; p.ldh = ldh; p.w = w; p.bias = bias; p.targets = targets; p.tgt_stride_b = tgt_stride_b;
   p.lengths = lengths; p.N = T1 * B; p.B = B; p.H = H; p.V = V; p.sos = sos;
   p.nsplit = ce_nsplit(p.N, V, &p.tiles_per_split);
@@ -345,13 +437,29 @@
     float* hp = ws + ce_part_floats(p.N, V);
     float* wp = hp + tc16::plane_floats(p.N, H);
     int rc;
-    if ((rc = tc16::split_planes(h, ldh, p.N, H, 1.f, hp, st))) return rc;
+    if (live && live_ok(p.N, V, H, h, ldh, w)) {
+      float* tp = ws + live_off(p.N, V, H);
+      int* rows = reinterpret_cast<int*>(tp + tc16::plane_floats(H, p.N));
+      const int nthr = min(1024, ceil_div(B, 32) * 32);
+      vocab_live_rows_kernel<<<1, nthr, 0, st>>>(lengths, T1, B, rows, rows + p.N);
+      DVAE_LAUNCH_CHECK();
+      const bool single = tc16::single_acc_planes(H);
+      const int64_t items = (tc16::plane_floats(p.N, H) + tc16::plane_floats(H, p.N)) / 16;
+      const int blocks = ceil_div(items, 256) < 148 * 4 ? ceil_div(items, 256) : 148 * 4;
+      vocab_live_gather_kernel<<<blocks, 256, 0, st>>>(h, p.N, H, rows, rows + p.N, single ? tc16::kSingleScale : 1.f,
+                                                       single ? 1.f : tc16::kPlaneLoScale, reinterpret_cast<uint8_t*>(hp),
+                                                       reinterpret_cast<uint8_t*>(tp));
+      DVAE_LAUNCH_CHECK();
+      p.rows = rows; p.m_live = rows + p.N;
+    } else if ((rc = tc16::split_planes(h, ldh, p.N, H, 1.f, hp, st))) {
+      return rc;
+    }
     if (!(w_planes_ready && g_wsplit_ws == ws && g_wsplit_w == w) && (rc = tc16::split_planes(w, H, V, H, 1.f, wp, st))) return rc;
     p.h_planes = hp; p.w_planes = wp;
   }
   g_wsplit_ws = g_wsplit_w = nullptr;
   { int rc = ce_partials(p, st); if (rc) return rc; }
-  float* block_sums = ws + (int64_t)p.nsplit * p.N * 5 + 8;
+  float* block_sums = ws + (int64_t)p.nsplit * part_rows(p) * 5 + 8;
   const int nblk = min(kFinMaxBlocks, ceil_div(p.N, kFinThreads / kFinLanes));
   vocab_ce_finalize_kernel<<<nblk, kFinThreads, 0, st>>>(p, lse, nll, argmax, block_sums);
   DVAE_LAUNCH_CHECK();
@@ -365,7 +473,7 @@
                                  const int64_t* lengths, int sos, float* lse, float* nll, int32_t* argmax,
                                  float* loss, float* ws, void* stream) {
   return vocab_ce_fwd_impl(h, ldh, T1, B, H, V, w, bias, targets, tgt_stride_b, lengths, sos, lse, nll, argmax, loss, ws,
-                           false, stream);
+                           false, false, stream);
 }
 
 extern "C" int dvae_vocab_ce_fwd_ex(const float* h, int64_t ldh, int T1, int B, int H, int V, const float* w,
@@ -373,7 +481,15 @@
                                     const int64_t* lengths, int sos, float* lse, float* nll, int32_t* argmax,
                                     float* loss, float* ws, int flags, void* stream) {
   return vocab_ce_fwd_impl(h, ldh, T1, B, H, V, w, bias, targets, tgt_stride_b, lengths, sos, lse, nll, argmax, loss, ws,
-                           (flags & 1) != 0, stream);
+                           (flags & 1) != 0, false, stream);
+}
+
+extern "C" int dvae_vocab_ce_fwd_live(const float* h, int64_t ldh, int T1, int B, int H, int V, const float* w,
+                                      const float* bias, const int64_t* targets, int64_t tgt_stride_b,
+                                      const int64_t* lengths, int sos, float* lse, float* nll, int32_t* argmax,
+                                      float* loss, float* ws, int flags, void* stream) {
+  return vocab_ce_fwd_impl(h, ldh, T1, B, H, V, w, bias, targets, tgt_stride_b, lengths, sos, lse, nll, argmax, loss, ws,
+                           (flags & 1) != 0, true, stream);
 }
 
 static int p_buffers(int N, int V) { return p_chunk(N, V) < V ? 2 : 1; }
@@ -388,6 +504,56 @@
 extern "C" int64_t dvae_vocab_ce_bwd_ws_floats(int N, int V, int H) {
   return p_region_floats(N, V) / 4 * 4 + tc16::plane_floats(N, H) + tc16::plane_floats(V, H) + tc16::plane_floats(H, V) +
          tc16::plane_floats(H, N);
+}
+
+static int dw_max_ctas() {
+  static const int cap = [] { const char* e = getenv("DVAE_VOCAB_DW_MAX_CTAS"); return e ? atoi(e) : 0; }();
+  return cap;
+}
+
+static const void* wT_planes_of(const float* w, int H, int V, float* tp, tc16::PlaneTable& tab, int* kbtot) {
+  tc16::PlaneHit hit;
+  if (tc16::find_weight_planes(w, H, 1, H, V, &hit) && hit.tile0 == 0 && hit.kb0 == 0) {
+    *kbtot = hit.kbtot;
+    return hit.planes;
+  }
+  tab.e[tab.n++] = tc16::PlaneTable::Entry{w, V, H, nullptr, tp};
+  *kbtot = ceil_div(V, 32);
+  return tp;
+}
+
+static int planes_bwd(const float* h, int64_t ldh, int N, int B, int H, int V, const float* w, const float* bias,
+                      const int64_t* targets, int64_t tgt_stride_b, const int64_t* lengths, const float* lse,
+                      const float* grad_scale_dev, float* d_h, int64_t lddh, float* d_w, float* d_bias, const void* h_planes,
+                      const void* w_planes, const void* wT_planes, int wT_kbtot, const void* hT_planes, float a_scale, float* ws,
+                      const int* m_live, const int* rows, cudaStream_t st) {
+  const int vc_max = p_chunk_planes(N, V), nbuf = p_buffers_planes(N, V);
+  const int64_t pa_fl = tc16::plane_floats(N, vc_max), pt_fl = tc16::plane_floats(vc_max, N);
+  DVAE_CUDA(cudaMemsetAsync(d_bias, 0, sizeof(float) * V, st));
+  int chunk = 0;
+  const int nchunks = ceil_div(V, vc_max);
+  for (int v0 = 0; v0 < V; v0 += vc_max, ++chunk) {
+    const int vc = min(vc_max, V - v0);
+    float* pa = ws + (int64_t)(chunk % nbuf) * (pa_fl + pt_fl);
+    float* pt = pa + pa_fl;
+    float* dw = d_w + (int64_t)v0 * H;
+    const bool zh = chunk == 0 && lddh == H && (((uintptr_t)d_h) & 15) == 0 && ((int64_t)N * H) % 4 == 0;
+    const bool zw = (((uintptr_t)dw) & 15) == 0 && ((int64_t)vc * H) % 4 == 0;
+    if (m_live && chunk == 0 && !zh) DVAE_CUDA(cudaMemsetAsync(d_h, 0, sizeof(float) * (size_t)N * H, st));
+    if (m_live && !zw) DVAE_CUDA(cudaMemsetAsync(dw, 0, sizeof(float) * (size_t)vc * H, st));
+    int rc;
+    if ((rc = tc16::softmax_grad(h, ldh, N, B, H, V, v0, vc, w, bias, targets, tgt_stride_b, lengths, lse, grad_scale_dev, nullptr,
+                                 vc_max, h_planes, w_planes, zh ? d_h : nullptr, (int64_t)N * H / 4, zw ? dw : nullptr,
+                                 (int64_t)vc * H / 4, st, pa, pt, d_bias + v0, a_scale, m_live, rows))) return rc;
+    Fork fork(st);
+    if ((rc = tc16::linear_planes(pa, wT_planes, d_h, lddh, N, H, vc, nullptr, chunk ? 1.f : 0.f, 0, a_scale, 1.f, nullptr,
+                                  m_live ? true : zh, 16, st, v0 / 32, wT_kbtot, 0, 0, 0, nullptr, 1, m_live, rows, 0))) return rc;
+    if ((rc = tc16::linear_planes(pt, hT_planes, dw, H, vc, H, N, nullptr, 0.f, 0, a_scale, 1.f, nullptr, m_live ? true : zw, 16,
+                                  fork.side(0), 0, 0, dw_max_ctas(), 0, 0, nullptr, 1, m_live, nullptr, 1))) return rc;
+    if (chunk + 1 == nchunks || chunk + 1 >= nbuf)
+      if ((rc = fork.join())) return rc;
+  }
+  return DVAE_OK;
 }
 
 extern "C" int dvae_vocab_ce_bwd(const float* h, int64_t ldh, int T1, int B, int H, int V, const float* w,
@@ -424,18 +590,11 @@
   }
   const void *wT_planes = nullptr, *hT_planes = nullptr;
   int wT_kbtot = 0;
-  if (h_planes && H % 32 == 0 && N >= 128 && (reinterpret_cast<uintptr_t>(w) & 15) == 0 && ldh == H &&
-      !(getenv("DVAE_VOCAB_TPLANES") && getenv("DVAE_VOCAB_TPLANES")[0] == '0')) {
+  if (h_planes && H % 32 == 0 && N >= 128 && (reinterpret_cast<uintptr_t>(w) & 15) == 0 && ldh == H && tplanes_enabled()) {
     float* tp = ws + front + tc16::plane_floats(N, H) + tc16::plane_floats(V, H);
-    tc16::PlaneHit hit;
     tc16::PlaneTable tab;
     tab.n = 0;
-    if (tc16::find_weight_planes(w, H, 1, H, V, &hit) && hit.tile0 == 0 && hit.kb0 == 0) {
-      wT_planes = hit.planes; wT_kbtot = hit.kbtot;
-    } else {
-      tab.e[tab.n++] = tc16::PlaneTable::Entry{w, V, H, nullptr, tp};
-      wT_planes = tp; wT_kbtot = ceil_div(V, 32);
-    }
+    wT_planes = wT_planes_of(w, H, V, tp, tab, &wT_kbtot);
     float* hp_t = tp + tc16::plane_floats(H, V);
     tab.e[tab.n++] = tc16::PlaneTable::Entry{h, N, H, nullptr, hp_t};
     hT_planes = hp_t;
@@ -444,12 +603,9 @@
   }
   const bool pp = wT_planes && hT_planes && h_planes && w_planes && p_planes_enabled() && lddh % 4 == 0 &&
                   tc16::supported(h, ldh, 0, w, H, 0, N, min(vc_max, V), H);
-  int64_t pa_fl = 0, pt_fl = 0;
-  if (pp) {
-    vc_max = p_chunk_planes(N, V); nbuf = p_buffers_planes(N, V);
-    pa_fl = tc16::plane_floats(N, vc_max); pt_fl = tc16::plane_floats(vc_max, N);
-    DVAE_CUDA(cudaMemsetAsync(d_bias, 0, sizeof(float) * V, st));
-  }
+  if (pp)
+    return planes_bwd(h, ldh, N, B, H, V, w, bias, targets, tgt_stride_b, lengths, lse, grad_scale_dev, d_h, lddh, d_w, d_bias,
+                      h_planes, w_planes, wT_planes, wT_kbtot, hT_planes, ph.a_scale, ws, nullptr, nullptr, st);
   int chunk = 0;
   const int nchunks = ceil_div(V, vc_max);
   for (int v0 = 0; v0 < V; v0 += vc_max, ++chunk) {
@@ -458,24 +614,6 @@
     p.v0 = v0; p.vc = vc; p.P = Pc;
     int rc;
     bool dh_zeroed = false, dw_zeroed = false;
-    if (pp) {
-      float* pa = ws + (int64_t)(chunk % nbuf) * (pa_fl + pt_fl);
-      float* pt = pa + pa_fl;
-      const bool zh = chunk == 0 && lddh == H && (((uintptr_t)d_h) & 15) == 0 && ((int64_t)N * H) % 4 == 0;
-      const bool zw = (((uintptr_t)(d_w + (int64_t)v0 * H)) & 15) == 0 && ((int64_t)vc * H) % 4 == 0;
-      if ((rc = tc16::softmax_grad(h, ldh, N, B, H, V, v0, vc, w, bias, targets, tgt_stride_b, lengths, lse, grad_scale_dev, nullptr,
-                                   vc_max, h_planes, w_planes, zh ? d_h : nullptr, (int64_t)N * H / 4,
-                                   zw ? d_w + (int64_t)v0 * H : nullptr, (int64_t)vc * H / 4, st, pa, pt, d_bias + v0, ph.a_scale))) return rc;
-      Fork fork(st);
-      if ((rc = tc16::linear_planes(pa, wT_planes, d_h, lddh, N, H, vc, nullptr, chunk ? 1.f : 0.f, 0, ph.a_scale, 1.f, nullptr, zh, 16, st,
-                                    v0 / 32, wT_kbtot))) return rc;
-      static const int dw_cap = [] { const char* e = getenv("DVAE_VOCAB_DW_MAX_CTAS"); return e ? atoi(e) : 0; }();
-      if ((rc = tc16::linear_planes(pt, hT_planes, d_w + (int64_t)v0 * H, H, vc, H, N, nullptr, 0.f, 0, ph.a_scale, 1.f, nullptr, zw, 16,
-                                    fork.side(0), 0, 0, dw_cap))) return rc;
-      if (chunk + 1 == nchunks || chunk + 1 >= nbuf)
-        if ((rc = fork.join())) return rc;
-      continue;
-    }
     if (!force_simt_gemm() && N >= 64 && vc >= 128 && H >= 32 && tc16::supported(h, ldh, 0, w, H, 0, N, vc, H)) {
       const bool zh = chunk == 0 && lddh == H && (((uintptr_t)d_h) & 15) == 0 && ((int64_t)N * H) % 4 == 0;
       const bool zw = (((uintptr_t)(d_w + (int64_t)v0 * H)) & 15) == 0 && ((int64_t)vc * H) % 4 == 0;
@@ -505,12 +643,42 @@
   return DVAE_OK;
 }
 
+extern "C" int dvae_vocab_ce_bwd_live(const float* h, int64_t ldh, int T1, int B, int H, int V, const float* w,
+                                      const float* bias, const int64_t* targets, int64_t tgt_stride_b,
+                                      const int64_t* lengths, const float* lse, const float* grad_scale_dev,
+                                      float* d_h, int64_t lddh, float* d_w, float* d_bias, const float* fwd_ws, float* ws,
+                                      void* stream) {
+  cudaStream_t st = (cudaStream_t)stream;
+  DVAE_REQUIRE(h && w && bias && targets && lengths && lse && d_h && d_w && d_bias && ws && fwd_ws, "dvae_vocab_ce_bwd_live: null pointer");
+  DVAE_REQUIRE(T1 > 0 && B > 0 && H > 0 && V > 0, "dvae_vocab_ce_bwd_live: bad shape");
+  const int N = T1 * B;
+  const bool fwd_live = live_ok(N, V, H, h, ldh, w);
+  if (!fwd_live || lddh != H || (reinterpret_cast<uintptr_t>(d_h) & 15))
+    return dvae_vocab_ce_bwd(h, ldh, T1, B, H, V, w, bias, targets, tgt_stride_b, lengths, lse, grad_scale_dev, d_h, lddh, d_w,
+                             d_bias, fwd_live ? nullptr : fwd_ws, ws, stream);
+  const float* hp = fwd_ws + ce_part_floats(N, V);
+  const float* wp = hp + tc16::plane_floats(N, H);
+  const float* hT_planes = fwd_ws + live_off(N, V, H);
+  const int* rows = reinterpret_cast<const int*>(hT_planes + tc16::plane_floats(H, N));
+  float a_scale = 1.f;
+  while (a_scale * 2.f <= (float)B) a_scale *= 2.f;
+  tc16::PlaneTable tab;
+  tab.n = 0;
+  int wT_kbtot;
+  const void* wT_planes = wT_planes_of(w, H, V, ws + p_region_floats(N, V) / 4 * 4 + tc16::plane_floats(N, H) + tc16::plane_floats(V, H),
+                                       tab, &wT_kbtot);
+  int rc = tc16::weight_planes_launch(tab, st);
+  if (rc) return rc;
+  return planes_bwd(h, ldh, N, B, H, V, w, bias, targets, tgt_stride_b, lengths, lse, grad_scale_dev, d_h, lddh, d_w, d_bias, hp, wp,
+                    wT_planes, wT_kbtot, hT_planes, a_scale, ws, rows + N, rows, st);
+}
+
 extern "C" int dvae_vocab_ce_partials(const float* h, int64_t ldh, int T1, int B, int H, int V, const float* w,
                                       const float* bias, const int64_t* targets, int64_t tgt_stride_b,
                                       const int64_t* lengths, int sos, float* ws, void* stream) {
   DVAE_REQUIRE(h && w && bias && targets && lengths && ws, "dvae_vocab_ce_partials: null pointer");
   DVAE_REQUIRE(T1 > 0 && B > 0 && H > 0 && V > 0, "dvae_vocab_ce_partials: bad shape");
-  CeArgs p;
+  CeArgs p = {};
   p.h = h; p.ldh = ldh; p.w = w; p.bias = bias; p.targets = targets; p.tgt_stride_b = tgt_stride_b;
   p.lengths = lengths; p.N = T1 * B; p.B = B; p.H = H; p.V = V; p.sos = sos;
   p.nsplit = ce_nsplit(p.N, V, &p.tiles_per_split);
@@ -531,7 +699,7 @@
   cudaStream_t st = (cudaStream_t)stream;
   DVAE_REQUIRE(h && w && bias && seed_dev && tokens_out && ws, "dvae_vocab_sample_step: null pointer");
   DVAE_REQUIRE(B > 0 && H > 0 && V > 0, "dvae_vocab_sample_step: bad shape");
-  CeArgs p;
+  CeArgs p = {};
   p.h = h; p.ldh = ldh; p.w = w; p.bias = bias; p.targets = nullptr; p.tgt_stride_b = 0; p.lengths = nullptr;
   p.N = B; p.B = B; p.H = H; p.V = V; p.sos = 0;
   p.nsplit = ce_nsplit(p.N, V, &p.tiles_per_split);
diff --git a/disentanglement-vae_b200/engine.py b/disentanglement-vae_b200/engine.py
--- a/disentanglement-vae_b200/engine.py
+++ b/disentanglement-vae_b200/engine.py
@@ -24,6 +24,7 @@
         self.lib = _lib.load()
         self.device = model._flat.device
         self.plan = StepPlan(model, B, T, self.device)
+        self.plan.live_rows = True
         self.d = d = self.plan.d
         self.world = dist.get_world_size(process_group) if (dist.is_available() and dist.is_initialized()) else 1
         self.rank = dist.get_rank(process_group) if self.world > 1 else 0
diff --git a/disentanglement-vae_b200/plan.py b/disentanglement-vae_b200/plan.py
--- a/disentanglement-vae_b200/plan.py
+++ b/disentanglement-vae_b200/plan.py
@@ -73,6 +73,7 @@
         self.recon = self.out[_lib.HEADS_NSCALARS:_lib.HEADS_NSCALARS + 1]
         self.ce_ws = buf(self.lib.dvae_vocab_ce_ws_floats(max(self.N, 1), d.V, d.Hd))
         self.sample_ws = None
+        self.live_rows = False
         self._bwd_ready = False
         self.seed_dev = torch.zeros(1, device=device, dtype=torch.int64)
         self.labels = buf(max(sum(1 for o in d.dsc_out if o > 0), 1), B)
@@ -256,23 +257,27 @@
         lib, d, st = self.lib, self.d, _lib.stream_ptr()
         w_ready = getattr(self, "_w_planes_ready", None) == P["decoder.linear.weight"].data_ptr()
         self._w_planes_ready = None
-        check(lib.dvae_vocab_ce_fwd_ex(ptr(h_top), d.Hd, self.T1, self.B, d.Hd, d.V, ptr(P["decoder.linear.weight"]),
-                                       ptr(P["decoder.linear.bias"]), ptr(targets), targets.stride(0), ptr(lengths),
-                                       d.sos, ptr(self.lse), ptr(self.nll), ptr(self.argmax), ptr(self.recon),
-                                       ptr(self.ce_ws), 1 if w_ready else 0, st), "dvae_vocab_ce_fwd")
-        self._ce_planes_valid = (h_top.data_ptr(), P["decoder.linear.weight"].data_ptr())
+        fwd = lib.dvae_vocab_ce_fwd_live if self.live_rows else lib.dvae_vocab_ce_fwd_ex
+        check(fwd(ptr(h_top), d.Hd, self.T1, self.B, d.Hd, d.V, ptr(P["decoder.linear.weight"]),
+                  ptr(P["decoder.linear.bias"]), ptr(targets), targets.stride(0), ptr(lengths),
+                  d.sos, ptr(self.lse), ptr(self.nll), ptr(self.argmax), ptr(self.recon),
+                  ptr(self.ce_ws), 1 if w_ready else 0, st), "dvae_vocab_ce_fwd")
+        self._ce_planes_valid = (h_top.data_ptr(), P["decoder.linear.weight"].data_ptr(), lengths.data_ptr(), self.live_rows)
         return self.recon
 
     def vocab_ce_bwd(self, P, G, h_top, targets, lengths, grad_scale_dev):
         self._alloc_bwd()
         lib, d, st = self.lib, self.d, _lib.stream_ptr()
-        reuse = getattr(self, "_ce_planes_valid", None) == (h_top.data_ptr(), P["decoder.linear.weight"].data_ptr())
+        valid = getattr(self, "_ce_planes_valid", None)
+        reuse = valid is not None and valid[:3] == (h_top.data_ptr(), P["decoder.linear.weight"].data_ptr(), lengths.data_ptr())
+        live = reuse and valid[3]
         self._ce_planes_valid = None
-        check(lib.dvae_vocab_ce_bwd(ptr(h_top), d.Hd, self.T1, self.B, d.Hd, d.V, ptr(P["decoder.linear.weight"]),
-                                    ptr(P["decoder.linear.bias"]), ptr(targets), targets.stride(0), ptr(lengths),
-                                    ptr(self.lse), ptr(grad_scale_dev), ptr(self.g_top), d.Hd,
-                                    ptr(G["decoder.linear.weight"]), ptr(G["decoder.linear.bias"]),
-                                    ptr(self.ce_ws) if reuse else None, ptr(self.ce_bwd_ws), st),
+        bwd = lib.dvae_vocab_ce_bwd_live if live else lib.dvae_vocab_ce_bwd
+        check(bwd(ptr(h_top), d.Hd, self.T1, self.B, d.Hd, d.V, ptr(P["decoder.linear.weight"]),
+                  ptr(P["decoder.linear.bias"]), ptr(targets), targets.stride(0), ptr(lengths),
+                  ptr(self.lse), ptr(grad_scale_dev), ptr(self.g_top), d.Hd,
+                  ptr(G["decoder.linear.weight"]), ptr(G["decoder.linear.bias"]),
+                  ptr(self.ce_ws) if reuse else None, ptr(self.ce_bwd_ws), st),
               "dvae_vocab_ce_bwd")
         return self.g_top
 
diff --git a/include/dvae_b200.h b/include/dvae_b200.h
--- a/include/dvae_b200.h
+++ b/include/dvae_b200.h
@@ -162,6 +162,12 @@
                          const int64_t* lengths, int sos, float* lse, float* nll, int32_t* argmax,
                          float* loss, float* ws, int flags, void* stream);
 
+int dvae_vocab_ce_fwd_live(const float* h, int64_t ldh, int T1, int B, int H, int V, const float* w,
+                           const float* bias, const int64_t* targets, int64_t tgt_stride_b,
+                           const int64_t* lengths, int sos, float* lse, float* nll, int32_t* argmax,
+                           float* loss, float* ws, int flags, void* stream);
+int64_t dvae_vocab_live_rows_at(int N, int V, int H);
+
 int dvae_vocab_ce_partials(const float* h, int64_t ldh, int T1, int B, int H, int V, const float* w,
                            const float* bias, const int64_t* targets, int64_t tgt_stride_b,
                            const int64_t* lengths, int sos, float* ws, void* stream);
@@ -196,6 +202,12 @@
                       float* d_h, int64_t lddh, float* d_w, float* d_bias, const float* fwd_ws, float* ws,
                       void* stream);
 
+int dvae_vocab_ce_bwd_live(const float* h, int64_t ldh, int T1, int B, int H, int V, const float* w,
+                           const float* bias, const int64_t* targets, int64_t tgt_stride_b,
+                           const int64_t* lengths, const float* lse, const float* grad_scale_dev,
+                           float* d_h, int64_t lddh, float* d_w, float* d_bias, const float* fwd_ws, float* ws,
+                           void* stream);
+
 int dvae_grad_sumsq(const float* g, int64_t n, float* sumsq, float* ws, void* stream);
 int dvae_clip_adam(float* p, float* g, float* m, float* v, int64_t n, const float* sumsq,
                    float max_norm, float grad_scale, const float* hyper_dev, int zero_grad,
```

After: 1.229 million, median of 6. +6.7%, better.
